# kwea123/nsff_pl

Measured on AMD Instinct MI355X. Metric: ray-samples/sec (coarse+fine, static+dynamic), higher is better.
Workload: dtype f16x3 (fp32 operands split into 2 halfs, 3 f16 MFMAs per product, fp32 accumulate; same 1e-4 parity as f32); 1 GPU; C2 (BASELINE.json configs[1]): static+dynamic NSFF, 1024 rays/GPU x (64 coarse + 64 importance -> 192 fine pts), train-mode fwd, fw/bw flow warp t+-1, perturb=1 noise_std=1, 8x256 MLPs, N_tau=48, all 47 outputs on device.  `value` is render_rays' throughput with autograd DISABLED (the train-mode FLAGS, inference launches: nothing kept for a backward pass); what a trainer's forward costs is aux.tra; rays_per_gpu=1024, N_samples=64, N_importance=64, parallelism=single GPU, field_launch=persistent (one workgroup per CU)

## Files before the change

### include/nsff_render.h

```cpp
#ifndef NSFF_RENDER_H
#define NSFF_RENDER_H

#include <stddef.h>
#include <stdint.h>

#ifdef __cplusplus
extern "C" {
#endif

#define NSFF_OK               0
#define NSFF_ERR_INVALID     -1
#define NSFF_ERR_NULL        -2
#define NSFF_ERR_ALIGN       -3
#define NSFF_ERR_HIP         -4

#define NSFF_ABI_VERSION      32
#define NSFF_RAW_STRIDE      16
#define NSFF_MAX_FREQS       24
#define NSFF_MAX_LAYERS       8


typedef struct NsffModelDesc {
    int32_t D;
    int32_t W;
// ... 43 lines not shown
    int32_t tile_points;
    int32_t pts_per_ray;
    int32_t static_mode;
    int32_t transient_mode;
    int32_t flow_heads;
    const float* xyz;
    int32_t n_freqs;
    float   freqs[NSFF_MAX_FREQS];
    const float* dir_emb;
    const float* a_emb;
    const float* t_emb;
    const float* x_emb;
    int32_t ld_emb;
    int32_t off_xyz, off_dir, off_a, off_t;
    float*  raw;
    void*   save_acts;
    void*   save_xin;
    void*   save_masks;
    void*   save_side;
    const float* t_bias;
    int32_t t_bias_rows;
    int32_t reserved0;
    const float* s_bias;
    int32_t s_bias_rows;
    int32_t launch_form;
    int64_t save_lo_delta[3];
} NsffFieldArgs;

int nsff_field_query(const NsffModelDesc* desc, const void* packed,
                     const NsffFieldArgs* args, void* stream);

#define NSFF_MAX_TIME_BIAS_JOBS 4
typedef struct NsffTimeBiasJob {
    const NsffModelDesc* desc;
    const float* w[NSFF_MAX_LAYERS];
    const float* b[NSFF_MAX_LAYERS];
    const float* t_rows;
    float* out;
    const float* table;
    const int64_t* ts;
    int64_t n_table, max_t;
    int32_t delta, pad_;
    float* rows_out;
} NsffTimeBiasJob;
int nsff_time_bias_rows(const NsffModelDesc* desc);
int nsff_time_bias(const NsffTimeBiasJob* jobs, int32_t n_jobs, int64_t n_rays, void* stream);

#define NSFF_MAX_RNG_JOBS 12
typedef struct NsffRngJob {
    float*   out;
    int64_t  numel;
    uint64_t offset;
    int32_t  kind;
    uint32_t grid;
} NsffRngJob;
int nsff_rng_draws(const NsffRngJob* jobs, int32_t n_jobs, uint64_t seed, void* stream);
typedef struct NsffRngCoarse {
    const float* rays;
    const float* z_lin;
    float*       zs;
    float*       xyz;
    int32_t      n_samples;
    float        perturb;
    int32_t      job;
    int32_t      pad_;
} NsffRngCoarse;
int nsff_rng_draws_coarse(const NsffRngJob* jobs, int32_t n_jobs, uint64_t seed, const NsffRngCoarse* coarse, void* stream);

int nsff_side_bias(const NsffModelDesc* desc, const void* packed_f16x3, const float* w_dir, const float* dir_rows,
                   const float* a_rows, int64_t n_rays, float* out, void* stream);

int nsff_train_dims(const NsffModelDesc* desc, int32_t* xin_rows, int32_t* t_row0, int32_t* side_rows);
int nsff_bwd_packed_bytes(const NsffModelDesc* desc, size_t* bytes);
int nsff_pack_weights_bwd(const NsffModelDesc* desc, const float* const* params, void* packed, void* stream);
int nsff_pack_weights_bwd_ex(const NsffModelDesc* desc, const float* const* params, void* packed, const void* fwd_packed, void* stream);

typedef struct NsffFieldBwdArgs {
    int64_t n_points;
    int32_t static_mode;
    int32_t transient_mode;
    const float* d_raw;
    const float* raw;
    const float* gmax;
    const void*  masks;
    void*  dpre;
    void*  dhead;
    float* d_xin;
    float* d_side;
    int64_t dpre_lo_delta;
} NsffFieldBwdArgs;
int nsff_field_backward(const NsffModelDesc* desc, const void* packed_bwd, const NsffFieldBwdArgs* args, void* stream);
int nsff_last_bwd_kernel(void);
int nsff_last_bwd_grid(void);
int nsff_field_bwd_phase_program(const NsffModelDesc* desc, int32_t dynamic, int32_t want_xin, int64_t n_tiles, uint32_t* out,
                                 int32_t max_phases, uint32_t* seg_offsets, int32_t max_segs);

#define NSFF_BWD_LAUNCH_C    1
#define NSFF_BWD_LAUNCH_H3B  2
#define NSFF_BWD_LAUNCH_X3   3
int nsff_field_bwd_launch_plan(const NsffModelDesc* desc, const NsffFieldBwdArgs* args, int32_t n_cus, int32_t kernel_override,
                               int32_t persist, int32_t* out, int32_t max_launches);

int nsff_field_input_backward(const float* d_xin, int32_t xin_rows, int32_t t_row0, const float* xyz, int64_t n_rays,
                              int32_t pts_per_ray, const float* freqs_host, int32_t n_freqs, int32_t in_t, float* d_xyz,
                              float* d_t, void* stream);

typedef struct NsffWgradJob {
    const void* a;  const void* b;
    int32_t a_rows, b_rows;
    int64_t out_off;
    int32_t trunk, pad_;
    int64_t a_lo_delta, b_lo_delta;
} NsffWgradJob;
int64_t nsff_weight_grad_scratch(const NsffWgradJob* jobs, int32_t n_jobs, int64_t n_tiles, int32_t n_splits);
int nsff_weight_grad(const NsffWgradJob* jobs, int32_t n_jobs, int64_t n_tiles, int32_t n_splits,
                     float* scratch, float* out, float* bias, const float* gmax, void* stream);

typedef struct NsffGradMapEntry {
    int32_t dst;
    int32_t e_a, e_b;
    int16_t job_a, job_b;
} NsffGradMapEntry;
int nsff_weight_grad_accumulate(const NsffWgradJob* jobs, int32_t n_jobs, int64_t n_tiles, int32_t n_splits, float* scratch,
                                const NsffGradMapEntry* map, int64_t n_map, float* grad_base, const float* gmax, void* stream);

int nsff_weight_grad_accumulate_aux(const NsffWgradJob* jobs, int32_t n_jobs, int64_t n_tiles, int32_t n_splits, float* scratch,
                                    const NsffGradMapEntry* map, int64_t n_map, float* grad_base, float* aux, const float* gmax,
                                    void* stream);

typedef struct NsffFoldGradArgs {
    int32_t n_rows, pad_;
    const float* g; const float* gb;
    const float* w_final; const float* b_final;
    const float* w_head[16];
    float* d_w_head[16]; float* d_b_head[16];
    float* d_w_final; float* d_b_final;
} NsffFoldGradArgs;
int nsff_fold_grads(const NsffFoldGradArgs* args, void* stream);

typedef struct NsffFoldDenseArgs {
    int32_t n_rows, accumulate;
    int32_t ld_head, ld_dhead;
    const float* g; const float* g2; const float* gb; const float* gb2;
    const float* w_head; const float* w_final; const float* b_final;
    float* d_w_head; float* d_b_head; float* d_w_final; float* d_b_final;
} NsffFoldDenseArgs;
int nsff_fold_grads_dense(const NsffFoldDenseArgs* args, void* stream);

int nsff_absmax(const float* x, int64_t n, float* out, void* stream);
int nsff_absmax_raw(const float* d_raw, int64_t n_points, float* out16, void* stream);

int nsff_adam_step(float* param, const float* grad, float* exp_avg, float* exp_avg_sq, int64_t n, float* state,
                   const float* lr, double beta1, double beta2, double eps, double weight_decay, void* stream);

int nsff_adam_step_segments(float* param, const float* grad, float* exp_avg, float* exp_avg_sq, int64_t n, float* state,
                            const float* lr, double beta1, double beta2, double eps, double weight_decay,
                            const int64_t* seg_start, int n_seg, int32_t* seg_used, void* stream);

int nsff_sgd_step(float* param, const float* grad, float* momentum_buf, int64_t n, float* state, const float* lr,
                  double momentum, double weight_decay, const int64_t* seg_start, int n_seg, int32_t* seg_used, void* stream);

int nsff_radam_step(float* param, const float* grad, float* exp_avg, float* exp_avg_sq, int64_t n, float* state,
                    const float* lr, double beta1, double beta2, double eps, double weight_decay,
                    const int64_t* seg_start, int n_seg, int32_t* seg_used, void* stream);

typedef struct NsffLossArgs {
    int64_t n_rays; int32_t n_samples; int32_t n_keep;
    int32_t n_frames; int32_t max_t;
    double  topk;
    int32_t thickness; int32_t pad_;
    const float* rgb_fine; const float* rgb_coarse;
    const float* depth_fine; const float* depth_coarse;
    const float* t_weights; const float* s_weights;
    const float* xyz_fw; const float* xyz_bw;
    const float* rgb_fw; const float* rgb_bw;
    const float* disocc_fw; const float* disocc_bw;
    const float* disoccs_fw; const float* disoccs_bw;
    const float* xyzs_fw_bw; const float* xyzs_bw_fw;
    const float* xyzs_fine; const float* xyzs_fw; const float* xyzs_bw;
    const float* rgbs; const float* disps;
    const int64_t* ts; const int64_t* cam_ids;
    const float* uv_fw; const float* uv_bw;
    const float* Ks; const float* Ps;
    const float* hyper;
    float* stats;
    float* terms;
    const float* term_w;
    const float* weights;
    float* per_ray;
    float* coef;
    float* g_rgb_fine; float* g_rgb_coarse; float* g_depth_fine; float* g_depth_coarse;
    float* g_t_weights; float* g_s_weights; float* g_xyz_fw; float* g_xyz_bw; float* g_rgb_fw; float* g_rgb_bw;
    float* g_xyzs_fw_bw; float* g_xyzs_bw_fw; float* g_xyzs_fw; float* g_xyzs_bw;
} NsffLossArgs;
int nsff_nerfw_loss(const NsffLossArgs* args, int mode, void* stream);
#define NSFF_LOSS_MAX_RAYS 1048576
size_t nsff_nerfw_loss_work_bytes(long long n_rays);
int nsff_nerfw_loss_ex(const NsffLossArgs* args, int mode, void* work, size_t work_bytes, void* stream);
int nsff_last_loss_path(void);

int nsff_coarse_samples(const float* rays, int64_t n_rays, const float* z_lin, int32_t n_samples,
                        float perturb, const float* perturb_rand,
                        float* zs, float* xyz, void* stream);

int nsff_fine_samples(const float* rays, int64_t n_rays, const float* z_lin, const float* zs_coarse,
                      int32_t n_samples, int32_t n_importance,
                      const float* weights_static, const float* weights_transient,
                      const float* u_static, const float* u_transient, int32_t u_per_ray,
                      float* samples_static, float* samples_transient,
                      float* zs_fine, float* xyz_fine, void* stream);

int nsff_sample_pdf(const float* bins, const float* weights, int64_t n_rays, int32_t n_bins_minus1,
                    const float* u, int32_t n_importance, int32_t u_per_ray, float eps,
                    float* samples, void* stream);

int nsff_warp_points(const float* raw, const float* xyz, const float* zs, int64_t n_points,
                     float z_far, float* xyz_fw, float* xyz_bw, void* stream);

int nsff_frame_rays(const float* K4_host, const float* c2w_host, int32_t H, int32_t W, float near, float shift_near,
                    int64_t first_pixel, int64_t n_pixels, float* rays, void* stream);

#define NSFF_FRAME_TABLE     16
typedef struct NsffRayRecordArgs {
    int32_t n_frames, H, W;
    int32_t first_frame, frame_count;
    int32_t image_u8, mask_u8;
    float   fx, fy, cx, cy, near;
    int64_t n_pixels;
    const void*  images;
    const float* disps;
    const void*  masks;
    const float* flow_fw;
    const float* flow_bw;
    const float* frame_table;
    float*       records;
} NsffRayRecordArgs;
int nsff_ray_records(const NsffRayRecordArgs* args, void* stream);

#define NSFF_ERR_UNSUPPORTED     -5
#define NSFF_RESIZE_LANCZOS_U8    0
#define NSFF_RESIZE_NEAREST_PIL   1
#define NSFF_RESIZE_NEAREST_CV    2
#define NSFF_RESIZE_LINEAR_CV     3
#define NSFF_RESIZE_MAX_KSIZE    49
int nsff_resize_ksize(int32_t filter, int32_t n_in, int32_t n_out);
int nsff_resize_table(int32_t filter, int32_t n_in, int32_t n_out, int32_t* start, int32_t* count, void* weights);

typedef struct NsffFrameResizeArgs {
    int32_t n_frames, filter, channels, pad_;
    int32_t src_h, src_w, dst_h, dst_w;
    int32_t ksize_x, ksize_y;
    float   ratio[2];
    const void* src;  void* dst;
    const int32_t* x_start;  const int32_t* x_count;  const void* x_weights;
    const int32_t* y_start;  const int32_t* y_count;  const void* y_weights;
} NsffFrameResizeArgs;
int nsff_frame_resize(const NsffFrameResizeArgs* args, void* stream);

typedef struct NsffFrustumArgs {
    const float*   w2c;
    const int64_t* ts;
    float   K4[4];
    int32_t n_cams, n_frames, H, W;
} NsffFrustumArgs;

typedef struct NsffCompositeArgs {
    int64_t n_rays;
    int32_t n_samples;
    int32_t has_transient;
    int32_t has_rgb;
    int32_t flow_mode;
    int32_t want_disocc;
    float   noise_std;
    float   z_far;
    const float* raw;
    const float* raw_fw;
    const float* raw_bw;
    const float* zs;
    const float* xyz;
    const float* xyz_fw;
    const float* xyz_bw;
    const float* noise_static;
    const float* noise_transient;
    const float* noise_fw;
    const float* noise_bw;
    const float* visibility;
    float* static_rgbs;  float* transient_rgbs;
    float* flows_fw;     float* flows_bw;
    float* static_sigmas; float* transient_sigmas;
    float* static_alphas; float* transient_alphas;
    float* static_weights; float* transient_weights; float* weights;
    float* xyzs_fw_bw;   float* xyzs_bw_fw;
    float* disoccs_fw;   float* disoccs_bw;
    float* depth;  float* rgb;  float* transient_alpha;  float* transient_rgb;
    float* static_only_rgb;  float* static_only_depth;
    float* xyz_exp;  float* flow_fw_exp;  float* flow_bw_exp;  float* xyz_fw_exp;  float* xyz_bw_exp;
    float* rgb_fw;   float* rgb_bw;
    float* disocc_fw;  float* disocc_bw;
    NsffFrustumArgs vis;
} NsffCompositeArgs;

int nsff_composite(const NsffCompositeArgs* args, void* stream);

int nsff_frustum_visibility(const NsffFrustumArgs* vis, const float* xyz, int64_t n_points, float* vis_count,
                            void* stream);

typedef struct NsffSplatArgs {
    int32_t H, W, n_planes;
    float   K4[4];
    float   P[12];
    float   scale;
    const float* xyz;
    const float* flow;
    const float* rgb;
    const float* alpha;
    float*       accum;
    void*        work;
    int64_t      work_bytes;
} NsffSplatArgs;
int64_t nsff_splat_work_bytes(int32_t H, int32_t W, int32_t n_planes);
int nsff_splat_planes(const NsffSplatArgs* args, void* stream);

typedef struct NsffMpiArgs {
    int32_t H, W, n_planes;
    float   dt;
    const float* accum_fw;
    const float* accum_bw;
    const float* static_rgb;
    const float* static_alpha;
    const float* zs;
    float* rgb;
    float* depth;
} NsffMpiArgs;
int nsff_mpi_composite(const NsffMpiArgs* args, void* stream);

typedef struct NsffCompositeBwdArgs {
    int64_t n_rays;
    int32_t n_samples, has_transient, flow_mode;
    float   noise_std;
    const float* raw;  const float* raw_fw;  const float* raw_bw;
    const float* zs;   const float* xyz;     const float* f_fw;  const float* f_bw;
    const float* noise_static;  const float* noise_transient;  const float* noise_fw;  const float* noise_bw;
    const float* g_static_sigmas;  const float* g_transient_sigmas;
    const float* g_static_weights; const float* g_transient_weights;  const float* g_weights;
    const float* g_depth;  const float* g_rgb;  const float* g_transient_alpha;  const float* g_transient_rgb;
    const float* g_so_rgb; const float* g_so_depth;
    const float* g_xyz_exp;  const float* g_flow_fw_exp;  const float* g_flow_bw_exp;
    const float* g_rgb_fw;   const float* g_rgb_bw;
    float* scratch;
    float* d_raw;  float* d_raw_fw;  float* d_raw_bw;  float* d_f_fw;  float* d_f_bw;
} NsffCompositeBwdArgs;
int nsff_composite_backward(const NsffCompositeBwdArgs* args, void* stream);

typedef struct {
    int64_t n_points;
    const float* zs;
    float z_far;
    int32_t accumulate;
    int32_t col_a, col_b;
    int32_t pad_;
    const float* g_a[4];
    const float* g_b[4];
    float* out;
} NsffFlowGradArgs;
int nsff_flow_grad(const NsffFlowGradArgs* args, void* stream);

#define NSFF_RAY_RECORD      16

typedef struct NsffSsimArgs {
    int32_t n_frames, H, W, window;
    const float* gt;  const float* pred;  const uint8_t* mask;
    float* map;  float* mean_map;  double* sums;
    void* scratch;  int64_t scratch_bytes;
} NsffSsimArgs;
int64_t nsff_ssim_scratch_bytes(int32_t n_frames, int32_t H, int32_t W);
int nsff_ssim(const NsffSsimArgs* args, void* stream);

typedef struct NsffFrameFinishArgs {
    int32_t n_frames, H, W, pad_;
    const float* rgb;  const float* gt;  const uint8_t* valid;  const float* depth;  const uint8_t* lut;
    float* rgb_clipped;  uint8_t* rgb_u8;  double* sums;  float* depth_range;  uint8_t* depth_u8;  uint8_t* depth_rgb_u8;
    void* scratch;  int64_t scratch_bytes;
} NsffFrameFinishArgs;
int64_t nsff_frame_finish_scratch_bytes(int32_t n_frames, int32_t H, int32_t W);
int nsff_frame_finish(const NsffFrameFinishArgs* args, void* stream);

typedef struct NsffValPanelsArgs {
    int32_t n_frames, H, W, pad_;
    const float* gt;  const float* pred;  const float* depth;  const float* transient_alpha;  const float* static_rgb;
    const float* static_depth;  const float* mask;  const float* disp;  const float* ssim_loss;
    const uint8_t* lut_depth;  const uint8_t* lut_mask;
    float* ranges;  uint8_t* grid_u8;  uint8_t* rmse_u8;  uint8_t* ssim_u8;  uint8_t* rmse_blend_u8;  uint8_t* ssim_blend_u8;
    void* scratch;  int64_t scratch_bytes;
} NsffValPanelsArgs;
int64_t nsff_val_panels_scratch_bytes(int32_t n_frames, int32_t H, int32_t W);
int nsff_val_panels(const NsffValPanelsArgs* args, void* stream);

#define NSFF_FLOW_UNKNOWN    1e10f
typedef struct NsffFlowMapsArgs {
    int32_t n_frames, H, W, n_poses, max_t, share_gt_scale;
    float   fx, fy, cx, cy;
    const float* xyz[2];  const float* Ps;  const int32_t* ts;
    float* flow[2];  const float* gt[2];  const uint8_t* mask;
    double* epe_sums;  int64_t* epe_counts;  float* maxrad;  const float* scale;
    uint8_t* image[2];  uint8_t* gt_image[2];
    void* scratch;  int64_t scratch_bytes;
} NsffFlowMapsArgs;
int64_t nsff_flow_maps_scratch_bytes(int32_t n_frames, int32_t H, int32_t W);
int nsff_flow_maps(const NsffFlowMapsArgs* args, void* stream);

#define NSFF_TRACK_MAX_POINTS 0x7fffffffLL
typedef struct NsffTrackStepArgs {
    int64_t n_rows;
    int32_t pts_per_row, direction, max_t, n_poses, fixed_view, pad_;
    float   fx, fy, cx, cy;
    const float* raw;  const float* xyz_in;  const int32_t* t_in;  const uint8_t* alive_in;
    float* xyz_out;  int32_t* t_out;  uint8_t* alive_out;
    const float* Ps;  float* uv;  float* depth;
} NsffTrackStepArgs;
int nsff_track_step(const NsffTrackStepArgs* args, void* stream);

#define NSFF_TRACK_MAX_TRACKS (1 << 20)
#define NSFF_TRACK_MAX_STEPS  (1 << 11)
typedef struct NsffTrackDrawArgs {
    int32_t H, W, n_steps, n_tracks;
    const float* uv;  const uint8_t* ok;  const uint8_t* image;  const uint8_t* lut;  uint8_t* out;
    void* scratch;  int64_t scratch_bytes;
} NsffTrackDrawArgs;
int64_t nsff_track_draw_scratch_bytes(int32_t H, int32_t W);
int nsff_track_draw(const NsffTrackDrawArgs* args, void* stream);

typedef struct NsffMotionMapsArgs {
    int32_t n_frames, H, W, epipolar;
    float   alpha, beta, threshold, pad_;
    const float* flow_fw;  const float* flow_bw;  const float* Fm;
    float* err;  uint8_t* valid;  uint8_t* raw;
    int64_t* counts;  double* err_sums;
    void* scratch;  int64_t scratch_bytes;
} NsffMotionMapsArgs;
int64_t nsff_motion_maps_scratch_bytes(int32_t n_frames, int32_t H, int32_t W);
int nsff_motion_maps(const NsffMotionMapsArgs* args, void* stream);

#define NSFF_ERODE_MAX_K 31
typedef struct NsffMaskErodeArgs {
    int32_t n_frames, H, W, k;
    const uint8_t* src;  uint8_t* dst;  int64_t* zero_counts;
    void* scratch;  int64_t scratch_bytes;
} NsffMaskErodeArgs;
int nsff_mask_erode(const NsffMaskErodeArgs* args, void* stream);

#define NSFF_OPTFLOW_MIN_SIZE 16
#define NSFF_OPTFLOW_TILE     32
#define NSFF_OPTFLOW_K        3
#define NSFF_OPTFLOW_FUSED    1
typedef struct NsffOptflowIterArgs {
    int32_t n_pairs, H, W, iters;
    int32_t fused, tile, k, pad_;
    float   lambda, theta, tau, pad1_;
    const float* consts;  float* state[2];
} NsffOptflowIterArgs;
typedef struct NsffOptflowArgs {
    int32_t n_pairs, H, W, channels;
    int32_t levels, warps, iters, median;
    int32_t fused, tile, k, pad_;
    float   lambda, theta, tau, pad1_;
    const void* images0;  const void* images1;  float* flow;
    void* scratch;  int64_t scratch_bytes;
} NsffOptflowArgs;
int     nsff_optflow_grey(const void* src, float* dst, int32_t n, int32_t H, int32_t W, int32_t channels, void* stream);
int     nsff_optflow_down(const float* src, float* dst, int32_t n, int32_t H, int32_t W, void* stream);
int     nsff_optflow_up(const float* src, float* dst, int32_t n, int32_t H, int32_t W, void* stream);
int     nsff_optflow_median(const float* src, float* dst, int32_t n, int32_t H, int32_t W, void* stream);
int     nsff_optflow_warp(const float* I0, const float* I1, const float* u, float* consts, int32_t n_pairs, int32_t H, int32_t W,
                          void* stream);
int     nsff_optflow_iterate(const NsffOptflowIterArgs* args, void* stream);
int     nsff_optflow_result_slot(int32_t iters, int32_t k);
int     nsff_optflow_levels(int32_t H, int32_t W, int32_t levels);
int64_t nsff_optflow_scratch_bytes(int32_t n_pairs, int32_t H, int32_t W, int32_t levels);
int     nsff_optflow(const NsffOptflowArgs* args, void* stream);

int nsff_cdf(const float* weights, int64_t n_frames, int64_t n, double* cdf, void* stream);

typedef struct NsffRayDrawArgs {
    int64_t n_frames, n_pixels, frame, batch;
    const float* records;  const double* cdf;  const float* u;
    float* rays;  float* rgbs;  int64_t* ts;  int64_t* cam_ids;  float* disps;  float* rays_mask;  float* uv_fw;  float* uv_bw;
    int64_t* rand_idx;
} NsffRayDrawArgs;
int nsff_ray_draw(const NsffRayDrawArgs* args, void* stream);

int nsff_prof_enable(int on);
int nsff_prof_collect(int64_t* launches, double* total_ms, double* total_flops, double* executed_flops);
int nsff_prof_collect_clock(int64_t* launches, double* total_ms, double* total_flops, double* executed_flops,
                            double* shader_ticks, double* ticks_ms);

#define NSFF_KERNEL_F32       1
#define NSFF_KERNEL_H3_64     2
#define NSFF_KERNEL_H3_8WAVE  3
#define NSFF_KERNEL_H3A       4
#define NSFF_KERNEL_H3_SAVE   5
#define NSFF_KERNEL_H3A_TBIAS 7
#define NSFF_KERNEL_H3A_SAVE  9
#define NSFF_KERNEL_H3A_SIDE  8
int         nsff_last_field_kernel(void);
int         nsff_last_field_grid(void);
int         nsff_field_mfma_shape(const NsffModelDesc* desc, const NsffFieldArgs* args);
int         nsff_repack_field_weights(const NsffModelDesc* desc, const void* packed, void* repacked, void* stream);
int         nsff_field_query_repacked(const NsffModelDesc* desc, const void* packed, const void* repacked, const NsffFieldArgs* args,
                                      void* stream);
int         nsff_last_field_mfma_shape(void);
int         nsff_field_phase_program(const NsffModelDesc* desc, int static_mode, int transient_mode, int fold_t, uint32_t* steps,
                             int* n_steps, int* n_static_steps, uint32_t* phases_static, uint32_t* phases_dynamic, int* n_phases);

#define NSFF_PLAN_WORDS 12
#define NSFF_LAUNCH_SIDE_TILE      1
#define NSFF_LAUNCH_H3_64          2
#define NSFF_LAUNCH_H3_64_SAVE     3
#define NSFF_LAUNCH_H3_8WAVE       4
#define NSFF_LAUNCH_H3_8WAVE_SAVE  5
#define NSFF_LAUNCH_H3A            6
#define NSFF_LAUNCH_H3A_SAVE       7
int         nsff_field_launch_plan(const NsffModelDesc* desc, const NsffFieldArgs* args, int32_t n_cus, int32_t no_persist,
                                   int32_t* out, int32_t max_launches);

#define NSFF_RANGE_ACT     0x1u
#define NSFF_RANGE_SAVED   0x2u
#define NSFF_RANGE_PARAMS  0x4u
#define NSFF_RANGE_CODES   0x8u
int         nsff_range_flags(uint32_t* out, int32_t clear, void* stream);

#define NSFF_LPIPS_MIN_SIZE  31

typedef struct NsffLpipsWeights {
    const float* conv_w[5];  const float* conv_b[5];  const float* lin[5];
} NsffLpipsWeights;
int64_t nsff_lpips_packed_bytes(void);
int     nsff_lpips_pack(const NsffLpipsWeights* weights, float* packed, void* stream);

int     nsff_lpips_dims(int32_t H, int32_t W, int32_t* hw);

typedef struct NsffLpipsArgs {
    int32_t n_frames, H, W, normalize;
    const float* gt;  const float* pred;  const uint8_t* valid;
    const float* packed;
    float* map;  double* sums;
    void* workspace;  int64_t workspace_bytes;
} NsffLpipsArgs;
int64_t nsff_lpips_workspace_bytes(int32_t n_frames, int32_t H, int32_t W);
int     nsff_lpips(const NsffLpipsArgs* args, void* stream);

typedef struct NsffSceneScaleArgs {
    int32_t n_frames, n_points, H, W;
    int32_t disp_rank[2];
    const double* points;  const uint8_t* vis;  const double* w2c;  const float* K;  const float* disps;
    double* stats;  float* disp_os;  double* depth_os;  int32_t* pix;
    void* work;  int64_t work_bytes;
} NsffSceneScaleArgs;
int64_t nsff_scene_scale_work_bytes(int32_t n_frames, int32_t n_points, int32_t H, int32_t W);
int     nsff_scene_scale(const NsffSceneScaleArgs* args, void* stream);

int         nsff_abi_version(void);
const char* nsff_last_hip_error(void);

#ifdef __cplusplus
}
#endif
#endif
```

### nsff_pl_amd/_lib.py

```python
import ctypes as C
import os

import torch

_HERE = os.path.dirname(os.path.abspath(__file__))
LIB_PATH = os.environ.get("NSFF_LIB") or os.path.join(_HERE, "libnsff_hip.so")

RAW_STRIDE = 16
ABI_VERSION = 32
MAX_FREQS = 24

_ERR = {-1: "NSFF_ERR_INVALID (bad shape/flag/unsupported architecture)",
        -2: "NSFF_ERR_NULL (required pointer missing)",
        -3: "NSFF_ERR_ALIGN (pointer not 16-byte aligned)",
        -4: "NSFF_ERR_HIP",
        -5: "NSFF_ERR_UNSUPPORTED (a valid request outside what the kernels are built for)"}

_fp = C.c_void_p


class ModelDesc(C.Structure):
    _fields_ = [("D", C.c_int32), ("W", C.c_int32), ("skip", C.c_int32),
                ("in_xyz", C.c_int32), ("in_dir", C.c_int32), ("in_a", C.c_int32),
                ("in_t", C.c_int32), ("use_viewdir", C.c_int32),
                ("has_transient", C.c_int32), ("has_flow", C.c_int32),
                ("flow_scale", C.c_float), ("skip_mask", C.c_int32)]


class FieldArgs(C.Structure):
    _fields_ = [("n_points", C.c_int64), ("precision", C.c_int32), ("tile_points", C.c_int32),
                ("pts_per_ray", C.c_int32),
                ("static_mode", C.c_int32), ("transient_mode", C.c_int32),
                ("flow_heads", C.c_int32),
                ("xyz", _fp), ("n_freqs", C.c_int32), ("freqs", C.c_float * MAX_FREQS),
                ("dir_emb", _fp), ("a_emb", _fp), ("t_emb", _fp),
                ("x_emb", _fp), ("ld_emb", C.c_int32),
                ("off_xyz", C.c_int32), ("off_dir", C.c_int32), ("off_a", C.c_int32),
                ("off_t", C.c_int32), ("raw", _fp), ("save_acts", _fp), ("save_xin", _fp), ("save_masks", _fp),
                ("save_side", _fp), ("t_bias", _fp), ("t_bias_rows", C.c_int32), ("reserved0", C.c_int32),
                ("s_bias", _fp), ("s_bias_rows", C.c_int32), ("launch_form", C.c_int32), ("save_lo_delta", C.c_int64 * 3)]


class TimeBiasJob(C.Structure):
    _fields_ = [("desc", C.POINTER(ModelDesc)), ("w", _fp * 8), ("b", _fp * 8), ("t_rows", _fp), ("out", _fp),
                ("table", _fp), ("ts", _fp), ("n_table", C.c_int64), ("max_t", C.c_int64), ("delta", C.c_int32), ("pad_", C.c_int32),
                ("rows_out", _fp)]


MAX_TIME_BIAS_JOBS = 4


class RngJob(C.Structure):
    _fields_ = [("out", _fp), ("numel", C.c_int64), ("offset", C.c_uint64), ("kind", C.c_int32), ("grid", C.c_uint32)]


MAX_RNG_JOBS = 12


class RngCoarse(C.Structure):
    _fields_ = [("rays", _fp), ("z_lin", _fp), ("zs", _fp), ("xyz", _fp), ("n_samples", C.c_int32), ("perturb", C.c_float),
                ("job", C.c_int32), ("pad_", C.c_int32)]


_COMPOSITE_PTRS_IN = ["raw", "raw_fw", "raw_bw", "zs", "xyz", "xyz_fw", "xyz_bw",
                      "noise_static", "noise_transient", "noise_fw", "noise_bw", "visibility"]
_COMPOSITE_PTRS_OUT = ["static_rgbs", "transient_rgbs", "flows_fw", "flows_bw",
                       "static_sigmas", "transient_sigmas", "static_alphas", "transient_alphas",
                       "static_weights", "transient_weights", "weights",
                       "xyzs_fw_bw", "xyzs_bw_fw", "disoccs_fw", "disoccs_bw",
                       "depth", "rgb", "transient_alpha", "transient_rgb",
                       "static_only_rgb", "static_only_depth",
                       "xyz_exp", "flow_fw_exp", "flow_bw_exp", "xyz_fw_exp", "xyz_bw_exp",
                       "rgb_fw", "rgb_bw", "disocc_fw", "disocc_bw"]


class FrustumArgs(C.Structure):
    _fields_ = [("w2c", _fp), ("ts", _fp), ("K4", C.c_float * 4), ("n_cams", C.c_int32), ("n_frames", C.c_int32),
                ("H", C.c_int32), ("W", C.c_int32)]


class CompositeArgs(C.Structure):
    _fields_ = ([("n_rays", C.c_int64), ("n_samples", C.c_int32), ("has_transient", C.c_int32),
                 ("has_rgb", C.c_int32), ("flow_mode", C.c_int32), ("want_disocc", C.c_int32),
                 ("noise_std", C.c_float), ("z_far", C.c_float)]
                + [(n, _fp) for n in _COMPOSITE_PTRS_IN]
                + [(n, _fp) for n in _COMPOSITE_PTRS_OUT]
                + [("vis", FrustumArgs)])


_CBWD_IN = ["raw", "raw_fw", "raw_bw", "zs", "xyz", "f_fw", "f_bw", "noise_static", "noise_transient", "noise_fw", "noise_bw"]
_CBWD_G = ["g_static_sigmas", "g_transient_sigmas", "g_static_weights", "g_transient_weights", "g_weights", "g_depth",
           "g_rgb", "g_transient_alpha", "g_transient_rgb", "g_so_rgb", "g_so_depth", "g_xyz_exp", "g_flow_fw_exp",
           "g_flow_bw_exp", "g_rgb_fw", "g_rgb_bw"]
_CBWD_OUT = ["scratch", "d_raw", "d_raw_fw", "d_raw_bw", "d_f_fw", "d_f_bw"]


class CompositeBwdArgs(C.Structure):
    _fields_ = ([("n_rays", C.c_int64), ("n_samples", C.c_int32), ("has_transient", C.c_int32), ("flow_mode", C.c_int32),
                 ("noise_std", C.c_float)] + [(n, _fp) for n in _CBWD_IN + _CBWD_G + _CBWD_OUT])


class FieldBwdArgs(C.Structure):
    _fields_ = [("n_points", C.c_int64), ("static_mode", C.c_int32), ("transient_mode", C.c_int32),
                ("d_raw", _fp), ("raw", _fp), ("gmax", _fp), ("masks", _fp), ("dpre", _fp), ("dhead", _fp),
                ("d_xin", _fp), ("d_side", _fp), ("dpre_lo_delta", C.c_int64)]


class WgradJob(C.Structure):
    _fields_ = [("a", _fp), ("b", _fp), ("a_rows", C.c_int32), ("b_rows", C.c_int32), ("out_off", C.c_int64), ("trunk", C.c_int32),
                ("pad_", C.c_int32), ("a_lo_delta", C.c_int64), ("b_lo_delta", C.c_int64)]


class FoldGradArgs(C.Structure):
    _fields_ = [("n_rows", C.c_int32), ("pad_", C.c_int32), ("g", _fp), ("gb", _fp), ("w_final", _fp), ("b_final", _fp),
                ("w_head", _fp * 16), ("d_w_head", _fp * 16), ("d_b_head", _fp * 16), ("d_w_final", _fp), ("d_b_final", _fp)]


class FoldDenseArgs(C.Structure):
    _fields_ = [("n_rows", C.c_int32), ("accumulate", C.c_int32), ("ld_head", C.c_int32), ("ld_dhead", C.c_int32),
                ("g", _fp), ("g2", _fp), ("gb", _fp), ("gb2", _fp), ("w_head", _fp), ("w_final", _fp), ("b_final", _fp),
                ("d_w_head", _fp), ("d_b_head", _fp), ("d_w_final", _fp), ("d_b_final", _fp)]


class SplatArgs(C.Structure):
    _fields_ = [("H", C.c_int32), ("W", C.c_int32), ("n_planes", C.c_int32), ("K4", C.c_float * 4),
                ("P", C.c_float * 12), ("scale", C.c_float),
                ("xyz", _fp), ("flow", _fp), ("rgb", _fp), ("alpha", _fp), ("accum", _fp), ("work", _fp),
                ("work_bytes", C.c_int64)]


class MpiArgs(C.Structure):
    _fields_ = [("H", C.c_int32), ("W", C.c_int32), ("n_planes", C.c_int32), ("dt", C.c_float),
                ("accum_fw", _fp), ("accum_bw", _fp), ("static_rgb", _fp), ("static_alpha", _fp), ("zs", _fp),
                ("rgb", _fp), ("depth", _fp)]


_LOSS_IN = ["rgb_fine", "rgb_coarse", "depth_fine", "depth_coarse", "t_weights", "s_weights", "xyz_fw", "xyz_bw", "rgb_fw",
            "rgb_bw", "disocc_fw", "disocc_bw", "disoccs_fw", "disoccs_bw", "xyzs_fw_bw", "xyzs_bw_fw", "xyzs_fine",
            "xyzs_fw", "xyzs_bw", "rgbs", "disps", "ts", "cam_ids", "uv_fw", "uv_bw", "Ks", "Ps", "hyper", "stats", "terms",
            "term_w"]
LOSS_GRADS = ["g_rgb_fine", "g_rgb_coarse", "g_depth_fine", "g_depth_coarse", "g_t_weights", "g_s_weights", "g_xyz_fw",
              "g_xyz_bw", "g_rgb_fw", "g_rgb_bw", "g_xyzs_fw_bw", "g_xyzs_bw_fw", "g_xyzs_fw", "g_xyzs_bw"]


class LossArgs(C.Structure):
    _fields_ = ([("n_rays", C.c_int64), ("n_samples", C.c_int32), ("n_keep", C.c_int32), ("n_frames", C.c_int32),
                 ("max_t", C.c_int32), ("topk", C.c_double), ("thickness", C.c_int32), ("pad_", C.c_int32)]
                + [(n, _fp) for n in _LOSS_IN] + [("weights", _fp), ("per_ray", _fp), ("coef", _fp)]
                + [(n, _fp) for n in LOSS_GRADS])


class FlowGradArgs(C.Structure):
    _fields_ = [("n_points", C.c_int64), ("zs", _fp), ("z_far", C.c_float), ("accumulate", C.c_int32), ("col_a", C.c_int32),
                ("col_b", C.c_int32), ("pad_", C.c_int32), ("g_a", _fp * 4), ("g_b", _fp * 4), ("out", _fp)]


class SsimArgs(C.Structure):
    _fields_ = [("n_frames", C.c_int32), ("H", C.c_int32), ("W", C.c_int32), ("window", C.c_int32),
                ("gt", _fp), ("pred", _fp), ("mask", _fp), ("map", _fp), ("mean_map", _fp), ("sums", _fp),
                ("scratch", _fp), ("scratch_bytes", C.c_int64)]


class LpipsWeights(C.Structure):
    _fields_ = [("conv_w", _fp * 5), ("conv_b", _fp * 5), ("lin", _fp * 5)]


class LpipsArgs(C.Structure):
    _fields_ = [("n_frames", C.c_int32), ("H", C.c_int32), ("W", C.c_int32), ("normalize", C.c_int32),
                ("gt", _fp), ("pred", _fp), ("valid", _fp), ("packed", _fp), ("map", _fp), ("sums", _fp),
                ("workspace", _fp), ("workspace_bytes", C.c_int64)]


_FINISH_PTRS = ["rgb", "gt", "valid", "depth", "lut", "rgb_clipped", "rgb_u8", "sums", "depth_range", "depth_u8", "depth_rgb_u8"]


class FrameFinishArgs(C.Structure):
    _fields_ = ([("n_frames", C.c_int32), ("H", C.c_int32), ("W", C.c_int32), ("pad_", C.c_int32)]
                + [(n, _fp) for n in _FINISH_PTRS] + [("scratch", _fp), ("scratch_bytes", C.c_int64)])


_PANEL_IN = ["gt", "pred", "depth", "transient_alpha", "static_rgb", "static_depth", "mask", "disp", "ssim_loss"]
_PANEL_LUT = ["lut_depth", "lut_mask"]
_PANEL_OUT = ["ranges", "grid_u8", "rmse_u8", "ssim_u8", "rmse_blend_u8", "ssim_blend_u8"]
PANEL_FIELDS = ("depth", "static_depth", "neg_disp", "neg_rmse", "neg_ssim")


class ValPanelsArgs(C.Structure):
    _fields_ = ([("n_frames", C.c_int32), ("H", C.c_int32), ("W", C.c_int32), ("pad_", C.c_int32)]
                + [(n, _fp) for n in _PANEL_IN + _PANEL_LUT + _PANEL_OUT] + [("scratch", _fp), ("scratch_bytes", C.c_int64)])


FLOW_UNKNOWN = 1e10


class FlowMapsArgs(C.Structure):
    _fields_ = [("n_frames", C.c_int32), ("H", C.c_int32), ("W", C.c_int32), ("n_poses", C.c_int32), ("max_t", C.c_int32),
                ("share_gt_scale", C.c_int32), ("fx", C.c_float), ("fy", C.c_float), ("cx", C.c_float), ("cy", C.c_float),
                ("xyz", _fp * 2), ("Ps", _fp), ("ts", _fp), ("flow", _fp * 2), ("gt", _fp * 2), ("mask", _fp),
                ("epe_sums", _fp), ("epe_counts", _fp), ("maxrad", _fp), ("scale", _fp), ("image", _fp * 2), ("gt_image", _fp * 2),
                ("scratch", _fp), ("scratch_bytes", C.c_int64)]


TRACK_MAX_POINTS, TRACK_MAX_TRACKS, TRACK_MAX_STEPS = 0x7fffffff, 1 << 20, 1 << 11


class TrackStepArgs(C.Structure):
    _fields_ = [("n_rows", C.c_int64), ("pts_per_row", C.c_int32), ("direction", C.c_int32), ("max_t", C.c_int32),
                ("n_poses", C.c_int32), ("fixed_view", C.c_int32), ("pad_", C.c_int32),
                ("fx", C.c_float), ("fy", C.c_float), ("cx", C.c_float), ("cy", C.c_float),
                ("raw", _fp), ("xyz_in", _fp), ("t_in", _fp), ("alive_in", _fp), ("xyz_out", _fp), ("t_out", _fp), ("alive_out", _fp),
                ("Ps", _fp), ("uv", _fp), ("depth", _fp)]


class TrackDrawArgs(C.Structure):
    _fields_ = [("H", C.c_int32), ("W", C.c_int32), ("n_steps", C.c_int32), ("n_tracks", C.c_int32),
                ("uv", _fp), ("ok", _fp), ("image", _fp), ("lut", _fp), ("out", _fp), ("scratch", _fp), ("scratch_bytes", C.c_int64)]


ERODE_MAX_K = 31


class MotionMapsArgs(C.Structure):
    _fields_ = [("n_frames", C.c_int32), ("H", C.c_int32), ("W", C.c_int32), ("epipolar", C.c_int32),
                ("alpha", C.c_float), ("beta", C.c_float), ("threshold", C.c_float), ("pad_", C.c_float),
                ("flow_fw", _fp), ("flow_bw", _fp), ("Fm", _fp), ("err", _fp), ("valid", _fp), ("raw", _fp),
                ("counts", _fp), ("err_sums", _fp), ("scratch", _fp), ("scratch_bytes", C.c_int64)]


class MaskErodeArgs(C.Structure):
    _fields_ = [("n_frames", C.c_int32), ("H", C.c_int32), ("W", C.c_int32), ("k", C.c_int32),
                ("src", _fp), ("dst", _fp), ("zero_counts", _fp), ("scratch", _fp), ("scratch_bytes", C.c_int64)]


OPTFLOW_MIN_SIZE, OPTFLOW_TILE, OPTFLOW_K, OPTFLOW_FUSED = 16, 32, 3, 1
OPTFLOW_PAIRS = ((16, 2), (32, 2), (32, 3), (32, 4), (32, 6))


class OptflowIterArgs(C.Structure):
    _fields_ = [("n_pairs", C.c_int32), ("H", C.c_int32), ("W", C.c_int32), ("iters", C.c_int32),
                ("fused", C.c_int32), ("tile", C.c_int32), ("k", C.c_int32), ("pad_", C.c_int32),
                ("lam", C.c_float), ("theta", C.c_float), ("tau", C.c_float), ("pad1_", C.c_float),
                ("consts", _fp), ("state", _fp * 2)]


class OptflowArgs(C.Structure):
    _fields_ = [("n_pairs", C.c_int32), ("H", C.c_int32), ("W", C.c_int32), ("channels", C.c_int32),
                ("levels", C.c_int32), ("warps", C.c_int32), ("iters", C.c_int32), ("median", C.c_int32),
                ("fused", C.c_int32), ("tile", C.c_int32), ("k", C.c_int32), ("pad_", C.c_int32),
                ("lam", C.c_float), ("theta", C.c_float), ("tau", C.c_float), ("pad1_", C.c_float),
                ("images0", _fp), ("images1", _fp), ("flow", _fp), ("scratch", _fp), ("scratch_bytes", C.c_int64)]


RAY_RECORD = 16
_DRAW_OUT = ["rays", "rgbs", "ts", "cam_ids", "disps", "rays_mask", "uv_fw", "uv_bw", "rand_idx"]


class RayDrawArgs(C.Structure):
    _fields_ = ([("n_frames", C.c_int64), ("n_pixels", C.c_int64), ("frame", C.c_int64), ("batch", C.c_int64),
                 ("records", _fp), ("cdf", _fp), ("u", _fp)] + [(n, _fp) for n in _DRAW_OUT])


FRAME_TABLE = 16


class RayRecordArgs(C.Structure):
    _fields_ = [("n_frames", C.c_int32), ("H", C.c_int32), ("W", C.c_int32), ("first_frame", C.c_int32),
                ("frame_count", C.c_int32), ("image_u8", C.c_int32), ("mask_u8", C.c_int32),
                ("fx", C.c_float), ("fy", C.c_float), ("cx", C.c_float), ("cy", C.c_float), ("near", C.c_float),
                ("n_pixels", C.c_int64), ("images", _fp), ("disps", _fp), ("masks", _fp), ("flow_fw", _fp), ("flow_bw", _fp),
                ("frame_table", _fp), ("records", _fp)]


RESIZE_LANCZOS_U8, RESIZE_NEAREST_PIL, RESIZE_NEAREST_CV, RESIZE_LINEAR_CV = range(4)
RESIZE_MAX_KSIZE = 49
ERR_UNSUPPORTED = -5


class FrameResizeArgs(C.Structure):
    _fields_ = [("n_frames", C.c_int32), ("filter", C.c_int32), ("channels", C.c_int32), ("pad_", C.c_int32),
                ("src_h", C.c_int32), ("src_w", C.c_int32), ("dst_h", C.c_int32), ("dst_w", C.c_int32),
                ("ksize_x", C.c_int32), ("ksize_y", C.c_int32), ("ratio", C.c_float * 2), ("src", _fp), ("dst", _fp),
                ("x_start", _fp), ("x_count", _fp), ("x_weights", _fp), ("y_start", _fp), ("y_count", _fp), ("y_weights", _fp)]


class SceneScaleArgs(C.Structure):
    _fields_ = [("n_frames", C.c_int32), ("n_points", C.c_int32), ("H", C.c_int32), ("W", C.c_int32),
                ("disp_rank", C.c_int32 * 2), ("points", _fp), ("vis", _fp), ("w2c", _fp), ("K", _fp), ("disps", _fp),
                ("stats", _fp), ("disp_os", _fp), ("depth_os", _fp), ("pix", _fp), ("work", _fp), ("work_bytes", C.c_int64)]


_SIGNATURES = {
    "nsff_abi_version": (C.c_int, []),
    "nsff_range_flags": (C.c_int, [_fp, C.c_int32, _fp]),
    "nsff_last_field_kernel": (C.c_int, []),
    "nsff_last_field_grid": (C.c_int, []),
    "nsff_field_mfma_shape": (C.c_int, [C.POINTER(ModelDesc), C.POINTER(FieldArgs)]),
    "nsff_repack_field_weights": (C.c_int, [C.POINTER(ModelDesc), _fp, _fp, _fp]),
    "nsff_field_query_repacked": (C.c_int, [C.POINTER(ModelDesc), _fp, _fp, C.POINTER(FieldArgs), _fp]),
    "nsff_last_field_mfma_shape": (C.c_int, []),
    "nsff_field_phase_program": (C.c_int, [C.POINTER(ModelDesc), C.c_int, C.c_int, C.c_int, C.POINTER(C.c_uint32), C.POINTER(C.c_int),
                                   C.POINTER(C.c_int), C.POINTER(C.c_uint32), C.POINTER(C.c_uint32), C.POINTER(C.c_int)]),
    "nsff_field_launch_plan": (C.c_int, [C.POINTER(ModelDesc), C.POINTER(FieldArgs), C.c_int32, C.c_int32, C.POINTER(C.c_int32), C.c_int32]),
    "nsff_time_bias_rows": (C.c_int, [C.POINTER(ModelDesc)]),
    "nsff_time_bias": (C.c_int, [C.POINTER(TimeBiasJob), C.c_int32, C.c_int64, C.c_void_p]),
    "nsff_rng_draws": (C.c_int, [C.POINTER(RngJob), C.c_int32, C.c_uint64, C.c_void_p]),
    "nsff_rng_draws_coarse": (C.c_int, [C.POINTER(RngJob), C.c_int32, C.c_uint64, C.POINTER(RngCoarse), C.c_void_p]),
    "nsff_side_bias": (C.c_int, [C.POINTER(ModelDesc), _fp, _fp, _fp, _fp, C.c_int64, _fp, C.c_void_p]),
    "nsff_last_hip_error": (C.c_char_p, []),
    "nsff_packed_bytes": (C.c_int, [C.POINTER(ModelDesc), C.c_int, C.POINTER(C.c_size_t)]),
    "nsff_param_count": (C.c_int, [C.POINTER(ModelDesc)]),
    "nsff_pack_weights": (C.c_int, [C.POINTER(ModelDesc), C.c_int, C.POINTER(_fp), _fp, _fp]),
    "nsff_pack_weights_ex": (C.c_int, [C.POINTER(ModelDesc), C.c_int, C.POINTER(_fp), _fp, C.c_int32, _fp]),
    "nsff_fold_heads": (C.c_int, [C.POINTER(ModelDesc), C.c_int, C.POINTER(_fp), _fp, _fp]),
    "nsff_posenc": (C.c_int, [_fp, C.c_int64, C.POINTER(C.c_float), C.c_int, _fp, _fp]),
    "nsff_time_rows": (C.c_int, [_fp, C.c_int64, C.c_int32, _fp, C.c_int64, C.c_int64, _fp, _fp, _fp]),
    "nsff_time_rows_backward": (C.c_int, [_fp, _fp, _fp, _fp, C.c_int64, C.c_int64, C.c_int64, C.c_int32, _fp, _fp]),
    "nsff_field_query": (C.c_int, [C.POINTER(ModelDesc), _fp, C.POINTER(FieldArgs), _fp]),
    "nsff_coarse_samples": (C.c_int, [_fp, C.c_int64, _fp, C.c_int32, C.c_float, _fp, _fp, _fp, _fp]),
    "nsff_fine_samples": (C.c_int, [_fp, C.c_int64, _fp, _fp, C.c_int32, C.c_int32, _fp, _fp, _fp, _fp,
                                    C.c_int32, _fp, _fp, _fp, _fp, _fp]),
    "nsff_sample_pdf": (C.c_int, [_fp, _fp, C.c_int64, C.c_int32, _fp, C.c_int32, C.c_int32,
                                  C.c_float, _fp, _fp]),
    "nsff_warp_points": (C.c_int, [_fp, _fp, _fp, C.c_int64, C.c_float, _fp, _fp, _fp]),
    "nsff_composite": (C.c_int, [C.POINTER(CompositeArgs), _fp]),
    "nsff_frustum_visibility": (C.c_int, [C.POINTER(FrustumArgs), _fp, C.c_int64, _fp, _fp]),
    "nsff_frame_rays": (C.c_int, [C.POINTER(C.c_float), C.POINTER(C.c_float), C.c_int32, C.c_int32, C.c_float,
                                  C.c_float, C.c_int64, C.c_int64, _fp, _fp]),
    "nsff_ray_records": (C.c_int, [C.POINTER(RayRecordArgs), _fp]),
    "nsff_resize_ksize": (C.c_int, [C.c_int32, C.c_int32, C.c_int32]),
    "nsff_resize_table": (C.c_int, [C.c_int32, C.c_int32, C.c_int32, C.c_void_p, C.c_void_p, C.c_void_p]),
    "nsff_frame_resize": (C.c_int, [C.POINTER(FrameResizeArgs), _fp]),
    "nsff_scene_scale_work_bytes": (C.c_int64, [C.c_int32, C.c_int32, C.c_int32, C.c_int32]),
    "nsff_scene_scale": (C.c_int, [C.POINTER(SceneScaleArgs), _fp]),
    "nsff_bwd_packed_bytes": (C.c_int, [C.POINTER(ModelDesc), C.POINTER(C.c_size_t)]),
    "nsff_pack_weights_bwd": (C.c_int, [C.POINTER(ModelDesc), C.POINTER(_fp), _fp, _fp]),
    "nsff_field_backward": (C.c_int, [C.POINTER(ModelDesc), _fp, C.POINTER(FieldBwdArgs), _fp]),
    "nsff_field_input_backward": (C.c_int, [_fp, C.c_int32, C.c_int32, _fp, C.c_int64, C.c_int32, C.POINTER(C.c_float), C.c_int32,
                                            C.c_int32, _fp, _fp, _fp]),
    "nsff_train_dims": (C.c_int, [C.POINTER(ModelDesc), C.POINTER(C.c_int32), C.POINTER(C.c_int32), C.POINTER(C.c_int32)]),
    "nsff_weight_grad_scratch": (C.c_int64, [C.POINTER(WgradJob), C.c_int32, C.c_int64, C.c_int32]),
    "nsff_weight_grad": (C.c_int, [C.POINTER(WgradJob), C.c_int32, C.c_int64, C.c_int32, _fp, _fp, _fp, _fp, _fp]),
    "nsff_weight_grad_accumulate": (C.c_int, [C.POINTER(WgradJob), C.c_int32, C.c_int64, C.c_int32, _fp, _fp, C.c_int64,
                                              _fp, _fp, _fp]),
    "nsff_weight_grad_accumulate_aux": (C.c_int, [C.POINTER(WgradJob), C.c_int32, C.c_int64, C.c_int32, _fp, _fp, C.c_int64,
                                                  _fp, _fp, _fp, _fp]),
    "nsff_absmax_raw": (C.c_int, [_fp, C.c_int64, _fp, _fp]),
    "nsff_last_bwd_kernel": (C.c_int, []),
    "nsff_last_bwd_grid": (C.c_int, []),
    "nsff_field_bwd_phase_program": (C.c_int, [C.POINTER(ModelDesc), C.c_int32, C.c_int32, C.c_int64, C.POINTER(C.c_uint32), C.c_int32,
                                                C.POINTER(C.c_uint32), C.c_int32]),
    "nsff_field_bwd_launch_plan": (C.c_int, [C.POINTER(ModelDesc), C.POINTER(FieldBwdArgs), C.c_int32, C.c_int32, C.c_int32,
                                             C.POINTER(C.c_int32), C.c_int32]),
    "nsff_fold_grads": (C.c_int, [C.POINTER(FoldGradArgs), _fp]),
    "nsff_fold_grads_dense": (C.c_int, [C.POINTER(FoldDenseArgs), _fp]),
    "nsff_pack_weights_bwd_ex": (C.c_int, [C.POINTER(ModelDesc), C.POINTER(_fp), _fp, _fp, _fp]),
    "nsff_absmax": (C.c_int, [_fp, C.c_int64, _fp, _fp]),
    "nsff_adam_step": (C.c_int, [_fp, _fp, _fp, _fp, C.c_int64, _fp, _fp, C.c_double, C.c_double, C.c_double, C.c_double, _fp]),
    "nsff_adam_step_segments": (C.c_int, [_fp, _fp, _fp, _fp, C.c_int64, _fp, _fp, C.c_double, C.c_double, C.c_double, C.c_double,
                                          _fp, C.c_int, _fp, _fp]),
    "nsff_sgd_step": (C.c_int, [_fp, _fp, _fp, C.c_int64, _fp, _fp, C.c_double, C.c_double, _fp, C.c_int, _fp, _fp]),
    "nsff_radam_step": (C.c_int, [_fp, _fp, _fp, _fp, C.c_int64, _fp, _fp, C.c_double, C.c_double, C.c_double, C.c_double,
                                  _fp, C.c_int, _fp, _fp]),
    "nsff_composite_backward": (C.c_int, [C.POINTER(CompositeBwdArgs), _fp]),
    "nsff_flow_grad": (C.c_int, [C.POINTER(FlowGradArgs), _fp]),
    "nsff_nerfw_loss": (C.c_int, [C.POINTER(LossArgs), C.c_int, _fp]),
    "nsff_nerfw_loss_work_bytes": (C.c_size_t, [C.c_longlong]),
    "nsff_nerfw_loss_ex": (C.c_int, [C.POINTER(LossArgs), C.c_int, _fp, C.c_size_t, _fp]),
    "nsff_last_loss_path": (C.c_int, []),
    "nsff_splat_planes": (C.c_int, [C.POINTER(SplatArgs), _fp]),
    "nsff_splat_work_bytes": (C.c_int64, [C.c_int32, C.c_int32, C.c_int32]),
    "nsff_mpi_composite": (C.c_int, [C.POINTER(MpiArgs), _fp]),
    "nsff_ssim_scratch_bytes": (C.c_int64, [C.c_int32, C.c_int32, C.c_int32]),
    "nsff_ssim": (C.c_int, [C.POINTER(SsimArgs), _fp]),
    "nsff_lpips_packed_bytes": (C.c_int64, []),
    "nsff_lpips_pack": (C.c_int, [C.POINTER(LpipsWeights), _fp, _fp]),
    "nsff_lpips_dims": (C.c_int, [C.c_int32, C.c_int32, C.POINTER(C.c_int32)]),
    "nsff_lpips_workspace_bytes": (C.c_int64, [C.c_int32, C.c_int32, C.c_int32]),
    "nsff_lpips": (C.c_int, [C.POINTER(LpipsArgs), _fp]),
    "nsff_frame_finish_scratch_bytes": (C.c_int64, [C.c_int32, C.c_int32, C.c_int32]),
    "nsff_frame_finish": (C.c_int, [C.POINTER(FrameFinishArgs), _fp]),
    "nsff_val_panels_scratch_bytes": (C.c_int64, [C.c_int32, C.c_int32, C.c_int32]),
    "nsff_val_panels": (C.c_int, [C.POINTER(ValPanelsArgs), _fp]),
    "nsff_flow_maps_scratch_bytes": (C.c_int64, [C.c_int32, C.c_int32, C.c_int32]),
    "nsff_flow_maps": (C.c_int, [C.POINTER(FlowMapsArgs), _fp]),
    "nsff_track_step": (C.c_int, [C.POINTER(TrackStepArgs), _fp]),
    "nsff_track_draw_scratch_bytes": (C.c_int64, [C.c_int32, C.c_int32]),
    "nsff_track_draw": (C.c_int, [C.POINTER(TrackDrawArgs), _fp]),
    "nsff_motion_maps_scratch_bytes": (C.c_int64, [C.c_int32, C.c_int32, C.c_int32]),
    "nsff_motion_maps": (C.c_int, [C.POINTER(MotionMapsArgs), _fp]),
    "nsff_mask_erode": (C.c_int, [C.POINTER(MaskErodeArgs), _fp]),
    "nsff_optflow_grey": (C.c_int, [_fp, _fp, C.c_int32, C.c_int32, C.c_int32, C.c_int32, _fp]),
    "nsff_optflow_down": (C.c_int, [_fp, _fp, C.c_int32, C.c_int32, C.c_int32, _fp]),
    "nsff_optflow_up": (C.c_int, [_fp, _fp, C.c_int32, C.c_int32, C.c_int32, _fp]),
    "nsff_optflow_median": (C.c_int, [_fp, _fp, C.c_int32, C.c_int32, C.c_int32, _fp]),
    "nsff_optflow_warp": (C.c_int, [_fp, _fp, _fp, _fp, C.c_int32, C.c_int32, C.c_int32, _fp]),
    "nsff_optflow_iterate": (C.c_int, [C.POINTER(OptflowIterArgs), _fp]),
    "nsff_optflow_result_slot": (C.c_int, [C.c_int32, C.c_int32]),
    "nsff_optflow_levels": (C.c_int, [C.c_int32, C.c_int32, C.c_int32]),
    "nsff_optflow_scratch_bytes": (C.c_int64, [C.c_int32, C.c_int32, C.c_int32, C.c_int32]),
    "nsff_optflow": (C.c_int, [C.POINTER(OptflowArgs), _fp]),
    "nsff_cdf": (C.c_int, [_fp, C.c_int64, C.c_int64, _fp, _fp]),
    "nsff_ray_draw": (C.c_int, [C.POINTER(RayDrawArgs), _fp]),
    "nsff_prof_enable": (C.c_int, [C.c_int]),
    "nsff_prof_collect": (C.c_int, [C.POINTER(C.c_int64), C.POINTER(C.c_double), C.POINTER(C.c_double), C.POINTER(C.c_double)]),
    "nsff_prof_collect_clock": (C.c_int, [C.POINTER(C.c_int64)] + [C.POINTER(C.c_double)] * 5),
}
EXPORTED_SYMBOLS = tuple(_SIGNATURES)

_lib = None


def load():
    global _lib
    if _lib is None:
        if not os.path.exists(LIB_PATH):
            raise RuntimeError(
                f"{LIB_PATH} is missing: build it with `python -c 'import __graft_entry__ as g; g.build()'` "
                "(or `make -C nsff_pl_amd/csrc`).  There is no CPU fallback for the render path.")
        lib = C.CDLL(LIB_PATH)
        for name, (res, args) in _SIGNATURES.items():
            fn = getattr(lib, name)
            fn.restype, fn.argtypes = res, args
        if lib.nsff_abi_version() != ABI_VERSION:
            raise RuntimeError("libnsff_hip.so ABI version mismatch")
        _lib = lib
    return _lib


def _check(rc, what):
    if rc != 0:
        msg = _ERR.get(rc, f"error {rc}")
        if rc == -4:
            msg += ": " + load().nsff_last_hip_error().decode()
        raise RuntimeError(f"{what} failed: {msg}")


def require_gpu_tensor(t, what):
    if not isinstance(t, torch.Tensor) or not t.is_cuda:
        raise RuntimeError(f"{what} must be a GPU tensor: the NSFF render path runs only on the "
                           "HIP kernels of libnsff_hip.so (no CPU fallback)")


def _ptr(t):
    if t is None:
        return None
    assert t.is_cuda and t.dtype == torch.float32 and t.is_contiguous(), "need contiguous fp32 GPU tensor"
    return t.data_ptr()


def _stream():
    return torch.cuda.current_stream().cuda_stream


def model_desc(model):
    if model.W != 256:
        raise RuntimeError(f"unsupported NeRF architecture: W={model.W} (the gfx950 field kernels tile W=256 trunks "
                           "into 4 x 64-neuron wave blocks; other widths are not built)")
    skips = sorted(set(int(s) for s in model.skips))
    if not 2 <= model.D <= 8 or any(not 1 <= s < model.D for s in skips):
        raise RuntimeError(f"unsupported NeRF architecture: D={model.D}, skips={list(model.skips)} (need 2 <= D <= 8 "
                           "and every skip layer in 1..D-1; a skip at layer 0 would concatenate the input with itself)")
    mask = sum(1 << s for s in skips)
    return ModelDesc(D=model.D, W=model.W, skip=skips[0] if len(skips) == 1 else 0, skip_mask=mask if len(skips) != 1 else 0,
                     in_xyz=model.in_channels_xyz,
                     in_dir=model.in_channels_dir,
                     in_a=model.in_channels_a if model.use_viewdir else 0,
                     in_t=model.in_channels_t, use_viewdir=int(model.use_viewdir),
                     has_transient=int(model.encode_transient),
                     has_flow=int(getattr(model, "has_flow_heads", hasattr(model, "transient_flow_fw"))),
                     flow_scale=float(getattr(model, "flow_scale", 0.0)))


def param_list(model):
    def lin(m):
        layer = m[0] if isinstance(m, torch.nn.Sequential) else m
        return [layer.weight, layer.bias]
    out = []
    for i in range(model.D):
        out += lin(getattr(model, f"static_xyz_encoding_{i + 1}"))
    out += lin(model.static_xyz_encoding_final)
    if model.use_viewdir:
        out += lin(model.static_dir_encoding)
    out += lin(model.static_sigma) + lin(model.static_rgb)
    if model.encode_transient:
        for i in range(model.D):
            out += lin(getattr(model, f"transient_xyz_encoding_{i + 1}"))
        out += lin(model.transient_xyz_encoding_final)
        out += lin(model.transient_sigma) + lin(model.transient_rgb)
        if hasattr(model, "transient_flow_fw"):
            out += lin(model.transient_flow_fw) + lin(model.transient_flow_bw)
    return out


def packed_bytes(desc, precision=0):
    n = C.c_size_t(0)
    _check(load().nsff_packed_bytes(C.byref(desc), int(precision), C.byref(n)), "nsff_packed_bytes")
    return n.value


PACK_SKIP_FOLD = 1


def pack_weights(desc, params, packed, precision=0, fold=True):
    lib = load()
    if lib.nsff_param_count(C.byref(desc)) != len(params):
        raise RuntimeError("parameter list does not match the model description")
    keep = [p.detach().contiguous().float() for p in params]
    for p in keep:
        require_gpu_tensor(p, "model parameter")
    arr = (_fp * len(keep))(*[p.data_ptr() for p in keep])
    _check(lib.nsff_pack_weights_ex(C.byref(desc), int(precision), arr, _ptr(packed), 0 if fold else PACK_SKIP_FOLD,
                                    _stream()), "nsff_pack_weights_ex")
    return keep


def fold_heads(desc, params, packed, precision):
    keep = [p.detach().contiguous().float() for p in params]
    arr = (_fp * len(keep))(*[p.data_ptr() for p in keep])
    _check(load().nsff_fold_heads(C.byref(desc), int(precision), arr, _ptr(packed), _stream()), "nsff_fold_heads")
    return keep


def time_rows_backward(g_cur, g_next, g_prev, ts, max_t, n_table):
    gs = [None if g is None else g.contiguous() for g in (g_cur, g_next, g_prev)]
    width = next(g for g in gs if g is not None).shape[1]
    assert ts.dtype == torch.int64 and ts.is_cuda and ts.is_contiguous()
    d = torch.empty(int(n_table), width, device=ts.device)
    _check(load().nsff_time_rows_backward(_ptr(gs[0]), _ptr(gs[1]), _ptr(gs[2]), C.c_void_p(ts.data_ptr()), ts.shape[0],
                                          int(max_t), int(n_table), width, _ptr(d), _stream()), "nsff_time_rows_backward")
    return d


def time_rows(table, ts, max_t, want_next=True, want_prev=True):
    n, width = ts.shape[0], table.shape[1]
    if want_next and want_prev:
        both = torch.empty(2, n, width, device=table.device)
        nxt, prv = both[0], both[1]
    else:
        nxt = torch.empty(n, width, device=table.device) if want_next else None
        prv = torch.empty(n, width, device=table.device) if want_prev else None
    assert ts.dtype == torch.int64 and ts.is_cuda and ts.is_contiguous()
    _check(load().nsff_time_rows(_ptr(table), table.shape[0], width, C.c_void_p(ts.data_ptr()), n, int(max_t),
                                 _ptr(nxt), _ptr(prv), _stream()), "nsff_time_rows")
    return nxt, prv


def posenc(x, freqs, out):
    f = [float(v) for v in freqs]
    arr = (C.c_float * len(f))(*f)
    _check(load().nsff_posenc(_ptr(x), x.shape[0], arr, len(f), _ptr(out), _stream()), "nsff_posenc")


def field_query(model, raw, n_points, pts_per_ray, static_mode, transient_mode, flow_heads=0,
                xyz=None, freqs=None, dir_emb=None, a_emb=None, t_emb=None,
                x_emb=None, emb_offsets=(0, -1, -1, -1), save_acts=None, save_xin=None, save_masks=None, save_side=None,
                precision=None, t_bias=None, s_bias=None, save_lo=False):
    from . import config
    desc = model_desc(model)
    prec = config.precision_code(model) if precision is None else precision
    saves = not (save_acts is None and save_xin is None and save_masks is None and save_side is None)
    packed = model.packed(prec)
    a = FieldArgs()
    a.precision, a.tile_points = prec, config.get_tile_points()
    a.launch_form = 0 if config.get_persistent() else 1
    a.n_points, a.pts_per_ray = int(n_points), int(pts_per_ray)
    a.static_mode, a.transient_mode, a.flow_heads = int(static_mode), int(transient_mode), int(flow_heads)
    a.xyz = _ptr(xyz)
    if freqs is not None:
        f = [float(v) for v in freqs]
        if len(f) > MAX_FREQS:
            raise RuntimeError("too many embedding frequencies")
        a.n_freqs = len(f)
        for i, v in enumerate(f):
            a.freqs[i] = v
    a.dir_emb, a.a_emb, a.t_emb = _ptr(dir_emb), _ptr(a_emb), _ptr(t_emb)
    a.x_emb = _ptr(x_emb)
    a.ld_emb = int(x_emb.shape[1]) if x_emb is not None else 0
    a.off_xyz, a.off_dir, a.off_a, a.off_t = [int(v) for v in emb_offsets]
    a.raw = _ptr(raw)
    a.save_acts = None if save_acts is None else save_acts.data_ptr()
    a.save_xin = None if save_xin is None else save_xin.data_ptr()
    a.save_masks = None if save_masks is None else save_masks.data_ptr()
    a.save_side = None if save_side is None else save_side.data_ptr()
    if save_lo:
        for i, t in enumerate((save_acts, save_xin, save_side)):
            a.save_lo_delta[i] = 0 if t is None else lo_delta(t)
    if t_bias is not None:
        a.t_bias, a.t_bias_rows = _ptr(t_bias), int(t_bias.shape[1])
    if s_bias is not None:
        a.s_bias, a.s_bias_rows = _ptr(s_bias), int(s_bias.shape[1])
    if os.environ.get("NSFF_H3A_SHAPE") != "32" and prec == config.PRECISIONS["f16x3"] and not saves and \
            load().nsff_field_mfma_shape(C.byref(desc), C.byref(a)) == 16:
        _check(load().nsff_field_query_repacked(C.byref(desc), _ptr(packed), _ptr(model.packed(REPACKED)), C.byref(a), _stream()),
               "nsff_field_query_repacked")
        return
    _check(load().nsff_field_query(C.byref(desc), _ptr(packed), C.byref(a), _stream()), "nsff_field_query")


def lo_delta(t):
    n = t.numel()
    if t.untyped_storage().nbytes() < (t.storage_offset() + 2 * n) * t.element_size():
        raise RuntimeError("three-product backward: this buffer has no remainder plane behind it (field_grad.alloc_saves(..., x3=True))")
    return n


def side_bias(model, dir_rows, a_rows=None):
    from . import config
    desc = model_desc(model)
    n_rays = int(dir_rows.shape[0])
    assert dir_rows.shape == (n_rays, desc.in_dir) and (desc.in_a == 0 or (a_rows is not None and a_rows.shape == (n_rays, desc.in_a)))
    packed = model.packed(config.PRECISIONS["f16x3"])
    w = model.static_dir_encoding[0].weight.detach()
    out = torch.empty(n_rays, 1, 256, device=dir_rows.device, dtype=torch.float32)
    _check(load().nsff_side_bias(C.byref(desc), _ptr(packed), _ptr(w), _ptr(dir_rows), _ptr(a_rows) if desc.in_a > 0 else None,
                                 n_rays, _ptr(out), _stream()), "nsff_side_bias")
    return out


_DEVICE_RNG_GEOMETRY = {}


def fused_draws(plan, device, values=True, coarse=None):
    dev = torch.device(device)
    idx = dev.index if dev.index is not None else torch.cuda.current_device()
    if idx not in _DEVICE_RNG_GEOMETRY:
        p = torch.cuda.get_device_properties(idx)
        _DEVICE_RNG_GEOMETRY[idx] = p.multi_processor_count * (p.max_threads_per_multi_processor // 256)
    max_grid = _DEVICE_RNG_GEOMETRY[idx]
    gen = torch.cuda.default_generators[idx]
    seed, offset = gen.initial_seed(), gen.get_offset()
    wanted = values if isinstance(values, (list, tuple)) else [bool(values)] * len(plan)
    sizes = []
    for kind, shape in plan:
        n = 1
        for s in shape:
            n *= int(s)
        sizes.append(n)
    total = sum(n for n, w in zip(sizes, wanted) if w)
    buf = torch.empty(max(total, 1), device=dev, dtype=torch.float32)
    outs, jobs, at = [], [], 0
    for (kind, shape), numel, want in zip(plan, sizes, wanted):
        if numel == 0:
            outs.append(torch.empty(*shape, device=dev, dtype=torch.float32))
            continue
        grid = min(max_grid, (numel + 255) // 256)
        if coarse is not None and not outs and not want:
            jobs.append((None, numel, offset, 0, grid))
            outs.append(None)
        elif want:
            t = buf[at:at + numel].view(*shape)
            at += numel
            jobs.append((t, numel, offset, 1 if kind == "randn" else 0, grid))
            outs.append(t)
        else:
            outs.append(None)
        offset += ((numel - 1) // (1024 * grid) + 1) * 4
    hook = None
    if coarse is not None:
        rays, z_lin, perturb, zs, xyz = coarse
        assert plan and plan[0][0] == "rand" and tuple(plan[0][1]) == (rays.shape[0], z_lin.shape[0]) and perturb > 0
        if sizes[0]:
            hook = RngCoarse(_ptr(rays), _ptr(z_lin), _ptr(zs), _ptr(xyz), int(z_lin.shape[0]), float(perturb), 0, 0)
    for k in range(0, len(jobs), MAX_RNG_JOBS):
        part = jobs[k:k + MAX_RNG_JOBS]
        arr = (RngJob * len(part))()
        for j, (t, numel, off, kind, grid) in enumerate(part):
            arr[j].out, arr[j].numel, arr[j].offset, arr[j].kind, arr[j].grid = (None if t is None else t.data_ptr()), numel, off, kind, grid
        with torch.cuda.device(idx):
            _check(load().nsff_rng_draws_coarse(arr, len(part), seed, C.byref(hook) if (hook is not None and k == 0) else None, _stream()),
                   "nsff_rng_draws")
    gen.set_offset(offset)
    return outs


_FUSED_DRAWS_OK = {}


def fused_draws_match_torch(device):
    dev = torch.device(device)
    idx = dev.index if dev.index is not None else torch.cuda.current_device()
    if idx in _FUSED_DRAWS_OK:
        return _FUSED_DRAWS_OK[idx]
    if torch.cuda.is_current_stream_capturing():
        return False
    gen = torch.cuda.default_generators[idx]
    state = gen.get_state()
    ok = True
    try:
        plan = [("rand", (7, 64)), ("randn", (1031,)), ("rand", (3, 5, 2)), ("randn", (70000,)), ("rand", (300001,))]
        gen.manual_seed(0x5EED1234)
        gen.set_offset(8)
        mine = fused_draws(plan, torch.device("cuda", idx))
        end_mine = gen.get_offset()
        gen.manual_seed(0x5EED1234)
        gen.set_offset(8)
        with torch.cuda.device(idx):
            ref = [(torch.rand if k == "rand" else torch.randn)(*shape, device=torch.device("cuda", idx)) for k, shape in plan]
        end_ref = gen.get_offset()
        ok = end_mine == end_ref and all(torch.equal(a.view(torch.int32), b.view(torch.int32)) for a, b in zip(mine, ref))
    except Exception:
        ok = False
    finally:
        gen.set_state(state)
    if not ok:
        import warnings
        warnings.warn("nsff_pl_amd: the fused generator kernel (nsff_rng_draws) no longer reproduces torch.rand / torch.randn on "
                      f"cuda:{idx} (torch {torch.__version__}); render_rays draws with the torch calls instead (slower by ~1 %, same "
                      "numbers as the reference)")
    _FUSED_DRAWS_OK[idx] = ok
    return ok


def time_bias_rows(model):
    return load().nsff_time_bias_rows(C.byref(model_desc(model)))


def time_bias(jobs, index=None):
    assert 1 <= len(jobs) <= MAX_TIME_BIAS_JOBS
    arr = (TimeBiasJob * len(jobs))()
    keep, outs, per_model, pair = [], [], {}, None
    rows_of = {}
    if index is not None:
        table, ts, max_t = index
        assert ts.dtype == torch.int64 and ts.is_cuda and ts.is_contiguous() and ts.dim() == 1, "ts: one int64 frame index per ray"
        n_rays, width = int(ts.shape[0]), int(table.shape[1])
        deltas = sorted({int(d) for _, d in jobs})
        if 1 in deltas and -1 in deltas:
            both = torch.empty(2, n_rays, width, device=table.device, dtype=torch.float32)
            rows_of[1], rows_of[-1] = both[0], both[1]
        for d in deltas:
            if d not in rows_of:
                rows_of[d] = torch.empty(n_rays, width, device=table.device, dtype=torch.float32)
        written = set()
    else:
        n_rays = int(jobs[0][1].shape[0])
    for j, (model, t_rows) in enumerate(jobs):
        if id(model) not in per_model:
            desc = model_desc(model)
            lins = [getattr(model, f"transient_xyz_encoding_{l + 1}")[0] for l in [0] + sorted(set(int(v) for v in model.skips))]
            wb = [(m.weight.detach(), m.bias.detach()) for m in lins]
            for w, b in wb:
                _ptr(w), _ptr(b)
            per_model[id(model)] = (desc, C.pointer(desc), wb)
        desc, pdesc, wb = per_model[id(model)]
        if index is not None:
            delta, t_rows = int(t_rows), None
            assert width == desc.in_t
        else:
            assert t_rows.shape == (n_rays, desc.in_t)
        dev = wb[0][0].device
        if j + 1 < len(jobs) and jobs[j + 1][0] is model and pair is None:
            pair = torch.empty(2, n_rays, len(wb), 256, device=dev, dtype=torch.float32)
            out = pair[0]
        elif pair is not None:
            out, pair = pair[1], None
        else:
            out = torch.empty(n_rays, len(wb), 256, device=dev, dtype=torch.float32)
        arr[j].desc = pdesc
        for i, (w, b) in enumerate(wb):
            arr[j].w[i], arr[j].b[i] = w.data_ptr(), b.data_ptr()
        arr[j].t_rows, arr[j].out = _ptr(t_rows), _ptr(out)
        if index is not None:
            arr[j].table, arr[j].ts = _ptr(table), ts.data_ptr()
            arr[j].n_table, arr[j].max_t, arr[j].delta = int(table.shape[0]), int(max_t), delta
            if delta not in written:
                arr[j].rows_out = _ptr(rows_of[delta])
                written.add(delta)
        outs.append(out)
    keep.append(per_model)
    _check(load().nsff_time_bias(arr, len(jobs), n_rays, _stream()), "nsff_time_bias")
    return outs if index is None else (outs, rows_of)


def coarse_samples(rays, z_lin, perturb, perturb_rand, zs, xyz):
    _check(load().nsff_coarse_samples(_ptr(rays), rays.shape[0], _ptr(z_lin), z_lin.shape[0],
                                      float(perturb), _ptr(perturb_rand), _ptr(zs), _ptr(xyz), _stream()),
           "nsff_coarse_samples")


def fine_samples(rays, z_lin, zs_coarse, n_importance, w_static, w_transient, u_static, u_transient,
                 u_per_ray, samples_static, samples_transient, zs_fine, xyz_fine):
    _check(load().nsff_fine_samples(_ptr(rays), rays.shape[0], _ptr(z_lin), _ptr(zs_coarse),
                                    z_lin.shape[0], int(n_importance), _ptr(w_static), _ptr(w_transient),
                                    _ptr(u_static), _ptr(u_transient), int(u_per_ray),
                                    _ptr(samples_static), _ptr(samples_transient),
                                    _ptr(zs_fine), _ptr(xyz_fine), _stream()), "nsff_fine_samples")


def sample_pdf(bins, weights, u, u_per_ray, eps, samples):
    _check(load().nsff_sample_pdf(_ptr(bins), _ptr(weights), weights.shape[0], weights.shape[1],
                                  _ptr(u), samples.shape[1], int(u_per_ray), float(eps),
                                  _ptr(samples), _stream()), "nsff_sample_pdf")


def warp_points(raw, xyz, zs, z_far, xyz_fw, xyz_bw):
    _check(load().nsff_warp_points(_ptr(raw), _ptr(xyz), _ptr(zs), zs.numel(), float(z_far),
                                   _ptr(xyz_fw), _ptr(xyz_bw), _stream()), "nsff_warp_points")


def frustum_args(w2c, ts, K4, n_cams, n_frames, H, W):
    assert w2c.is_cuda and w2c.dtype == torch.float32 and w2c.is_contiguous() and w2c.shape == (n_cams * n_frames, 12)
    assert ts.is_cuda and ts.dtype == torch.int64 and ts.is_contiguous() and ts.numel() >= 1
    a = FrustumArgs(w2c=w2c.data_ptr(), ts=ts.data_ptr(), n_cams=int(n_cams), n_frames=int(n_frames), H=int(H), W=int(W))
    a.K4[:] = [float(v) for v in K4]
    a._keep = (w2c, ts)
    return a


def frustum_visibility(vis, xyz, out):
    _check(load().nsff_frustum_visibility(C.byref(vis), _ptr(xyz), xyz.shape[0], _ptr(out), _stream()),
           "nsff_frustum_visibility")


def composite(vis=None, **kw):
    a = CompositeArgs()
    for k, v in kw.items():
        if k in _COMPOSITE_PTRS_IN or k in _COMPOSITE_PTRS_OUT:
            setattr(a, k, _ptr(v))
        else:
            setattr(a, k, v)
    if vis is not None:
        a.vis = vis
    _check(load().nsff_composite(C.byref(a), _stream()), "nsff_composite")


def frame_rays(K4, c2w12, H, W, near, shift_near, first, count, rays):
    k = (C.c_float * 4)(*[float(v) for v in K4])
    m = (C.c_float * 12)(*[float(v) for v in c2w12])
    _check(load().nsff_frame_rays(k, m, int(H), int(W), float(near), float(shift_near), int(first), int(count),
                                  _ptr(rays), _stream()), "nsff_frame_rays")


REPACKED = 101


def repack_weights(desc, packed, repacked):
    _check(load().nsff_repack_field_weights(C.byref(desc), _ptr(packed), _ptr(repacked), _stream()), "nsff_repack_field_weights")


def last_field_mfma_shape():
    return int(load().nsff_last_field_mfma_shape())


BWD_PACK = 100


def bwd_packed_bytes(desc):
    n = C.c_size_t(0)
    _check(load().nsff_bwd_packed_bytes(C.byref(desc), C.byref(n)), "nsff_bwd_packed_bytes")
    return n.value


def pack_weights_bwd(desc, params, packed, fwd_packed=None):
    arr = (_fp * len(params))(*[p.data_ptr() for p in params])
    _check(load().nsff_pack_weights_bwd_ex(C.byref(desc), arr, _ptr(packed), _ptr(fwd_packed), _stream()), "nsff_pack_weights_bwd_ex")


def last_bwd_kernel():
    return {0: "c", 1: "h3b", 2: "c+h3b", 3: "x3"}[load().nsff_last_bwd_kernel()]


def last_bwd_grid():
    return load().nsff_last_bwd_grid()


PLAN_WORDS = 12


def field_launch_plan(desc, args, n_cus, no_persist=False):
    out = (C.c_int32 * (3 * PLAN_WORDS))()
    code = load().nsff_field_launch_plan(C.byref(desc), C.byref(args), int(n_cus), int(bool(no_persist)), out, 3)
    recs = [list(out[i * PLAN_WORDS:(i + 1) * PLAN_WORDS]) for i in range(3)]
    return code, [r for r in recs if r[0] != 0]


def field_bwd_launch_plan(desc, args, n_cus, kernel_override=None, persist=True):
    out = (C.c_int32 * (2 * PLAN_WORDS))()
    code = load().nsff_field_bwd_launch_plan(C.byref(desc), C.byref(args), int(n_cus), ord(kernel_override) if kernel_override else 0,
                                                      int(bool(persist)), out, 2)
    recs = [list(out[i * PLAN_WORDS:(i + 1) * PLAN_WORDS]) for i in range(2)]
    return code, [r for r in recs if r[0] != 0]


def field_bwd_phase_program(model, dynamic, want_xin, n_tiles, max_phases=32):
    import numpy as np
    desc = model_desc(model)
    out = (C.c_uint32 * (8 * max_phases))()
    segs = (C.c_uint32 * 48)()
    n = load().nsff_field_bwd_phase_program(C.byref(desc), 1 if dynamic else 0, 1 if want_xin else 0, int(n_tiles), out, max_phases, segs, 48)
    if n < 0:
        raise RuntimeError(f"nsff_field_bwd_phase_program failed ({n})")
    offs = np.array(list(segs), np.uint32)
    return (np.array(list(out), np.uint32).reshape(max_phases, 8)[:n] if n > 0 else None), offs


def field_backward(model, n_points, static, transient, d_raw, raw, gmax, masks, dpre, dhead, d_xin, d_side=None, x3=False):
    desc = model_desc(model)
    a = FieldBwdArgs(n_points=int(n_points), static_mode=2 if static else 0, transient_mode=2 if transient else 0,
                     d_raw=_ptr(d_raw), raw=_ptr(raw), gmax=_ptr(gmax), masks=masks.data_ptr(), dpre=dpre.data_ptr(),
                     dhead=dhead.data_ptr(), d_xin=_ptr(d_xin), d_side=_ptr(d_side), dpre_lo_delta=lo_delta(dpre) if x3 else 0)
    _check(load().nsff_field_backward(C.byref(desc), _ptr(model.packed(BWD_PACK)), C.byref(a), _stream()),
           "nsff_field_backward")


def train_dims(model):
    desc = model_desc(model)
    xr, t0, sr = C.c_int32(0), C.c_int32(0), C.c_int32(0)
    _check(load().nsff_train_dims(C.byref(desc), C.byref(xr), C.byref(t0), C.byref(sr)), "nsff_train_dims")
    return xr.value, t0.value, sr.value


def field_input_backward(d_xin, t_row0, xyz, pts_per_ray, freqs, in_t, want_xyz, want_t):
    P, xin_rows = d_xin.shape
    n_rays = P // pts_per_ray
    d_xyz = torch.empty(P, 3, device=d_xin.device) if want_xyz else None
    d_t = torch.empty(n_rays, in_t, device=d_xin.device) if want_t else None
    f = [float(v) for v in freqs]
    arr = (C.c_float * max(len(f), 1))(*f)
    _check(load().nsff_field_input_backward(_ptr(d_xin), int(xin_rows), int(t_row0), _ptr(xyz), n_rays, int(pts_per_ray), arr,
                                            len(f), int(in_t), _ptr(d_xyz), _ptr(d_t), _stream()), "nsff_field_input_backward")
    return d_xyz, d_t


def _wgrad_jobs(jobs, with_off):
    return (WgradJob * len(jobs))(*[WgradJob(a=j[0], b=j[1], a_rows=j[2], b_rows=j[3], out_off=j[4] if with_off else 0, trunk=j[5],
                                             a_lo_delta=j[6] if len(j) > 6 else 0, b_lo_delta=j[7] if len(j) > 7 else 0) for j in jobs])


def weight_grad(jobs, n_tiles, n_splits, out, bias, gmax):
    arr = _wgrad_jobs(jobs, True)
    n = load().nsff_weight_grad_scratch(arr, len(jobs), int(n_tiles), int(n_splits))
    if n < 0:
        raise RuntimeError("nsff_weight_grad_scratch failed")
    scratch = torch.empty(n, device=out.device)
    _check(load().nsff_weight_grad(arr, len(jobs), int(n_tiles), int(n_splits), _ptr(scratch), _ptr(out), _ptr(bias),
                                   _ptr(gmax), _stream()), "nsff_weight_grad")


def weight_grad_accumulate(jobs, n_tiles, n_splits, grad_map, grad_base_ptr, gmax, aux=None):
    arr = _wgrad_jobs(jobs, False)
    n = load().nsff_weight_grad_scratch(arr, len(jobs), int(n_tiles), int(n_splits))
    if n < 0:
        raise RuntimeError("nsff_weight_grad_scratch failed")
    assert grad_map.dtype == torch.int32 and grad_map.is_contiguous() and grad_map.shape[1] == 4
    scratch = torch.empty(n, device=gmax.device)
    _check(load().nsff_weight_grad_accumulate_aux(arr, len(jobs), int(n_tiles), int(n_splits), _ptr(scratch),
                                                  C.c_void_p(grad_map.data_ptr()), grad_map.shape[0], C.c_void_p(grad_base_ptr),
                                                  _ptr(aux), _ptr(gmax), _stream()), "nsff_weight_grad_accumulate_aux")
    return scratch


def fold_grads(g, gb, w_final, b_final, head_rows, d_w_final, d_b_final):
    a = FoldGradArgs(n_rows=len(head_rows), g=_ptr(g), gb=_ptr(gb), w_final=_ptr(w_final), b_final=_ptr(b_final),
                     d_w_final=_ptr(d_w_final), d_b_final=_ptr(d_b_final))
    for r, (w, dw, db) in enumerate(head_rows):
        a.w_head[r], a.d_w_head[r], a.d_b_head[r] = w.data_ptr(), dw.data_ptr(), db.data_ptr()
    _check(load().nsff_fold_grads(C.byref(a), _stream()), "nsff_fold_grads")


def fold_grads_dense(g, gb, w_head, w_final, b_final, d_w_head, d_b_head, d_w_final, d_b_final, accumulate, g2=None, gb2=None):
    R = int(g.shape[0])
    for t in (g, g2, gb, gb2, w_final, b_final, d_w_final, d_b_final, d_b_head):
        assert t is None or (t.is_cuda and t.dtype == torch.float32 and t.is_contiguous())
    for t in (w_head, d_w_head):
        assert t.is_cuda and t.dtype == torch.float32 and t.shape[0] == R and t.shape[1] == 256 and t.stride(1) == 1
    a = FoldDenseArgs(n_rows=R, accumulate=1 if accumulate else 0, ld_head=int(w_head.stride(0)), ld_dhead=int(d_w_head.stride(0)),
                      g=g.data_ptr(), g2=None if g2 is None else g2.data_ptr(), gb=gb.data_ptr(), gb2=None if gb2 is None else gb2.data_ptr(),
                      w_head=w_head.data_ptr(), w_final=w_final.data_ptr(), b_final=b_final.data_ptr(), d_w_head=d_w_head.data_ptr(),
                      d_b_head=d_b_head.data_ptr(), d_w_final=d_w_final.data_ptr(), d_b_final=d_b_final.data_ptr())
    _check(load().nsff_fold_grads_dense(C.byref(a), _stream()), "nsff_fold_grads_dense")


def absmax(x):
    x = x.contiguous()
    if x.dim() == 2 and x.shape[1] == RAW_STRIDE:
        out = torch.empty(RAW_STRIDE, device=x.device, dtype=torch.float32)
        _check(load().nsff_absmax_raw(_ptr(x), x.shape[0], _ptr(out), _stream()), "nsff_absmax_raw")
        return out
    out = torch.empty((), device=x.device, dtype=torch.float32)
    _check(load().nsff_absmax(_ptr(x), x.numel(), _ptr(out), _stream()), "nsff_absmax")
    return out


def adam_step(param, grad, exp_avg, exp_avg_sq, state, lr, beta1, beta2, eps, weight_decay, seg_start=None, seg_used=None):
    if seg_start is None:
        _check(load().nsff_adam_step(_ptr(param), _ptr(grad), _ptr(exp_avg), _ptr(exp_avg_sq), param.numel(), _ptr(state), _ptr(lr),
                                     float(beta1), float(beta2), float(eps), float(weight_decay), _stream()), "nsff_adam_step")
        return
    _check(load().nsff_adam_step_segments(_ptr(param), _ptr(grad), _ptr(exp_avg), _ptr(exp_avg_sq), param.numel(), _ptr(state),
                                          _ptr(lr), float(beta1), float(beta2), float(eps), float(weight_decay),
                                          C.c_void_p(seg_start.data_ptr()), int(seg_used.numel()),
                                          C.c_void_p(seg_used.data_ptr()), _stream()),
           "nsff_adam_step_segments")


def _segments(seg_start, seg_used):
    if seg_start is None:
        return None, 0, None
    return C.c_void_p(seg_start.data_ptr()), int(seg_used.numel()), C.c_void_p(seg_used.data_ptr())


def sgd_step(param, grad, momentum_buf, state, lr, momentum, weight_decay, seg_start=None, seg_used=None):
    _check(load().nsff_sgd_step(_ptr(param), _ptr(grad), _ptr(momentum_buf), param.numel(), _ptr(state), _ptr(lr), float(momentum),
                                float(weight_decay), *_segments(seg_start, seg_used), _stream()), "nsff_sgd_step")


def radam_step(param, grad, exp_avg, exp_avg_sq, state, lr, beta1, beta2, eps, weight_decay, seg_start=None, seg_used=None):
    _check(load().nsff_radam_step(_ptr(param), _ptr(grad), _ptr(exp_avg), _ptr(exp_avg_sq), param.numel(), _ptr(state), _ptr(lr),
                                  float(beta1), float(beta2), float(eps), float(weight_decay), *_segments(seg_start, seg_used),
                                  _stream()), "nsff_radam_step")


def composite_backward(n_rays, n_samples, has_transient, flow_mode, noise_std, **tensors):
    a = CompositeBwdArgs(n_rays=int(n_rays), n_samples=int(n_samples), has_transient=int(has_transient),
                         flow_mode=int(flow_mode), noise_std=float(noise_std))
    for k, v in tensors.items():
        setattr(a, k, _ptr(v))
    _check(load().nsff_composite_backward(C.byref(a), _stream()), "nsff_composite_backward")


def flow_grad(zs, z_far, out, accumulate, col_a=-1, g_a=(), col_b=-1, g_b=()):
    a = FlowGradArgs(n_points=int(out.shape[0]), zs=_ptr(zs), z_far=float(z_far), accumulate=int(bool(accumulate)),
                     col_a=int(col_a), col_b=int(col_b), out=_ptr(out))
    if len(g_a) > 4 or len(g_b) > 4:
        raise ValueError("flow_grad: at most four cotangents per group")
    keep = [g.contiguous() for g in list(g_a) + list(g_b)]
    for i, g in enumerate(keep[:len(g_a)]):
        a.g_a[i] = _ptr(g)
    for i, g in enumerate(keep[len(g_a):]):
        a.g_b[i] = _ptr(g)
    _check(load().nsff_flow_grad(C.byref(a), _stream()), "nsff_flow_grad")


def nerfw_loss(mode, n_rays, n_samples, n_keep, n_frames, max_t, topk=1.0, thickness=1, work=None, **tensors):
    a = LossArgs(n_rays=int(n_rays), n_samples=int(n_samples), n_keep=int(n_keep), n_frames=int(n_frames), max_t=int(max_t),
                 topk=float(topk), thickness=int(thickness))
    for k, v in tensors.items():
        if v is None:
            continue
        if not torch.is_tensor(v):
            raise TypeError(f"nerfw_loss: {k} must be a tensor")
        if v.dtype == torch.int64:
            assert v.is_cuda and v.is_contiguous()
            setattr(a, k, v.data_ptr())
        else:
            setattr(a, k, _ptr(v))
    if work is None:
        _check(load().nsff_nerfw_loss(C.byref(a), int(mode), _stream()), "nsff_nerfw_loss")
        return
    if not (torch.is_tensor(work) and work.is_cuda and work.dtype == torch.uint8 and work.is_contiguous()):
        raise TypeError("nerfw_loss: work must be a contiguous uint8 GPU tensor")
    _check(load().nsff_nerfw_loss_ex(C.byref(a), int(mode), work.data_ptr(), work.numel(), _stream()), "nsff_nerfw_loss_ex")


LOSS_MAX_RAYS = 1 << 20


def nerfw_loss_work_bytes(n_rays):
    return int(load().nsff_nerfw_loss_work_bytes(int(n_rays)))


def last_loss_path():
    return int(load().nsff_last_loss_path())


def splat_work_bytes(H, W, S):
    return int(load().nsff_splat_work_bytes(int(H), int(W), int(S)))


def splat_planes(H, W, S, K4, P12, scale, xyz, flow, rgb, alpha, accum, work=None):
    a = SplatArgs(H=int(H), W=int(W), n_planes=int(S), scale=float(scale), xyz=_ptr(xyz), flow=_ptr(flow),
                  rgb=_ptr(rgb), alpha=_ptr(alpha), accum=_ptr(accum))
    if work is not None:
        assert work.is_cuda and work.is_contiguous() and work.dtype == torch.uint8
        a.work, a.work_bytes = work.data_ptr(), work.numel()
    a.K4[:] = [float(v) for v in K4]
    a.P[:] = [float(v) for v in P12]
    _check(load().nsff_splat_planes(C.byref(a), _stream()), "nsff_splat_planes")


def mpi_composite(H, W, S, dt, accum_fw, accum_bw, static_rgb, static_alpha, zs, rgb, depth):
    a = MpiArgs(H=int(H), W=int(W), n_planes=int(S), dt=float(dt), accum_fw=_ptr(accum_fw), accum_bw=_ptr(accum_bw),
                static_rgb=_ptr(static_rgb), static_alpha=_ptr(static_alpha), zs=_ptr(zs), rgb=_ptr(rgb),
                depth=_ptr(depth))
    _check(load().nsff_mpi_composite(C.byref(a), _stream()), "nsff_mpi_composite")


KERNEL_NAMES = {0: None, 1: "f32", 2: "h3_64", 3: "h3_8wave", 4: "h3a", 5: "h3_save", 7: "h3a_tb", 8: "h3a_side", 9: "h3a_save"}


def _dptr(t, dtype, what):
    if t is None:
        return None
    require_gpu_tensor(t, what)
    if t.dtype != dtype or not t.is_contiguous():
        raise RuntimeError(f"{what}: need a contiguous {dtype} tensor, got {t.dtype}"
                           f"{'' if t.is_contiguous() else ' (non-contiguous)'}")
    return t.data_ptr()


def ssim_scratch_bytes(n_frames, H, W):
    return int(load().nsff_ssim_scratch_bytes(int(n_frames), int(H), int(W)))


def ssim(gt, pred, mask=None, map=None, mean_map=None, sums=None, scratch=None):
    require_gpu_tensor(gt, "ssim: image_gt")
    require_gpu_tensor(pred, "ssim: image_pred")
    if gt.dim() != 4 or gt.shape[-1] != 3 or pred.shape != gt.shape:
        raise RuntimeError(f"ssim: need (F, H, W, 3) image pairs of one shape, got {tuple(gt.shape)} and {tuple(pred.shape)}")
    F, H, W = (int(v) for v in gt.shape[:3])
    if mask is not None and mask.dtype == torch.bool:
        mask = mask.view(torch.uint8)
    if sums is not None and scratch is None:
        scratch = torch.zeros(max(ssim_scratch_bytes(F, H, W), 16), dtype=torch.uint8, device=gt.device)
    a = SsimArgs(n_frames=F, H=H, W=W, window=11, gt=_dptr(gt, torch.float32, "ssim: image_gt"),
                 pred=_dptr(pred, torch.float32, "ssim: image_pred"), mask=_dptr(mask, torch.uint8, "ssim: mask"),
                 map=_dptr(map, torch.float32, "ssim: map"), mean_map=_dptr(mean_map, torch.float32, "ssim: mean_map"),
                 sums=_dptr(sums, torch.float64, "ssim: sums"), scratch=_dptr(scratch, torch.uint8, "ssim: scratch"),
                 scratch_bytes=0 if scratch is None else scratch.numel())
    for t, n in ((mask, F * H * W), (map, F * H * W * 3), (mean_map, F * H * W), (sums, F * 3)):
        if t is not None and t.numel() != n:
            raise RuntimeError(f"ssim: an output / mask has {t.numel()} elements, expected {n}")
    with torch.cuda.device(gt.device):
        _check(load().nsff_ssim(C.byref(a), _stream()), "nsff_ssim")


# ... 516 lines not shown
```

### nsff_pl_amd/csrc/rays.hip

```cpp
#include <hip/hip_runtime.h>
#include <cstdlib>
#include "nsff_common.h"

namespace {

constexpr int WAVES_PER_BLOCK = 4;
constexpr int RS = NSFF_RAW_STRIDE;

__device__ __forceinline__ float wave_sum(float v) {
#pragma unroll
    for (int off = 32; off > 0; off >>= 1) v += __shfl_xor(v, off);
    return v;
}

__device__ __forceinline__ float wave_scan_mul(float v, int lane) {
#pragma unroll
    for (int off = 1; off < 64; off <<= 1) {
        const float u = __shfl_up(v, off);
        if (lane >= off) v *= u;
    }
    return v;
}
__device__ __forceinline__ float wave_scan_add(float v, int lane) {
#pragma unroll
    for (int off = 1; off < 64; off <<= 1) {
        const float u = __shfl_up(v, off);
        if (lane >= off) v += u;
    }
    return v;
}

__device__ __forceinline__ float softplus(float x) { return x > 20.f ? x : log1pf(expf(x)); }

__global__ void coarse_samples_kernel(const float* __restrict__ rays, long long n_rays,
                                      const float* __restrict__ z_lin, int S, float perturb,
                                      const float* __restrict__ rnd, float* __restrict__ zs,
                                      float* __restrict__ xyz) {
    const long long idx = (long long)blockIdx.x * blockDim.x + threadIdx.x;
    if (idx >= n_rays * S) return;
    const long long n = idx / S;
    const int i = (int)(idx - n * S);
    float z = z_lin[i];
    if (perturb > 0.f) {
        const float lower = i > 0 ? 0.5f * (z_lin[i - 1] + z_lin[i]) : z_lin[0];
        const float upper = i < S - 1 ? 0.5f * (z_lin[i] + z_lin[i + 1]) : z_lin[S - 1];
        z = lower + (upper - lower) * (perturb * rnd[idx]);
    }
    zs[idx] = z;
    const float* r = rays + n * 6;
#pragma unroll
    for (int c = 0; c < 3; ++c) xyz[idx * 3 + c] = r[c] + r[3 + c] * z;
}

__device__ __forceinline__ void sample_pdf_ray(const float* w, const float* bins, int M, float eps,
                                               const float* u, int n_imp, float* cdf,
                                               float* out_a, float* out_b, int lane, bool active) {
    float part = 0.f;
    for (int j = lane; j < M; j += 64) part += (active ? w[j] : 0.f) + eps;
    const float total = wave_sum(part);
    float carry = 0.f;
    if (lane == 0) cdf[0] = 0.f;
    for (int base = 0; base < M; base += 64) {
        const int j = base + lane;
        const float pdf = j < M ? ((active ? w[j] : 0.f) + eps) / total : 0.f;
        const float inc = wave_scan_add(pdf, lane) + carry;
        if (j < M) cdf[j + 1] = inc;
        carry = __shfl(inc, 63);
    }
    __syncthreads();
    for (int k = lane; k < n_imp; k += 64) {
        const float uk = active ? u[k] : 0.f;
        int lo = 0, hi = M + 1;
        while (lo < hi) {
            const int mid = (lo + hi) >> 1;
            if (cdf[mid] <= uk) lo = mid + 1; else hi = mid;
        }
        const int below = max(lo - 1, 0), above = min(lo, M);
        const float cb = cdf[below], ca = cdf[above];
        const float bb = bins[below], ba = bins[above];
        float denom = ca - cb;
        if (denom < eps) denom = 1.f;
        const float s = bb + (uk - cb) / denom * (ba - bb);
        if (active) {
            if (out_a) out_a[k] = s;
            if (out_b) out_b[k] = s;
        }
    }
    __syncthreads();
}

struct FineArgs {
    const float* rays; long long n_rays; const float* z_lin; const float* zs_coarse;
    int S, n_imp;
    const float* w_static; const float* w_transient;
    const float* u_static; const float* u_transient; int u_per_ray;
    float* samples_static; float* samples_transient;
    float* zs_fine; float* xyz_fine;
};

__global__ __launch_bounds__(64 * WAVES_PER_BLOCK) void fine_samples_kernel(const FineArgs a) {
    extern __shared__ __attribute__((aligned(16))) float smem[];
    const int lane = threadIdx.x & 63, wave = threadIdx.x >> 6, tid = threadIdx.x;
    constexpr int T = 64 * WAVES_PER_BLOCK;
    const long long ray = blockIdx.x;
    const int S = a.S, n_imp = a.n_imp;
    const int k_sets = a.w_transient ? 2 : 1;
    const int Sf = S + k_sets * n_imp;
    float* cdf = smem + wave * S;
    float* bins = smem + WAVES_PER_BLOCK * S;
    float* merged = bins + ((S + 3) & ~3);
    for (int j = tid; j < S - 1; j += T) bins[j] = 0.5f * (a.z_lin[j] + a.z_lin[j + 1]);
    for (int j = tid; j < S; j += T) merged[j] = a.zs_coarse[ray * S + j];
    __syncthreads();
    {
        const bool mine = wave < k_sets;
        const int set = mine ? wave : 0;
        const float* w = (set == 0 ? a.w_static : a.w_transient) + ray * S + 1;
        const float* ub = set == 0 ? a.u_static : a.u_transient;
        const float* u = a.u_per_ray ? ub + ray * n_imp : ub;
        float* keep = set == 0 ? a.samples_static : a.samples_transient;
        sample_pdf_ray(w, bins, S - 2, 1e-5f, u, n_imp, cdf, merged + S + set * n_imp,
                       keep ? keep + ray * n_imp : nullptr, lane, mine);
    }
    const float* r = a.rays + ray * 6;
    const float o0 = r[0], o1 = r[1], o2 = r[2], d0 = r[3], d1 = r[4], d2 = r[5];
    for (int i = tid; i < Sf; i += T) {
        const float v = merged[i];
        int rank = 0;
        int j = 0;
        for (; j + 4 <= Sf; j += 4) {
            const float4 o = *reinterpret_cast<const float4*>(merged + j);
            rank += (o.x < v || (o.x == v && j < i)) ? 1 : 0;
            rank += (o.y < v || (o.y == v && j + 1 < i)) ? 1 : 0;
            rank += (o.z < v || (o.z == v && j + 2 < i)) ? 1 : 0;
            rank += (o.w < v || (o.w == v && j + 3 < i)) ? 1 : 0;
        }
        for (; j < Sf; ++j) {
            const float o = merged[j];
            rank += (o < v || (o == v && j < i)) ? 1 : 0;
        }
        const long long dst = ray * Sf + rank;
        a.zs_fine[dst] = v;
        a.xyz_fine[dst * 3 + 0] = o0 + d0 * v;
        a.xyz_fine[dst * 3 + 1] = o1 + d1 * v;
        a.xyz_fine[dst * 3 + 2] = o2 + d2 * v;
    }
}

struct PdfArgs {
    const float* bins; const float* weights; long long n_rays; int M;
    const float* u; int n_imp; int u_per_ray; float eps; float* samples;
};

__global__ __launch_bounds__(64 * WAVES_PER_BLOCK) void sample_pdf_kernel(const PdfArgs a) {
    extern __shared__ __attribute__((aligned(16))) float smem[];
    const int lane = threadIdx.x & 63, wave = threadIdx.x >> 6;
    const long long ray_raw = (long long)blockIdx.x * WAVES_PER_BLOCK + wave;
    const bool active = ray_raw < a.n_rays;
    const long long ray = active ? ray_raw : a.n_rays - 1;
    float* cdf = smem + wave * (a.M + 1);
    const float* u = a.u_per_ray ? a.u + ray * a.n_imp : a.u;
    sample_pdf_ray(a.weights + ray * a.M, a.bins + ray * (a.M + 1), a.M, a.eps, u, a.n_imp, cdf,
                   active ? a.samples + ray * a.n_imp : nullptr, nullptr, lane, true);
}

struct FrameRayArgs {
    float fx, fy, cx, cy;
    float c2w[12];
    int W;
    float near, shift_near;
    long long first, count;
    float* rays;
};

__device__ __forceinline__ void ndc_pixel_ray(float fx, float fy, float cx, float cy, const float* c2w, float near,
                                              float shift_near, float i, float j, float* r) {
    const float dc[3] = {(i - cx) / fx, -(j - cy) / fy, -1.0f};
    float d[3];
#pragma unroll
    for (int k = 0; k < 3; ++k) d[k] = dc[0] * c2w[4 * k + 0] + dc[1] * c2w[4 * k + 1] + dc[2] * c2w[4 * k + 2];
    const float nrm = sqrtf(d[0] * d[0] + d[1] * d[1] + d[2] * d[2]);
#pragma unroll
    for (int k = 0; k < 3; ++k) d[k] /= nrm;
    float o[3] = {c2w[3], c2w[7], c2w[11]};
    const float t = -(shift_near + o[2]) / d[2];
#pragma unroll
    for (int k = 0; k < 3; ++k) o[k] = o[k] + t * d[k];
    const float ox_oz = o[0] / o[2], oy_oz = o[1] / o[2];
    const float sx = -1.0f / (cx / fx), sy = -1.0f / (cy / fy);
    const float o2 = 1.0f + 2.0f * near / o[2];
    r[0] = sx * ox_oz;
    r[1] = sy * oy_oz;
    r[2] = o2;
    r[3] = sx * (d[0] / d[2] - ox_oz);
    r[4] = sy * (d[1] / d[2] - oy_oz);
    r[5] = 1.0f - o2;
}

__global__ void frame_rays_kernel(const FrameRayArgs a) {
    const long long idx = (long long)blockIdx.x * blockDim.x + threadIdx.x;
    if (idx >= a.count) return;
    float r[6];
    const long long pix = a.first + idx;
    ndc_pixel_ray(a.fx, a.fy, a.cx, a.cy, a.c2w, a.near, a.shift_near, (float)(pix % a.W), (float)(pix / a.W), r);
    float* out = a.rays + idx * 6;
#pragma unroll
    for (int k = 0; k < 6; ++k) out[k] = r[k];
}

constexpr int REC_THREADS = 256;

__global__ __launch_bounds__(REC_THREADS) void ray_records_kernel(const NsffRayRecordArgs a) {
    const long long n = (long long)a.H * a.W;
    const long long pix = (long long)blockIdx.x * REC_THREADS + threadIdx.x;
    const int frame = a.first_frame + (int)blockIdx.y;
    float4 q[4] = {};
    if (pix < n) {
        const float* tab = a.frame_table + (long long)frame * NSFF_FRAME_TABLE;
        const unsigned row = (unsigned)pix / (unsigned)a.W, col = (unsigned)pix - row * (unsigned)a.W;
        const float u = (float)col, v = (float)row;
        float r[6];
        ndc_pixel_ray(a.fx, a.fy, a.cx, a.cy, tab, a.near, tab[12], u, v, r);
        const long long p = (long long)frame * n + pix;
        float rgb[3];
        if (a.image_u8) {
            const uint8_t* s = static_cast<const uint8_t*>(a.images) + p * 3;
#pragma unroll
            for (int c = 0; c < 3; ++c) rgb[c] = (float)s[c] / 255.0f;
        } else {
            const float* s = static_cast<const float*>(a.images) + p * 3;
#pragma unroll
            for (int c = 0; c < 3; ++c) rgb[c] = s[c];
        }
        const float mask = a.mask_u8 ? (float)static_cast<const uint8_t*>(a.masks)[p] / 255.0f
                                     : static_cast<const float*>(a.masks)[p];
        float2 fw = {0.f, 0.f}, bw = {0.f, 0.f};
        if (a.flow_fw && frame < a.n_frames - 1) fw = reinterpret_cast<const float2*>(a.flow_fw)[p];
        if (a.flow_bw && frame > 0) bw = reinterpret_cast<const float2*>(a.flow_bw)[p];
        q[0] = make_float4(r[0], r[1], r[2], r[3]);
        q[1] = make_float4(r[4], r[5], rgb[0], rgb[1]);
        q[2] = make_float4(rgb[2], (float)frame, a.disps[p], mask);
        q[3] = make_float4(u + fw.x, v + fw.y, u + bw.x, v + bw.y);
    }
    float4* out = reinterpret_cast<float4*>(a.records) + (long long)frame * n * 4;
    __shared__ float4 s_rec[REC_THREADS * 4];
    const int lane = threadIdx.x & 63, wave = threadIdx.x >> 6;
    float4* sw = s_rec + wave * 256;
#pragma unroll
    for (int k = 0; k < 4; ++k) sw[lane * 4 + (k ^ ((lane >> 2) & 3))] = q[k];
    __syncthreads();
    const long long pix0 = (long long)blockIdx.x * REC_THREADS + wave * 64;
#pragma unroll
    for (int k = 0; k < 4; ++k) {
        const int rec = k * 16 + (lane >> 2), c = lane & 3;
        if (pix0 + rec < n) out[(pix0 + rec) * 4 + c] = sw[rec * 4 + (c ^ ((rec >> 2) & 3))];
    }
}

__global__ void warp_points_kernel(const float* __restrict__ raw, const float* __restrict__ xyz,
                                   const float* __restrict__ zs, long long n_points, float z_far,
                                   float* __restrict__ xyz_fw, float* __restrict__ xyz_bw) {
    const long long idx = (long long)blockIdx.x * blockDim.x + threadIdx.x;
    if (idx >= n_points * 3) return;
    const long long p = idx / 3;
    const int c = (int)(idx - p * 3);
    const bool far = zs[p] > z_far;
    const float x = xyz[idx];
    xyz_fw[idx] = x + (far ? 0.f : raw[p * RS + 8 + c]);
    xyz_bw[idx] = x + (far ? 0.f : raw[p * RS + 11 + c]);
}

__device__ __forceinline__ float frustum_count(const NsffFrustumArgs& v, float x, float y, float z) {
    const float fx = v.K4[0], fy = v.K4[1], cx = v.K4[2], cy = v.K4[3];
    const float rz = 2.0f / (z - 1.0f - 1e-6f);
    const float rx = -rz * x * cx / fx;
    const float ry = -rz * y * cy / fy;
    const long long frame = v.ts[0];
    float count = 0.f;
    if (frame < 0 || frame >= v.n_frames) return count;
    for (int c = 0; c < v.n_cams; ++c) {
        const float* m = v.w2c + ((long long)c * v.n_frames + frame) * 12;
        const float cam0 = fmaf(m[2], rz, fmaf(m[1], ry, m[0] * rx)) + m[3];
        const float cam1 = fmaf(m[6], rz, fmaf(m[5], ry, m[4] * rx)) + m[7];
        const float cam2 = fmaf(m[10], rz, fmaf(m[9], ry, m[8] * rx)) + m[11];
        if (!(cam2 < 0.f)) continue;
        const float c1 = -cam1, c2 = -cam2;
        const float u = fmaf(cx, c2, fx * cam0) / c2, w = fmaf(cy, c2, fy * c1) / c2;
        if (u >= 0.f && u < (float)v.W && w >= 0.f && w < (float)v.H) count += 1.f;
    }
    return count;
}

__global__ __launch_bounds__(256) void frustum_visibility_kernel(const NsffFrustumArgs v, const float* __restrict__ xyz,
                                                                 long long n_points, float* __restrict__ out) {
    const long long p = (long long)blockIdx.x * 256 + threadIdx.x;
    if (p < n_points) out[p] = frustum_count(v, xyz[3 * p], xyz[3 * p + 1], xyz[3 * p + 2]);
}

__global__ __launch_bounds__(64 * WAVES_PER_BLOCK) void composite_kernel(const NsffCompositeArgs a) {
    const int lane = threadIdx.x & 63;
    const long long ray = (long long)blockIdx.x * WAVES_PER_BLOCK + (threadIdx.x >> 6);
    if (ray >= a.n_rays) return;
    const int S = a.n_samples;
    const bool tr = a.has_transient != 0;
    const bool flows = tr && a.flow_mode >= 1;
    const bool warps = tr && a.flow_mode >= 2;

    float cT = 1.f, cTs = 1.f, cTfw = 1.f, cTbw = 1.f;
    float s_depth = 0.f, s_rgb[3] = {0, 0, 0}, s_talpha = 0.f, s_trgb[3] = {0, 0, 0};
    float s_sorgb[3] = {0, 0, 0}, s_sodepth = 0.f;
    float s_xyz[3] = {0, 0, 0}, s_ffw[3] = {0, 0, 0}, s_fbw[3] = {0, 0, 0};
    float s_rgbfw[3] = {0, 0, 0}, s_rgbbw[3] = {0, 0, 0}, s_occfw = 0.f, s_occbw = 0.f;

    for (int base = 0; base < S; base += 64) {
        const int i = base + lane;
        const bool on = i < S;
        const long long idx = ray * S + (on ? i : S - 1);
        const float z = a.zs[idx];
        const bool last = i >= S - 1;
        const float dz = last ? 0.f : a.zs[idx + 1] - z;
        const float d_s = last ? 100.f : dz;
        const float d_t = last ? 1e-3f : dz;
        const float* rec = a.raw + idx * RS;

        float sig_s = rec[3];
        if (a.noise_static) sig_s += a.noise_static[idx] * a.noise_std;
        sig_s = softplus(sig_s);
        const float al_s = 1.f - expf(-d_s * sig_s);
        float rgb_s[3] = {0, 0, 0};
        if (a.has_rgb) { rgb_s[0] = rec[0]; rgb_s[1] = rec[1]; rgb_s[2] = rec[2]; }

        float sig_t = 0.f, al_t = 0.f, alpha = al_s;
        float rgb_t[3] = {0, 0, 0};
        if (tr) {
            sig_t = rec[7];
            if (a.visibility && a.visibility[idx] == 0.f) sig_t = -10.f;
            if (a.vis.w2c && frustum_count(a.vis, a.xyz[idx * 3], a.xyz[idx * 3 + 1], a.xyz[idx * 3 + 2]) == 0.f) sig_t = -10.f;
            if (a.noise_transient) sig_t += a.noise_transient[idx] * a.noise_std;
            sig_t = softplus(sig_t);
            al_t = 1.f - expf(-d_t * sig_t);
            alpha = 1.f - (1.f - al_s) * (1.f - al_t);
            if (a.has_rgb) { rgb_t[0] = rec[4]; rgb_t[1] = rec[5]; rgb_t[2] = rec[6]; }
        }
        const float om = on ? 1.f - alpha : 1.f;
        const float inc = wave_scan_mul(om, lane);
        float exc = __shfl_up(inc, 1);
        if (lane == 0) exc = 1.f;
        const float T = cT * exc;
        cT *= __shfl(inc, 63);
        const float w = alpha * T, w_s = al_s * T, w_t = al_t * T;

        if (on) {
            if (a.static_sigmas) a.static_sigmas[idx] = sig_s;
            if (a.has_rgb && a.static_rgbs) {
                a.static_rgbs[idx * 3 + 0] = rgb_s[0]; a.static_rgbs[idx * 3 + 1] = rgb_s[1];
                a.static_rgbs[idx * 3 + 2] = rgb_s[2];
            }
            if (tr) {
                if (a.transient_sigmas) a.transient_sigmas[idx] = sig_t;
                if (a.has_rgb && a.transient_rgbs) {
                    a.transient_rgbs[idx * 3 + 0] = rgb_t[0]; a.transient_rgbs[idx * 3 + 1] = rgb_t[1];
                    a.transient_rgbs[idx * 3 + 2] = rgb_t[2];
                }
                if (a.static_alphas) a.static_alphas[idx] = al_s;
                if (a.transient_alphas) a.transient_alphas[idx] = al_t;
                if (a.static_weights) a.static_weights[idx] = w_s;
                if (a.transient_weights) a.transient_weights[idx] = w_t;
                if (a.weights) a.weights[idx] = w;
            } else {
                if (a.static_weights) a.static_weights[idx] = w;
                if (a.weights) a.weights[idx] = w;
            }
        }
        if (!a.has_rgb) continue;

        if (on) {
            s_depth += w * z;
            if (tr) {
#pragma unroll
                for (int c = 0; c < 3; ++c) { s_rgb[c] += w_s * rgb_s[c]; s_trgb[c] += w_t * rgb_t[c]; }
                s_talpha += w_t;
            } else {
#pragma unroll
                for (int c = 0; c < 3; ++c) s_rgb[c] += w * rgb_s[c];
            }
        }
        if (!tr) continue;

        {
            const float oms = on ? 1.f - al_s : 1.f;
            const float incs = wave_scan_mul(oms, lane);
            float excs = __shfl_up(incs, 1);
            if (lane == 0) excs = 1.f;
            const float Ts = cTs * excs;
            cTs *= __shfl(incs, 63);
            const float wso = al_s * Ts;
            if (on) {
#pragma unroll
                for (int c = 0; c < 3; ++c) s_sorgb[c] += wso * rgb_s[c];
                s_sodepth += wso * z;
            }
        }
        if (!flows) continue;

        const bool far = z > a.z_far;
        float ffw[3], fbw[3], x[3];
#pragma unroll
        for (int c = 0; c < 3; ++c) {
            ffw[c] = far ? 0.f : rec[8 + c];
            fbw[c] = far ? 0.f : rec[11 + c];
            x[c] = a.xyz[idx * 3 + c];
        }
        if (on) {
#pragma unroll
            for (int c = 0; c < 3; ++c) {
                if (a.flows_fw) a.flows_fw[idx * 3 + c] = ffw[c];
                if (a.flows_bw) a.flows_bw[idx * 3 + c] = fbw[c];
                s_xyz[c] += w * x[c]; s_ffw[c] += w * ffw[c]; s_fbw[c] += w * fbw[c];
            }
        }
        if (!warps) continue;

#pragma unroll
        for (int dir = 0; dir < 2; ++dir) {
            const float* recw = (dir == 0 ? a.raw_fw : a.raw_bw) + idx * RS;
            const float* nz = dir == 0 ? a.noise_fw : a.noise_bw;
            float sg = recw[7];
            if (nz) sg += nz[idx] * a.noise_std;
            const float al_tw = 1.f - expf(-d_t * softplus(sg));
            const float al_w = 1.f - (1.f - al_s) * (1.f - al_tw);
            const float omw = on ? 1.f - al_w : 1.f;
            const float incw = wave_scan_mul(omw, lane);
            float excw = __shfl_up(incw, 1);
            if (lane == 0) excw = 1.f;
            float& cw = dir == 0 ? cTfw : cTbw;
            const float Tw = cw * excw;
            cw *= __shfl(incw, 63);
            const float ws_w = al_s * Tw, wt_w = al_tw * Tw;
            if (on) {
                float* srgb = dir == 0 ? s_rgbfw : s_rgbbw;
#pragma unroll
                for (int c = 0; c < 3; ++c) srgb[c] += ws_w * rgb_s[c] + wt_w * recw[4 + c];
                const float* xw = (dir == 0 ? a.xyz_fw : a.xyz_bw) + idx * 3;
                float* cyc = dir == 0 ? a.xyzs_fw_bw : a.xyzs_bw_fw;
                const int head = dir == 0 ? 11 : 8;
                if (cyc) {
#pragma unroll
                    for (int c = 0; c < 3; ++c) cyc[idx * 3 + c] = xw[c] + (far ? 0.f : recw[head + c]);
                }
                const float occ = wt_w - w_t;
                if (dir == 0) { s_occfw += occ; if (a.disoccs_fw) a.disoccs_fw[idx] = 1.f - fabsf(occ); }
                else          { s_occbw += occ; if (a.disoccs_bw) a.disoccs_bw[idx] = 1.f - fabsf(occ); }
            }
        }
    }
    if (!a.has_rgb) return;

    s_depth = wave_sum(s_depth);
#pragma unroll
    for (int c = 0; c < 3; ++c) s_rgb[c] = wave_sum(s_rgb[c]);
    if (tr) {
        s_talpha = wave_sum(s_talpha); s_sodepth = wave_sum(s_sodepth);
#pragma unroll
        for (int c = 0; c < 3; ++c) { s_trgb[c] = wave_sum(s_trgb[c]); s_sorgb[c] = wave_sum(s_sorgb[c]); }
    }
    if (flows) {
#pragma unroll
        for (int c = 0; c < 3; ++c) { s_xyz[c] = wave_sum(s_xyz[c]); s_ffw[c] = wave_sum(s_ffw[c]); s_fbw[c] = wave_sum(s_fbw[c]); }
    }
    if (warps) {
        s_occfw = wave_sum(s_occfw); s_occbw = wave_sum(s_occbw);
#pragma unroll
        for (int c = 0; c < 3; ++c) { s_rgbfw[c] = wave_sum(s_rgbfw[c]); s_rgbbw[c] = wave_sum(s_rgbbw[c]); }
    }
    if (lane != 0) return;
    if (a.depth) a.depth[ray] = s_depth;
    if (!tr) {
        if (a.rgb) for (int c = 0; c < 3; ++c) a.rgb[ray * 3 + c] = s_rgb[c];
        return;
    }
    for (int c = 0; c < 3; ++c) {
        if (a.rgb) a.rgb[ray * 3 + c] = s_rgb[c] + s_trgb[c];
        if (a.transient_rgb) a.transient_rgb[ray * 3 + c] = s_trgb[c] + 0.8f * (1.f - s_talpha);
        if (a.static_only_rgb) a.static_only_rgb[ray * 3 + c] = s_sorgb[c];
    }
    if (a.transient_alpha) a.transient_alpha[ray] = s_talpha;
    if (a.static_only_depth) a.static_only_depth[ray] = s_sodepth;
    if (flows) {
        for (int c = 0; c < 3; ++c) {
            if (a.xyz_exp) a.xyz_exp[ray * 3 + c] = s_xyz[c];
            if (a.flow_fw_exp) a.flow_fw_exp[ray * 3 + c] = s_ffw[c];
            if (a.flow_bw_exp) a.flow_bw_exp[ray * 3 + c] = s_fbw[c];
            if (a.xyz_fw_exp) a.xyz_fw_exp[ray * 3 + c] = s_xyz[c] + s_ffw[c];
            if (a.xyz_bw_exp) a.xyz_bw_exp[ray * 3 + c] = s_xyz[c] + s_fbw[c];
        }
    }
    if (warps) {
        for (int c = 0; c < 3; ++c) {
            if (a.rgb_fw) a.rgb_fw[ray * 3 + c] = s_rgbfw[c];
            if (a.rgb_bw) a.rgb_bw[ray * 3 + c] = s_rgbbw[c];
        }
        if (a.disocc_fw) a.disocc_fw[ray] = 1.f - fabsf(s_occfw);
        if (a.disocc_bw) a.disocc_bw[ray] = 1.f - fabsf(s_occbw);
    }
}

template <int NCH>
__global__ __launch_bounds__(64 * NCH) void composite_kernel_chunks(const NsffCompositeArgs a) {
    __shared__ float tot[NCH][4];
    __shared__ float part[NCH][32];
    const int lane = threadIdx.x & 63, c = threadIdx.x >> 6;
    const long long ray = blockIdx.x;
    const int S = a.n_samples;
    const bool tr = a.has_transient != 0;
    const bool flows = tr && a.flow_mode >= 1;
    const bool warps = tr && a.flow_mode >= 2;

    const int i = 64 * c + lane;
    const bool on = i < S;
    const long long idx = ray * S + (on ? i : S - 1);
    const float z = a.zs[idx];
    const bool last = i >= S - 1;
    const float dz = last ? 0.f : a.zs[idx + 1] - z;
    const float d_s = last ? 100.f : dz;
    const float d_t = last ? 1e-3f : dz;
    const float* rec = a.raw + idx * RS;

    float sig_s = rec[3];
    if (a.noise_static) sig_s += a.noise_static[idx] * a.noise_std;
    sig_s = softplus(sig_s);
    const float al_s = 1.f - expf(-d_s * sig_s);
    float rgb_s[3] = {0, 0, 0};
    if (a.has_rgb) { rgb_s[0] = rec[0]; rgb_s[1] = rec[1]; rgb_s[2] = rec[2]; }

    float sig_t = 0.f, al_t = 0.f, alpha = al_s;
    float rgb_t[3] = {0, 0, 0};
    if (tr) {
        sig_t = rec[7];
        if (a.visibility && a.visibility[idx] == 0.f) sig_t = -10.f;
        if (a.vis.w2c && frustum_count(a.vis, a.xyz[idx * 3], a.xyz[idx * 3 + 1], a.xyz[idx * 3 + 2]) == 0.f) sig_t = -10.f;
        if (a.noise_transient) sig_t += a.noise_transient[idx] * a.noise_std;
        sig_t = softplus(sig_t);
        al_t = 1.f - expf(-d_t * sig_t);
        alpha = 1.f - (1.f - al_s) * (1.f - al_t);
        if (a.has_rgb) { rgb_t[0] = rec[4]; rgb_t[1] = rec[5]; rgb_t[2] = rec[6]; }
    }
    const float inc = wave_scan_mul(on ? 1.f - alpha : 1.f, lane);
    float incs = 1.f, incw[2] = {1.f, 1.f}, al_tw[2] = {0.f, 0.f};
    if (a.has_rgb && tr) incs = wave_scan_mul(on ? 1.f - al_s : 1.f, lane);
    if (a.has_rgb && warps) {
#pragma unroll
        for (int dir = 0; dir < 2; ++dir) {
            const float* recw = (dir == 0 ? a.raw_fw : a.raw_bw) + idx * RS;
            const float* nz = dir == 0 ? a.noise_fw : a.noise_bw;
            float sg = recw[7];
            if (nz) sg += nz[idx] * a.noise_std;
            al_tw[dir] = 1.f - expf(-d_t * softplus(sg));
            const float al_w = 1.f - (1.f - al_s) * (1.f - al_tw[dir]);
            incw[dir] = wave_scan_mul(on ? 1.f - al_w : 1.f, lane);
        }
    }
    if (lane == 63) { tot[c][0] = inc; tot[c][1] = incs; tot[c][2] = incw[0]; tot[c][3] = incw[1]; }
    __syncthreads();
    float cT = 1.f, cTs = 1.f, cTw[2] = {1.f, 1.f};
    for (int cc = 0; cc < c; ++cc) { cT *= tot[cc][0]; cTs *= tot[cc][1]; cTw[0] *= tot[cc][2]; cTw[1] *= tot[cc][3]; }

    float exc = __shfl_up(inc, 1);
    if (lane == 0) exc = 1.f;
    const float T = cT * exc;
    const float w = alpha * T, w_s = al_s * T, w_t = al_t * T;
    if (on) {
        if (a.static_sigmas) a.static_sigmas[idx] = sig_s;
        if (a.has_rgb && a.static_rgbs) {
            a.static_rgbs[idx * 3 + 0] = rgb_s[0]; a.static_rgbs[idx * 3 + 1] = rgb_s[1];
            a.static_rgbs[idx * 3 + 2] = rgb_s[2];
        }
        if (tr) {
            if (a.transient_sigmas) a.transient_sigmas[idx] = sig_t;
            if (a.has_rgb && a.transient_rgbs) {
                a.transient_rgbs[idx * 3 + 0] = rgb_t[0]; a.transient_rgbs[idx * 3 + 1] = rgb_t[1];
                a.transient_rgbs[idx * 3 + 2] = rgb_t[2];
            }
            if (a.static_alphas) a.static_alphas[idx] = al_s;
            if (a.transient_alphas) a.transient_alphas[idx] = al_t;
            if (a.static_weights) a.static_weights[idx] = w_s;
            if (a.transient_weights) a.transient_weights[idx] = w_t;
            if (a.weights) a.weights[idx] = w;
        } else {
            if (a.static_weights) a.static_weights[idx] = w;
            if (a.weights) a.weights[idx] = w;
        }
    }
    if (!a.has_rgb) return;

    enum { P_DEPTH, P_RGB, P_TRGB = P_RGB + 3, P_TALPHA = P_TRGB + 3, P_SORGB, P_SODEPTH = P_SORGB + 3, P_XYZ, P_FFW = P_XYZ + 3,
           P_FBW = P_FFW + 3, P_RGBFW = P_FBW + 3, P_RGBBW = P_RGBFW + 3, P_OCCFW = P_RGBBW + 3, P_OCCBW, P_N };
    static_assert(P_N <= 32, "part[] columns");
    float p[P_N];
#pragma unroll
    for (int k = 0; k < P_N; ++k) p[k] = 0.f;
    if (on) {
        p[P_DEPTH] = w * z;
        if (tr) {
#pragma unroll
            for (int k = 0; k < 3; ++k) { p[P_RGB + k] = w_s * rgb_s[k]; p[P_TRGB + k] = w_t * rgb_t[k]; }
            p[P_TALPHA] = w_t;
        } else {
#pragma unroll
            for (int k = 0; k < 3; ++k) p[P_RGB + k] = w * rgb_s[k];
        }
    }
    if (tr) {
        float excs = __shfl_up(incs, 1);
        if (lane == 0) excs = 1.f;
        const float wso = al_s * (cTs * excs);
        if (on) {
#pragma unroll
            for (int k = 0; k < 3; ++k) p[P_SORGB + k] = wso * rgb_s[k];
            p[P_SODEPTH] = wso * z;
        }
    }
    if (flows) {
        const bool far = z > a.z_far;
        float ffw[3], fbw[3], x[3];
#pragma unroll
        for (int k = 0; k < 3; ++k) {
            ffw[k] = far ? 0.f : rec[8 + k];
            fbw[k] = far ? 0.f : rec[11 + k];
            x[k] = a.xyz[idx * 3 + k];
        }
        if (on) {
#pragma unroll
            for (int k = 0; k < 3; ++k) {
                if (a.flows_fw) a.flows_fw[idx * 3 + k] = ffw[k];
                if (a.flows_bw) a.flows_bw[idx * 3 + k] = fbw[k];
                p[P_XYZ + k] = w * x[k]; p[P_FFW + k] = w * ffw[k]; p[P_FBW + k] = w * fbw[k];
            }
        }
        if (warps) {
#pragma unroll
            for (int dir = 0; dir < 2; ++dir) {
                const float* recw = (dir == 0 ? a.raw_fw : a.raw_bw) + idx * RS;
                float excw = __shfl_up(incw[dir], 1);
                if (lane == 0) excw = 1.f;
                const float Tw = cTw[dir] * excw;
                const float ws_w = al_s * Tw, wt_w = al_tw[dir] * Tw;
                if (on) {
#pragma unroll
                    for (int k = 0; k < 3; ++k) p[(dir == 0 ? P_RGBFW : P_RGBBW) + k] = ws_w * rgb_s[k] + wt_w * recw[4 + k];
                    const float* xw = (dir == 0 ? a.xyz_fw : a.xyz_bw) + idx * 3;
                    float* cyc = dir == 0 ? a.xyzs_fw_bw : a.xyzs_bw_fw;
                    const int head = dir == 0 ? 11 : 8;
                    if (cyc) {
#pragma unroll
                        for (int k = 0; k < 3; ++k) cyc[idx * 3 + k] = xw[k] + (far ? 0.f : recw[head + k]);
                    }
                    const float occ = wt_w - w_t;
                    if (dir == 0) { p[P_OCCFW] = occ; if (a.disoccs_fw) a.disoccs_fw[idx] = 1.f - fabsf(occ); }
                    else          { p[P_OCCBW] = occ; if (a.disoccs_bw) a.disoccs_bw[idx] = 1.f - fabsf(occ); }
                }
            }
        }
    }
    const int n_used = warps ? (int)P_N : (flows ? (int)P_RGBFW : (tr ? (int)P_XYZ : (int)P_TRGB));
#pragma unroll
    for (int k = 0; k < P_N; ++k) {
        if (k < n_used) {
            const float v = wave_sum(p[k]);
            if (lane == 0) part[c][k] = v;
        }
    }
    __syncthreads();
    if (threadIdx.x != 0) return;
    float s[P_N];
#pragma unroll
    for (int k = 0; k < P_N; ++k) {
        s[k] = 0.f;
        if (k < n_used) for (int cc = 0; cc < NCH; ++cc) s[k] += part[cc][k];
    }
    if (a.depth) a.depth[ray] = s[P_DEPTH];
    if (!tr) {
        if (a.rgb) for (int k = 0; k < 3; ++k) a.rgb[ray * 3 + k] = s[P_RGB + k];
        return;
    }
    for (int k = 0; k < 3; ++k) {
        if (a.rgb) a.rgb[ray * 3 + k] = s[P_RGB + k] + s[P_TRGB + k];
        if (a.transient_rgb) a.transient_rgb[ray * 3 + k] = s[P_TRGB + k] + 0.8f * (1.f - s[P_TALPHA]);
        if (a.static_only_rgb) a.static_only_rgb[ray * 3 + k] = s[P_SORGB + k];
    }
    if (a.transient_alpha) a.transient_alpha[ray] = s[P_TALPHA];
    if (a.static_only_depth) a.static_only_depth[ray] = s[P_SODEPTH];
    if (flows) {
        for (int k = 0; k < 3; ++k) {
            if (a.xyz_exp) a.xyz_exp[ray * 3 + k] = s[P_XYZ + k];
            if (a.flow_fw_exp) a.flow_fw_exp[ray * 3 + k] = s[P_FFW + k];
            if (a.flow_bw_exp) a.flow_bw_exp[ray * 3 + k] = s[P_FBW + k];
            if (a.xyz_fw_exp) a.xyz_fw_exp[ray * 3 + k] = s[P_XYZ + k] + s[P_FFW + k];
            if (a.xyz_bw_exp) a.xyz_bw_exp[ray * 3 + k] = s[P_XYZ + k] + s[P_FBW + k];
        }
    }
    if (warps) {
        for (int k = 0; k < 3; ++k) {
            if (a.rgb_fw) a.rgb_fw[ray * 3 + k] = s[P_RGBFW + k];
            if (a.rgb_bw) a.rgb_bw[ray * 3 + k] = s[P_RGBBW + k];
        }
        if (a.disocc_fw) a.disocc_fw[ray] = 1.f - fabsf(s[P_OCCFW]);
        if (a.disocc_bw) a.disocc_bw[ray] = 1.f - fabsf(s[P_OCCBW]);
    }
}

__global__ __launch_bounds__(256) void time_rows_kernel(const float* __restrict__ table, long long n_table, int width,
                                                         const long long* __restrict__ ts, long long n, long long max_t,
                                                         float* __restrict__ next, float* __restrict__ prev, int vec) {
    const int per_row = vec ? width / 4 : width;
    const long long i = (long long)blockIdx.x * 256 + threadIdx.x;
    if (i >= n * per_row) return;
    const long long r = i / per_row;
    const int c = (int)(i - r * per_row);
    const long long t = ts[r];
    long long tn = t + 1 < max_t ? t + 1 : max_t, tp = t - 1 > 0 ? t - 1 : 0;
    tn = tn < 0 ? 0 : (tn > n_table - 1 ? n_table - 1 : tn);
    tp = tp > n_table - 1 ? n_table - 1 : tp;
    if (vec) {
        if (next) reinterpret_cast<float4*>(next)[i] = reinterpret_cast<const float4*>(table + tn * width)[c];
        if (prev) reinterpret_cast<float4*>(prev)[i] = reinterpret_cast<const float4*>(table + tp * width)[c];
    } else {
        if (next) next[i] = table[tn * width + c];
        if (prev) prev[i] = table[tp * width + c];
    }
}

constexpr int TRB_CHUNK = 2048;
constexpr int TRB_COLS = 4;
__global__ __launch_bounds__(256) void time_rows_bwd_kernel(const float* __restrict__ g_cur, const float* __restrict__ g_next,
                                                             const float* __restrict__ g_prev, const long long* __restrict__ ts,
                                                             long long n, long long max_t, long long n_table, int width,
                                                             float* __restrict__ d_table) {
    __shared__ int sList[3][TRB_CHUNK];
    __shared__ int sTs[TRB_CHUNK];
    __shared__ int sCnt[3];
    __shared__ float sPart[4][64];
    const long long r = blockIdx.x;
    const int lane = threadIdx.x & 63, part = threadIdx.x >> 6;
    const float* gs[3] = {g_cur, g_next, g_prev};
    for (int cg = 0; cg < width; cg += 64 * TRB_COLS) {
        float acc[TRB_COLS];
#pragma unroll
        for (int j = 0; j < TRB_COLS; ++j) acc[j] = 0.f;
        for (long long base = 0; base < n; base += TRB_CHUNK) {
            const long long end = base + TRB_CHUNK < n ? base + TRB_CHUNK : n;
            for (long long i = base + threadIdx.x; i < end; i += 256) {
                const long long t = ts[i];
                sTs[i - base] = (int)(t < -2 ? -2 : (t > 0x7ffffff0LL ? 0x7ffffff0LL : t));
            }
            __syncthreads();
            if (part == 0) {
                int cnt[3] = {0, 0, 0};
                for (long long i0 = base; i0 < end; i0 += 64) {
                    const long long i = i0 + lane;
                    bool hit[3] = {false, false, false};
                    if (i < end) {
                        const long long t = sTs[i - base];
                        long long tn = t + 1 < max_t ? t + 1 : max_t, tp = t - 1 > 0 ? t - 1 : 0;
                        tn = tn < 0 ? 0 : (tn > n_table - 1 ? n_table - 1 : tn);
                        tp = tp > n_table - 1 ? n_table - 1 : tp;
                        hit[0] = t == r; hit[1] = tn == r; hit[2] = tp == r;
                    }
#pragma unroll
                    for (int l = 0; l < 3; ++l) {
                        const unsigned long long m = __ballot(hit[l] && gs[l] != nullptr);
                        if (hit[l] && gs[l] != nullptr) sList[l][cnt[l] + __popcll(m & ((1ull << lane) - 1ull))] = (int)(i - base);
                        cnt[l] += __popcll(m);
                    }
                }
                if (lane == 0) { sCnt[0] = cnt[0]; sCnt[1] = cnt[1]; sCnt[2] = cnt[2]; }
            }
            __syncthreads();
#pragma unroll
            for (int l = 0; l < 3; ++l) {
                const float* __restrict__ g = gs[l];
                const int cnt = sCnt[l];
                for (int k0 = part; k0 < cnt; k0 += 16) {
                    float v[4][TRB_COLS];
#pragma unroll
                    for (int u = 0; u < 4; ++u) {
                        const int k = k0 + 4 * u;
                        const float* row = g + (base + sList[l][k < cnt ? k : k0]) * width + cg + lane;
#pragma unroll
                        for (int j = 0; j < TRB_COLS; ++j)
                            v[u][j] = (k < cnt && cg + 64 * j + lane < width) ? row[64 * j] : 0.f;
                    }
#pragma unroll
                    for (int u = 0; u < 4; ++u)
#pragma unroll
                        for (int j = 0; j < TRB_COLS; ++j) acc[j] += v[u][j];
                }
            }
            __syncthreads();
        }
#pragma unroll
        for (int j = 0; j < TRB_COLS; ++j) {
            const int c = cg + 64 * j + lane;
            if (cg + 64 * j >= width) break;
            sPart[part][lane] = acc[j];
            __syncthreads();
            if (part == 0 && c < width) d_table[r * width + c] = (sPart[0][lane] + sPart[1][lane]) + (sPart[2][lane] + sPart[3][lane]);
            __syncthreads();
        }
    }
}

}

extern "C" {

int nsff_time_rows_backward(const float* g_cur, const float* g_next, const float* g_prev, const int64_t* ts, int64_t n,
                            int64_t max_t, int64_t n_table, int32_t width, float* d_table, void* stream) {
    if (n < 0 || n_table < 1 || n_table > 0x7fffffffLL || width < 1) return NSFF_ERR_INVALID;
    if (!d_table || (n > 0 && !ts)) return NSFF_ERR_NULL;
    hipLaunchKernelGGL(time_rows_bwd_kernel, dim3((unsigned)n_table), dim3(256), 0, (hipStream_t)stream, g_cur, g_next, g_prev,
                       reinterpret_cast<const long long*>(ts), (long long)n, (long long)max_t, (long long)n_table, (int)width,
                       d_table);
    return nsff_launch_status();
}

int nsff_time_rows(const float* table, int64_t n_table, int32_t width, const int64_t* ts, int64_t n, int64_t max_t,
                   float* next, float* prev, void* stream) {
    if (n < 0 || n_table < 1 || width < 1) return NSFF_ERR_INVALID;
    if (n == 0 || (!next && !prev)) return NSFF_OK;
    if (!table || !ts) return NSFF_ERR_NULL;
    const int vec = (width % 4 == 0) && !(((uintptr_t)table | (uintptr_t)next | (uintptr_t)prev) & 15);
    const long long total = n * (vec ? width / 4 : width);
    hipLaunchKernelGGL(time_rows_kernel, dim3((unsigned)((total + 255) / 256)), dim3(256), 0, (hipStream_t)stream, table,
                       (long long)n_table, (int)width, reinterpret_cast<const long long*>(ts), (long long)n, (long long)max_t,
                       next, prev, vec);
    return nsff_launch_status();
}


int nsff_coarse_samples(const float* rays, int64_t n_rays, const float* z_lin, int32_t n_samples,
                        float perturb, const float* perturb_rand, float* zs, float* xyz, void* stream) {
    if (n_rays < 0 || n_samples < 1) return NSFF_ERR_INVALID;
    if (n_rays == 0) return NSFF_OK;
    if (!rays || !z_lin || !zs || !xyz) return NSFF_ERR_NULL;
    if (perturb > 0.f && !perturb_rand) return NSFF_ERR_NULL;
    const long long total = (long long)n_rays * n_samples;
    hipLaunchKernelGGL(coarse_samples_kernel, dim3((unsigned)((total + 255) / 256)), dim3(256), 0,
                       (hipStream_t)stream, rays, (long long)n_rays, z_lin, n_samples, perturb,
                       perturb_rand, zs, xyz);
    return nsff_launch_status();
}

int nsff_fine_samples(const float* rays, int64_t n_rays, const float* z_lin, const float* zs_coarse,
                      int32_t n_samples, int32_t n_importance,
                      const float* weights_static, const float* weights_transient,
                      const float* u_static, const float* u_transient, int32_t u_per_ray,
                      float* samples_static, float* samples_transient,
                      float* zs_fine, float* xyz_fine, void* stream) {
    if (n_rays < 0 || n_samples < 3 || n_importance < 1) return NSFF_ERR_INVALID;
    if (n_rays == 0) return NSFF_OK;
    if (!rays || !z_lin || !zs_coarse || !weights_static || !u_static || !zs_fine || !xyz_fine) return NSFF_ERR_NULL;
    if (weights_transient && !u_transient) return NSFF_ERR_NULL;
    FineArgs a{rays, (long long)n_rays, z_lin, zs_coarse, n_samples, n_importance,
               weights_static, weights_transient, u_static, u_transient, u_per_ray,
               samples_static, samples_transient, zs_fine, xyz_fine};
    const int Sf = n_samples + (weights_transient ? 2 : 1) * n_importance;
    const size_t lds = (size_t)(WAVES_PER_BLOCK * n_samples + ((n_samples + 3) & ~3) + Sf) * sizeof(float);
    if (lds > 64 * 1024 || n_rays > 0x7fffffffLL) return NSFF_ERR_INVALID;
    const unsigned blocks = (unsigned)n_rays;
    hipLaunchKernelGGL(fine_samples_kernel, dim3(blocks), dim3(64 * WAVES_PER_BLOCK), lds,
                       (hipStream_t)stream, a);
    return nsff_launch_status();
}

int nsff_sample_pdf(const float* bins, const float* weights, int64_t n_rays, int32_t n_bins_minus1,
                    const float* u, int32_t n_importance, int32_t u_per_ray, float eps,
                    float* samples, void* stream) {
    if (n_rays < 0 || n_bins_minus1 < 1 || n_importance < 1) return NSFF_ERR_INVALID;
    if (n_rays == 0) return NSFF_OK;
    if (!bins || !weights || !u || !samples) return NSFF_ERR_NULL;
    PdfArgs a{bins, weights, (long long)n_rays, n_bins_minus1, u, n_importance, u_per_ray, eps, samples};
    const size_t lds = (size_t)WAVES_PER_BLOCK * (n_bins_minus1 + 1) * sizeof(float);
    if (lds > 64 * 1024) return NSFF_ERR_INVALID;
    const unsigned blocks = (unsigned)((n_rays + WAVES_PER_BLOCK - 1) / WAVES_PER_BLOCK);
    hipLaunchKernelGGL(sample_pdf_kernel, dim3(blocks), dim3(64 * WAVES_PER_BLOCK), lds,
                       (hipStream_t)stream, a);
    return nsff_launch_status();
}

int nsff_warp_points(const float* raw, const float* xyz, const float* zs, int64_t n_points,
                     float z_far, float* xyz_fw, float* xyz_bw, void* stream) {
    if (n_points < 0) return NSFF_ERR_INVALID;
    if (n_points == 0) return NSFF_OK;
    if (!raw || !xyz || !zs || !xyz_fw || !xyz_bw) return NSFF_ERR_NULL;
    const long long total = (long long)n_points * 3;
    hipLaunchKernelGGL(warp_points_kernel, dim3((unsigned)((total + 255) / 256)), dim3(256), 0,
                       (hipStream_t)stream, raw, xyz, zs, (long long)n_points, z_far, xyz_fw, xyz_bw);
    return nsff_launch_status();
}

int nsff_frame_rays(const float* K4_host, const float* c2w_host, int32_t H, int32_t W, float near, float shift_near,
                    int64_t first_pixel, int64_t n_pixels, float* rays, void* stream) {
    if (!K4_host || !c2w_host) return NSFF_ERR_NULL;
    if (H < 1 || W < 1 || first_pixel < 0 || n_pixels < 0 || first_pixel + n_pixels > (int64_t)H * W) return NSFF_ERR_INVALID;
    if (n_pixels == 0) return NSFF_OK;
    if (!rays) return NSFF_ERR_NULL;
    FrameRayArgs a{};
    a.fx = K4_host[0]; a.fy = K4_host[1]; a.cx = K4_host[2]; a.cy = K4_host[3];
    for (int i = 0; i < 12; ++i) a.c2w[i] = c2w_host[i];
    a.W = W; a.near = near; a.shift_near = shift_near; a.first = first_pixel; a.count = n_pixels; a.rays = rays;
    hipLaunchKernelGGL(frame_rays_kernel, dim3((unsigned)((n_pixels + 255) / 256)), dim3(256), 0, (hipStream_t)stream, a);
    return nsff_launch_status();
}

int nsff_ray_records(const NsffRayRecordArgs* args, void* stream) {
    if (!args) return NSFF_ERR_NULL;
    const NsffRayRecordArgs& a = *args;
    if (a.n_frames < 0 || a.H < 1 || a.W < 1 || a.n_pixels != (int64_t)a.H * a.W) return NSFF_ERR_INVALID;
    if (a.first_frame < 0 || a.frame_count < 0 || (int64_t)a.first_frame + a.frame_count > a.n_frames) return NSFF_ERR_INVALID;
    if (a.frame_count > 65535 || a.n_pixels > 0x7fffffffLL) return NSFF_ERR_INVALID;
    if (a.frame_count == 0) return NSFF_OK;
    if (!a.images || !a.disps || !a.masks || !a.frame_table || !a.records) return NSFF_ERR_NULL;
    if (((uintptr_t)a.records & 15) || (((uintptr_t)a.flow_fw | (uintptr_t)a.flow_bw) & 7) ||
        (((uintptr_t)a.disps | (uintptr_t)a.frame_table) & 3) || (!a.image_u8 && ((uintptr_t)a.images & 3)) ||
        (!a.mask_u8 && ((uintptr_t)a.masks & 3)))
        return NSFF_ERR_ALIGN;
    const dim3 grid((unsigned)((a.n_pixels + REC_THREADS - 1) / REC_THREADS), (unsigned)a.frame_count);
    hipLaunchKernelGGL(ray_records_kernel, grid, dim3(REC_THREADS), 0, (hipStream_t)stream, a);
    return nsff_launch_status();
}

int nsff_composite(const NsffCompositeArgs* args, void* stream) {
    if (!args) return NSFF_ERR_NULL;
    const NsffCompositeArgs& a = *args;
    if (a.n_rays < 0 || a.n_samples < 1 || a.flow_mode < 0 || a.flow_mode > 2) return NSFF_ERR_INVALID;
    if (a.n_rays == 0) return NSFF_OK;
    if (!a.raw || !a.zs) return NSFF_ERR_NULL;
    if (a.flow_mode && (!a.has_transient || !a.has_rgb)) return NSFF_ERR_INVALID;
    if (a.flow_mode >= 1 && !a.xyz) return NSFF_ERR_NULL;
    if (a.flow_mode == 2 && (!a.raw_fw || !a.raw_bw || !a.xyz_fw || !a.xyz_bw)) return NSFF_ERR_NULL;
    if (a.vis.w2c && (!a.vis.ts || !a.xyz)) return NSFF_ERR_NULL;
    if (a.vis.w2c && (a.vis.n_cams < 1 || a.vis.n_frames < 1)) return NSFF_ERR_INVALID;
    const int nch = (a.n_samples + 63) / 64;
    if (nch >= 2 && nch <= 4 && a.n_rays <= 0x7fffffffLL && getenv("NSFF_SERIAL_COMPOSITE") == nullptr) {
        const dim3 grid((unsigned)a.n_rays);
        if (nch == 2) hipLaunchKernelGGL(composite_kernel_chunks<2>, grid, dim3(128), 0, (hipStream_t)stream, a);
        else if (nch == 3) hipLaunchKernelGGL(composite_kernel_chunks<3>, grid, dim3(192), 0, (hipStream_t)stream, a);
        else hipLaunchKernelGGL(composite_kernel_chunks<4>, grid, dim3(256), 0, (hipStream_t)stream, a);
        return nsff_launch_status();
    }
    const unsigned blocks = (unsigned)((a.n_rays + WAVES_PER_BLOCK - 1) / WAVES_PER_BLOCK);
    hipLaunchKernelGGL(composite_kernel, dim3(blocks), dim3(64 * WAVES_PER_BLOCK), 0,
                       (hipStream_t)stream, a);
    return nsff_launch_status();
}

int nsff_frustum_visibility(const NsffFrustumArgs* vis, const float* xyz, int64_t n_points, float* vis_count,
                            void* stream) {
    if (!vis || !vis->w2c || !vis->ts) return NSFF_ERR_NULL;
    if (n_points < 0 || vis->n_cams < 1 || vis->n_frames < 1) return NSFF_ERR_INVALID;
    if (n_points == 0) return NSFF_OK;
    if (!xyz || !vis_count) return NSFF_ERR_NULL;
    const long long blocks = (n_points + 255) / 256;
    if (blocks > 0x7fffffffLL) return NSFF_ERR_INVALID;
    hipLaunchKernelGGL(frustum_visibility_kernel, dim3((unsigned)blocks), dim3(256), 0, (hipStream_t)stream, *vis, xyz,
                       (long long)n_points, vis_count);
    return nsff_launch_status();
}

}
```

### nsff_pl_amd/graphs.py

```python
import os

import torch

from . import _lib, config
from .rendering import render_rays


class GraphedRender:
    def __init__(self, models, embeddings, max_t, N_samples=64, perturb=0, noise_std=0, N_importance=0, chunk=1024 * 32,
                 test_time=False, **kwargs):
        for k in ("view_dir", "t_embedded", "a_embedded"):
            if kwargs.get(k) is not None:
                raise ValueError(f"GraphedRender: per-ray keyword tensor '{k}' is not supported (static shapes only)")
        self.models, self.embeddings = models, embeddings
        self.args = (max_t, N_samples, perturb, noise_std, N_importance, chunk)
        self.test_time, self.kwargs = bool(test_time), dict(kwargs)
        self._graphs = {}

    def _param_addresses(self):
        mods = list(self.models.values()) + [m for m in self.embeddings.values() if isinstance(m, torch.nn.Module)]
        return tuple(p.data_ptr() for m in mods for p in m.parameters())

    def _refresh_packs(self):
        prec = config.PRECISIONS[config.get_precision()]
        for m in self.models.values():
            m.packed(prec)
            if prec == config.PRECISIONS["f16x3"] and m._pack_cache.built(_lib.REPACKED):
                m.packed(_lib.REPACKED)

    def _capture(self, key, rays, ts):
        dev = rays.device
        s_rays = rays.detach().clone().contiguous().float()
        s_ts = None if ts is None else ts.detach().clone()

        def call():
            with torch.no_grad():
                return render_rays(self.models, self.embeddings, s_rays, s_ts, *self.args, test_time=self.test_time, **self.kwargs)
        side = torch.cuda.Stream(device=dev)
        side.wait_stream(torch.cuda.current_stream(dev))
        with torch.cuda.stream(side):
            call()
            call()
        torch.cuda.current_stream(dev).wait_stream(side)
        graph = torch.cuda.CUDAGraph()
        with torch.cuda.graph(graph):
            results = call()
        self._graphs[key] = (graph, s_rays, s_ts, results)
        return self._graphs[key]

    def __call__(self, rays, ts=None):
        if not rays.is_cuda:
            raise RuntimeError("GraphedRender needs GPU tensors (there is no CPU path)")
        shape_key = (int(rays.shape[0]), ts is not None, config.get_precision(), config.get_tile_points(), config.get_persistent(),
                     os.environ.get("NSFF_H3A_SHAPE", ""))
        key = shape_key + (self._param_addresses(),)
        entry = self._graphs.get(key)
        if entry is None:
            for stale in [k for k in self._graphs if k[:-1] == shape_key]:
                del self._graphs[stale]
            entry = self._capture(key, rays, ts)
        graph, s_rays, s_ts, results = entry
        s_rays.copy_(rays)
        if s_ts is not None:
            s_ts.copy_(ts)
        self._refresh_packs()
        graph.replay()
        return results
```

### nsff_pl_amd/rendering.py

```python
import os

import torch

from . import _lib
from . import autograd
from . import config
from . import range_check
from . import field_grad
from . import ray_geometry

Z_FAR = 0.95

def _new(ref, *shape):
    return torch.empty(*shape, device=ref.device, dtype=torch.float32)


def sample_pdf(bins, weights, N_importance, det=False, eps=1e-5):
    _lib.require_gpu_tensor(bins, "sample_pdf bins")
    bins = bins.contiguous().float()
    weights = weights.contiguous().float()
    n_rays = weights.shape[0]
    if det:
        u = torch.linspace(0, 1, N_importance, device=bins.device)
    else:
        u = torch.rand(n_rays, N_importance, device=bins.device)
    out = _new(bins, n_rays, N_importance)
    if n_rays:
        _lib.sample_pdf(bins, weights, u.contiguous(), 0 if det else 1, eps, out)
    return out


_TORCH_RAND, _TORCH_RANDN = torch.rand, torch.randn


class _Draws:

    def __init__(self, device, n_rays, N_samples, N_importance, perturb, noise_std, test_time, models, kwargs, coarse=None):
        self.device = device
        self.coarse_done = False
        self.fused = (device.type == "cuda" and torch.rand is _TORCH_RAND and torch.randn is _TORCH_RANDN
                      and not os.environ.get("NSFF_TORCH_RNG") and not torch.cuda.is_current_stream_capturing()
                      and _lib.fused_draws_match_torch(device))
        self.at = 0
        if not self.fused:
            return
        first = models["coarse"] if N_importance > 0 else models["fine"]
        transient = bool(kwargs.get("output_transient", True) and first.encode_transient)
        flows = kwargs.get("output_transient_flow", []) if transient else []
        noisy = float(noise_std) != 0
        plan, need = [], []

        def add(kind, need_values, *shape):
            plan.append((kind, shape))
            need.append(bool(need_values))
        hook = None
        if perturb > 0:
            add("rand", coarse is None, n_rays, N_samples)
            if coarse is not None and n_rays:
                hook = (coarse[0], coarse[1], float(perturb), coarse[2], coarse[3])
        S = N_samples
        if N_importance > 0:
            add("randn", noisy, n_rays, S)
            if transient:
                add("randn", noisy, n_rays, S)
            if perturb != 0:
                add("rand", True, n_rays, N_importance)
                if transient:
                    add("rand", True, n_rays, N_importance)
            S = N_samples + (2 if transient else 1) * N_importance
        add("randn", noisy, n_rays, S)
        if transient:
            add("randn", noisy, n_rays, S)
            if flows and not test_time:
                add("randn", noisy, n_rays, S)
                add("randn", noisy, n_rays, S)
        self.plan = plan
        self.values = _lib.fused_draws(plan, device, need, coarse=hook)
        self.coarse_done = hook is not None

    def take(self, kind, *shape):
        if not self.fused:
            return (torch.rand if kind == "rand" else torch.randn)(*shape, device=self.device)
        if self.at >= len(self.plan) or self.plan[self.at] != (kind, shape):
            raise RuntimeError(f"draw {self.at}: {kind}{shape} is not the planned {self.plan[self.at:self.at + 1]}")
        self.at += 1
        return self.values[self.at - 1]


class _Pass:
    __slots__ = ("embeddings", "rays", "ts", "max_t", "noise_std", "test_time", "kwargs",
                 "freqs_xyz", "dir_embedded", "n_rays", "rec", "tbias", "neighbour_rows", "draws")


def _embed_rows(embeddings, key, idx):
    return embeddings[key](idx).detach().contiguous().float()


_LINSPACE = {}


def _unit_linspace(n, device):
    key = (int(n), str(device))
    if key not in _LINSPACE:
        if len(_LINSPACE) > 64:
            _LINSPACE.clear()
        _LINSPACE[key] = torch.linspace(0, 1, n, device=device)
    return _LINSPACE[key]


def _neighbour_time_rows(embeddings, ts, max_t):
    m = embeddings['t']
    if (isinstance(m, torch.nn.Embedding) and m.padding_idx is None and m.max_norm is None and m.weight.is_cuda
            and m.weight.dtype == torch.float32 and m.weight.is_contiguous() and ts.is_cuda and ts.dtype == torch.int64):
        return _lib.time_rows(m.weight.detach(), ts.contiguous(), max_t)
    return (_embed_rows(embeddings, 't', torch.clamp(ts + 1, max=max_t)),
            _embed_rows(embeddings, 't', torch.clamp(ts - 1, min=0)))


def _time_codes(ctx, models, kwargs, N_samples, N_importance, output_transient, flows):
    ctx.tbias, ctx.neighbour_rows = {}, None
    if not output_transient:
        return None
    n_rays, ts, m = ctx.n_rays, ctx.ts, ctx.embeddings.get('t')
    override = kwargs.get('t_embedded') if 't_embedded' in kwargs else None
    plan = []
    if not (ctx.rec is not None or n_rays == 0 or config.get_precision() != "f16x3" or config.get_tile_points() not in (0, 130)):
        passes = [('coarse', N_samples), ('fine', N_samples + 2 * N_importance)] if N_importance > 0 else [('fine', N_samples)]
        for typ, S in passes:
            model = models[typ]
            if not model.encode_transient or S % 64 or (n_rays * S < 32768 and config.get_tile_points() == 0):
                continue
            if model.in_channels_t > 64 or model.in_channels_t % 4:
                continue
            if typ == 'fine' and flows and not ctx.test_time and hasattr(model, "transient_flow_fw"):
                plan += [(typ, 'fw', model, 1), (typ, 'bw', model, -1)]
            plan.append((typ, 't', model, 0))
    plain = (override is None and isinstance(m, torch.nn.Embedding) and m.padding_idx is None and m.max_norm is None
             and m.weight.is_cuda and m.weight.dtype == torch.float32 and m.weight.is_contiguous()
             and torch.is_tensor(ts) and ts.is_cuda and ts.dtype == torch.int64
             and ts.dim() == 1 and ts.shape[0] == n_rays)
    if (plan and plain and all(mod.in_channels_t == m.weight.shape[1] for _, _, mod, _ in plan)
            and not os.environ.get('NSFF_NO_TIME_INDEX')):
        outs, rows = _lib.time_bias([(mod, d) for _, _, mod, d in plan], index=(m.weight.detach(), ts.contiguous(), ctx.max_t))
        for (typ, which, _, _), out in zip(plan, outs):
            ctx.tbias[(typ, which)] = out
        if 1 in rows:
            ctx.neighbour_rows = (rows[1], rows[-1])
        return rows[0]
    t_embedded = override if override is not None else ctx.embeddings['t'](ts)
    t_embedded = t_embedded.detach().contiguous().float()
    plan = [p for p in plan if t_embedded.shape == (n_rays, p[2].in_channels_t)]
    if plan:
        if any(w == 'fw' for _, w, _, _ in plan):
            ctx.neighbour_rows = _neighbour_time_rows(ctx.embeddings, ts, ctx.max_t)
        src = {0: t_embedded, 1: ctx.neighbour_rows[0] if ctx.neighbour_rows else None, -1: ctx.neighbour_rows[1] if ctx.neighbour_rows else None}
        for (typ, which, _, _), out in zip(plan, _lib.time_bias([(mod, src[d]) for _, _, mod, d in plan])):
            ctx.tbias[(typ, which)] = out
    return t_embedded


def _inference(results, ctx, model, xyz, zs, output_transient, output_transient_flow,
               t_embedded, a_embedded):
    typ = model.typ
    n_rays, S = zs.shape
    test_time = ctx.test_time
    results[f'zs_{typ}'] = zs
    results[f'xyzs_{typ}'] = xyz
    P = n_rays * S
    sigma_only = typ == 'coarse' and test_time
    want_flow = bool(output_transient_flow) and output_transient and not sigma_only
    warps = want_flow and not test_time
    disocc = warps and 'disocc' in output_transient_flow
    if want_flow and not hasattr(model, "transient_flow_fw"):
        raise AttributeError(f"{typ} model has no flow heads")

    raw = _new(zs, P, _lib.RAW_STRIDE)
    side = dict(dir_emb=ctx.dir_embedded if model.use_viewdir and not sigma_only else None,
                a_emb=a_embedded if (model.use_viewdir and model.in_channels_a > 0 and not sigma_only) else None)
    big_enough = ctx.rec is not None or config.get_tile_points() == 130 or (config.get_tile_points() == 0 and P >= 32768)
    if (side["dir_emb"] is not None and P and S % 64 == 0 and config.get_precision() == "f16x3" and config.get_tile_points() in (0, 130)
            and big_enough and not os.environ.get('NSFF_NO_SIDE_BIAS')):
        side["s_bias"] = _lib.side_bias(model, side["dir_emb"], side["a_emb"])

    def query(tag, raw_out, pts, static_mode, transient_mode, flow_heads, t_rows, which='t', **extra):
        saves = {}
        if ctx.rec is not None and field_grad.forward_can_save(model, static_mode, transient_mode):
            x3 = config.grad_x3()
            acts, xin, masks, side_rows = field_grad.alloc_saves(model, P, zs.device, bool(transient_mode), bool(static_mode), x3)
            saves = dict(save_acts=acts, save_xin=xin, save_masks=masks, save_side=side_rows, save_lo=x3)
            ctx.rec.setdefault("saved", {})[tag] = (raw_out, acts, xin, masks, pts.view(-1, 3), side_rows, x3)
        t_bias = ctx.tbias.get((typ, which)) if (transient_mode and not saves) else None
        _lib.field_query(model, raw_out, P, S, static_mode=static_mode, transient_mode=transient_mode,
                         flow_heads=flow_heads, xyz=pts, freqs=ctx.freqs_xyz, t_emb=t_rows, t_bias=t_bias, **saves, **extra)
    if P:
        query(typ, raw, xyz, 1 if sigma_only else 2, 0 if not output_transient else (1 if sigma_only else 2),
              2 if want_flow else 0, t_embedded if output_transient else None, **side)

    vis = None
    if test_time and output_transient and 'dataset' in ctx.kwargs and P:
        vis = ray_geometry.frustum_args(ctx.kwargs['dataset'], ctx.ts, zs.device)

    nstd = float(ctx.noise_std)
    noise_s = ctx.draws.take("randn", n_rays, S)
    noise_t = ctx.draws.take("randn", n_rays, S) if output_transient else None
    if ctx.rec is not None and nstd != 0:
        ctx.rec[f"{typ}_static"], ctx.rec[f"{typ}_transient"] = noise_s, noise_t

    args = dict(n_rays=n_rays, n_samples=S, has_transient=int(output_transient),
                has_rgb=int(not sigma_only), flow_mode=0, want_disocc=int(disocc),
                noise_std=nstd, z_far=Z_FAR, raw=raw, zs=zs, xyz=xyz, vis=vis,
                noise_static=noise_s if nstd != 0 else None,
                noise_transient=noise_t if (nstd != 0 and output_transient) else None)

    def out(key, *shape):
        t = _new(zs, *shape)
        results[key] = t
        return t

    if not sigma_only:
        args['static_rgbs'] = out(f'static_rgbs_{typ}', n_rays, S, 3)
        if output_transient:
            args['transient_rgbs'] = out(f'transient_rgbs_{typ}', n_rays, S, 3)
            if want_flow:
                args['flows_fw'] = out('transient_flows_fw', n_rays, S, 3)
                args['flows_bw'] = out('transient_flows_bw', n_rays, S, 3)
    args['static_sigmas'] = out(f'static_sigmas_{typ}', n_rays, S)
    if output_transient:
        args['transient_sigmas'] = out(f'transient_sigmas_{typ}', n_rays, S)

    if warps:
        ts = ctx.ts
        xyz_w = _new(zs, 2, n_rays, S, 3)
        xyz_fw, xyz_bw = xyz_w[0], xyz_w[1]
        results['xyzs_fw'] = xyz_fw
        raw_w = _new(zs, 2 * P, _lib.RAW_STRIDE)
        raw_fw, raw_bw = raw_w[:P], raw_w[P:]
        tp1, tm1 = ctx.neighbour_rows if ctx.neighbour_rows is not None else _neighbour_time_rows(ctx.embeddings, ts, ctx.max_t)
        tb_fw, tb_bw = ctx.tbias.get((typ, 'fw')), ctx.tbias.get((typ, 'bw'))
        def halves(a, b):
            return (a.untyped_storage().data_ptr() == b.untyped_storage().data_ptr()
                    and a.data_ptr() + a.numel() * 4 == b.data_ptr())
        merged = (ctx.rec is None and P > 0 and not os.environ.get('NSFF_NO_MERGED_REQUERY') and halves(tp1, tm1)
                  and (tb_fw is None) == (tb_bw is None) and (tb_fw is None or halves(tb_fw, tb_bw)))
        if P:
            _lib.warp_points(raw, xyz, zs, Z_FAR, xyz_fw, xyz_bw)
            if merged:
                ctx.tbias[(typ, 'fwbw')] = None if tb_fw is None else torch.as_strided(tb_fw, (2 * n_rays,) + tuple(tb_fw.shape[1:]),
                                                                                         tb_fw.stride())
                _lib.field_query(model, raw_w, 2 * P, S, static_mode=0, transient_mode=2, flow_heads=1, xyz=xyz_w,
                                 freqs=ctx.freqs_xyz, t_emb=torch.as_strided(tp1, (2 * n_rays, tp1.shape[1]), tp1.stride()),
                                 t_bias=ctx.tbias[(typ, 'fwbw')])
            else:
                query(f"{typ}_warp_fw", raw_fw, xyz_fw, 0, 2, 1, tp1, which='fw')
        noise_fw = ctx.draws.take("randn", n_rays, S)
        out('rgb_fw', n_rays, 3)
        results['xyzs_bw'] = xyz_bw
        if P and not merged:
            query(f"{typ}_warp_bw", raw_bw, xyz_bw, 0, 2, 1, tm1, which='bw')
        noise_bw = ctx.draws.take("randn", n_rays, S)
        if ctx.rec is not None and nstd != 0:
            ctx.rec[f"{typ}_warp_fw"], ctx.rec[f"{typ}_warp_bw"] = noise_fw, noise_bw
        out('rgb_bw', n_rays, 3)
        args.update(raw_fw=raw_fw, raw_bw=raw_bw, xyz_fw=xyz_fw, xyz_bw=xyz_bw,
                    noise_fw=noise_fw if nstd != 0 else None,
                    noise_bw=noise_bw if nstd != 0 else None,
                    rgb_fw=results['rgb_fw'], rgb_bw=results['rgb_bw'],
                    xyzs_fw_bw=out('xyzs_fw_bw', n_rays, S, 3),
                    xyzs_bw_fw=out('xyzs_bw_fw', n_rays, S, 3))

    if output_transient:
        args['static_weights'] = out(f'static_weights_{typ}', n_rays, S)
        args['transient_weights'] = out(f'transient_weights_{typ}', n_rays, S)
        args['weights'] = out(f'weights_{typ}', n_rays, S)
    else:
        args['static_weights'] = out(f'static_weights_{typ}', n_rays, S)
    if test_time and output_transient:
        args['static_alphas'] = out(f'static_alphas_{typ}', n_rays, S)
        args['transient_alphas'] = out(f'transient_alphas_{typ}', n_rays, S)

    if not sigma_only:
        args['depth'] = out(f'depth_{typ}', n_rays)
        args['rgb'] = out(f'rgb_{typ}', n_rays, 3)
        if output_transient:
            args['transient_alpha'] = out(f'transient_alpha_{typ}', n_rays)
            args['transient_rgb'] = out(f'transient_rgb_{typ}', n_rays, 3)
            args['static_only_rgb'] = out(f'_static_rgb_{typ}', n_rays, 3)
            args['static_only_depth'] = out(f'_static_depth_{typ}', n_rays)
            if want_flow:
                args['flow_mode'] = 2 if warps else 1
                args['xyz_exp'] = out('xyz_fine', n_rays, 3)
                args['flow_fw_exp'] = out('transient_flow_fw', n_rays, 3)
                args['xyz_fw_exp'] = out('xyz_fw', n_rays, 3)
                args['flow_bw_exp'] = out('transient_flow_bw', n_rays, 3)
                args['xyz_bw_exp'] = out('xyz_bw', n_rays, 3)
                if disocc:
                    args['disocc_fw'] = out('disocc_fw', n_rays, 1)
                    args['disoccs_fw'] = out('disoccs_fw', n_rays, S, 1)
                    args['disocc_bw'] = out('disocc_bw', n_rays, 1)
                    args['disoccs_bw'] = out('disoccs_bw', n_rays, S, 1)
    if n_rays:
        _lib.composite(**args)


def render_rays(models,
                embeddings,
                rays,
                ts,
                max_t,
                N_samples=64,
                perturb=0,
                noise_std=0,
                N_importance=0,
                chunk=1024 * 32,
                test_time=False,
                **kwargs):
    _lib.require_gpu_tensor(rays, "rays")
    return range_check.checked(
        "render_rays", rays.device,
        lambda: _render_rays(models, embeddings, rays, ts, max_t, N_samples, perturb, noise_std, N_importance, chunk, test_time, kwargs),
        can_fallback=bool(test_time) and perturb == 0 and noise_std == 0)


def _render_rays(models, embeddings, rays, ts, max_t, N_samples, perturb, noise_std, N_importance, chunk, test_time, kwargs,
                 fine_points=None):
    _lib.require_gpu_tensor(rays, "rays")
    _lib.load()
    want_grad = (torch.is_grad_enabled() and not test_time and
                 bool(autograd.grad_parameters(models, embeddings)))
    rec = {} if want_grad else None
    with torch.cuda.device(rays.device), torch.no_grad():
        results = {}
        rays = rays.contiguous().float()
        n_rays = rays.shape[0]
        embedding_xyz, embedding_dir = embeddings['xyz'], embeddings['dir']

        ctx = _Pass()
        ctx.embeddings, ctx.rays, ctx.ts, ctx.max_t = embeddings, rays, ts, max_t
        ctx.noise_std, ctx.test_time, ctx.kwargs, ctx.n_rays = noise_std, test_time, kwargs, n_rays
        ctx.freqs_xyz = [float(f) for f in embedding_xyz.freqs]
        ctx.rec = rec
        ctx.tbias, ctx.neighbour_rows = {}, None
        ctx.dir_embedded = None
        if any(m.use_viewdir for m in models.values()):
            view_dir = kwargs.get('view_dir', rays[:, 3:6])
            ctx.dir_embedded = embedding_dir(view_dir.contiguous().float())

        z_lin = _unit_linspace(N_samples, rays.device)
        zs = _new(rays, n_rays, N_samples)
        xyz_coarse = _new(rays, n_rays, N_samples, 3)
        ctx.draws = _Draws(rays.device, n_rays, N_samples, N_importance, perturb, noise_std, test_time, models, kwargs,
                           coarse=(rays, z_lin, zs, xyz_coarse))
        perturb_rand = ctx.draws.take("rand", n_rays, N_samples) if perturb > 0 else None
        if n_rays and not ctx.draws.coarse_done:
            _lib.coarse_samples(rays, z_lin, perturb, perturb_rand, zs, xyz_coarse)

        t_embedded = None
        if N_importance > 0:
            model = models['coarse']
            output_transient = bool(kwargs.get('output_transient', True) and model.encode_transient)
            t_embedded = _time_codes(ctx, models, kwargs, N_samples, N_importance, output_transient,
                                     kwargs.get('output_transient_flow', []))
            _inference(results, ctx, model, xyz_coarse, zs, output_transient, [], t_embedded, None)

            det = perturb == 0
            if det:
                u_s = _unit_linspace(N_importance, rays.device)
                u_t = u_s
            else:
                u_s = ctx.draws.take("rand", n_rays, N_importance)
                u_t = ctx.draws.take("rand", n_rays, N_importance) if output_transient else None
            S_fine = N_samples + (2 if output_transient else 1) * N_importance
            zs_static = _new(rays, n_rays, N_importance) if test_time else None
            zs_transient = _new(rays, n_rays, N_importance) if (test_time and output_transient) else None
            zs_fine = _new(rays, n_rays, S_fine)
            xyz_fine = _new(rays, n_rays, S_fine, 3)
            if n_rays:
                _lib.fine_samples(rays, z_lin, zs, N_importance,
                                  results['static_weights_coarse'],
                                  results['transient_weights_coarse'] if output_transient else None,
                                  u_s, u_t if output_transient else None, 0 if det else 1,
                                  zs_static, zs_transient, zs_fine, xyz_fine)
            if test_time:
                results['static_zs_fine'] = zs_static
                if output_transient:
                    results['transient_zs_fine'] = zs_transient
            if fine_points is not None:
                zs_fine, xyz_fine = fine_points(rays, zs_fine, xyz_fine)
                if tuple(zs_fine.shape) != (n_rays, S_fine) or tuple(xyz_fine.shape) != (n_rays, S_fine, 3):
                    raise ValueError(f"fine_points: expected shapes {(n_rays, S_fine)} / {(n_rays, S_fine, 3)}")
            zs, xyz = zs_fine, xyz_fine
        else:
            xyz = xyz_coarse

        model = models['fine']
        a_embedded = None
        if model.encode_appearance:
            a_embedded = kwargs['a_embedded'] if 'a_embedded' in kwargs else embeddings['a'](ts)
            a_embedded = a_embedded.detach().contiguous().float()
        if N_importance == 0:
            output_transient = bool(kwargs.get('output_transient', True) and model.encode_transient)
            t_embedded = _time_codes(ctx, models, kwargs, N_samples, 0, output_transient, kwargs.get('output_transient_flow', []))
        output_transient_flow = [] if not output_transient else kwargs.get('output_transient_flow', [])
        _inference(results, ctx, model, xyz, zs, output_transient, output_transient_flow,
                   t_embedded, a_embedded)
    if rec is None:
        return results
    rec.update(N_importance=N_importance, noise_std=float(noise_std), output_transient=output_transient,
               flows=list(output_transient_flow), zs_coarse=results.get('zs_coarse', results.get('zs_fine')),
               zs_fine=results['zs_fine'], view_dir=kwargs.get('view_dir', rays[:, 3:6]), dir_embedded=ctx.dir_embedded,
               t_embedded_override=kwargs.get('t_embedded'), a_embedded_override=kwargs.get('a_embedded'))
    return autograd.attach(results, models, embeddings, rays, ts, max_t, rec)


from .interpolation import interpolate
```

Baseline: 71.44 million ray-samples/s.

## Fuse coarse composite with fine sampling and vectorize chunked composite

Adds a coarse_fine kernel in which one wave composites the coarse ray and keeps its weights in LDS while the other waves stage bins and coarse z values. The fine importance sampling then reads those weights from LDS, which removes one kernel launch and a global round trip of the coarse weights. The chunked composite kernel also gains a vectorized variant that loads records as float4, stages xyz and per-sample outputs in LDS for coalesced stores, batches the four transmittance scans into one, and batches the wave reductions. The cost is that only one wave does the composite while the others wait, and the extra LDS may lower occupancy.

```diff
diff --git a/include/nsff_render.h b/include/nsff_render.h
--- a/include/nsff_render.h
+++ b/include/nsff_render.h
@@ -369,6 +369,10 @@
 
 int nsff_composite(const NsffCompositeArgs* args, void* stream);
 
+int nsff_coarse_fine(const NsffCompositeArgs* coarse, const float* rays, const float* z_lin, int32_t n_importance,
+                     const float* u_static, const float* u_transient, int32_t u_per_ray,
+                     float* samples_static, float* samples_transient, float* zs_fine, float* xyz_fine, void* stream);
+
 int nsff_frustum_visibility(const NsffFrustumArgs* vis, const float* xyz, int64_t n_points, float* vis_count,
                             void* stream);
 
diff --git a/nsff_pl_amd/_lib.py b/nsff_pl_amd/_lib.py
--- a/nsff_pl_amd/_lib.py
+++ b/nsff_pl_amd/_lib.py
@@ -323,6 +323,7 @@
                                   C.c_float, _fp, _fp]),
     "nsff_warp_points": (C.c_int, [_fp, _fp, _fp, C.c_int64, C.c_float, _fp, _fp, _fp]),
     "nsff_composite": (C.c_int, [C.POINTER(CompositeArgs), _fp]),
+    "nsff_coarse_fine": (C.c_int, [C.POINTER(CompositeArgs), _fp, _fp, C.c_int32, _fp, _fp, C.c_int32, _fp, _fp, _fp, _fp, _fp]),
     "nsff_frustum_visibility": (C.c_int, [C.POINTER(FrustumArgs), _fp, C.c_int64, _fp, _fp]),
     "nsff_frame_rays": (C.c_int, [C.POINTER(C.c_float), C.POINTER(C.c_float), C.c_int32, C.c_int32, C.c_float,
                                   C.c_float, C.c_int64, C.c_int64, _fp, _fp]),
@@ -812,7 +813,7 @@
            "nsff_frustum_visibility")
 
 
-def composite(vis=None, **kw):
+def _composite_args(vis, kw):
     a = CompositeArgs()
     for k, v in kw.items():
         if k in _COMPOSITE_PTRS_IN or k in _COMPOSITE_PTRS_OUT:
@@ -821,7 +822,28 @@
             setattr(a, k, v)
     if vis is not None:
         a.vis = vis
-    _check(load().nsff_composite(C.byref(a), _stream()), "nsff_composite")
+    return a
+
+
+def composite(vis=None, **kw):
+    _check(load().nsff_composite(C.byref(_composite_args(vis, kw)), _stream()), "nsff_composite")
+
+
+def stage_step_on(step):
+    return not (os.environ.get("NSFF_NO_STAGE_FUSION") or os.environ.get(step))
+
+
+def coarse_fine_can_fuse(coarse):
+    return (3 <= coarse["n_samples"] <= 64 and coarse.get("vis") is None and coarse.get("visibility") is None
+            and stage_step_on("NSFF_NO_COARSE_FINE"))
+
+
+def coarse_fine(coarse, rays, z_lin, n_importance, u_static, u_transient, u_per_ray, samples_static, samples_transient,
+                zs_fine, xyz_fine):
+    a = _composite_args(None, {k: v for k, v in coarse.items() if k != "vis"})
+    _check(load().nsff_coarse_fine(C.byref(a), _ptr(rays), _ptr(z_lin), int(n_importance), _ptr(u_static), _ptr(u_transient),
+                                   int(u_per_ray), _ptr(samples_static), _ptr(samples_transient), _ptr(zs_fine), _ptr(xyz_fine),
+                                   _stream()), "nsff_coarse_fine")
 
 
 def frame_rays(K4, c2w12, H, W, near, shift_near, first, count, rays):
diff --git a/nsff_pl_amd/csrc/rays.hip b/nsff_pl_amd/csrc/rays.hip
--- a/nsff_pl_amd/csrc/rays.hip
+++ b/nsff_pl_amd/csrc/rays.hip
@@ -11,6 +11,26 @@
 #pragma unroll
     for (int off = 32; off > 0; off >>= 1) v += __shfl_xor(v, off);
     return v;
+}
+
+template <int N>
+__device__ __forceinline__ void wave_sum_many(float* p) {
+#pragma unroll
+    for (int off = 32; off > 0; off >>= 1) {
+        float u[N];
+#pragma unroll
+        for (int k = 0; k < N; ++k) u[k] = __shfl_xor(p[k], off);
+#pragma unroll
+        for (int k = 0; k < N; ++k) p[k] += u[k];
+    }
+}
+
+__device__ __forceinline__ void wave_scan_mul4(float& a, float& b, float& c, float& d, int lane) {
+#pragma unroll
+    for (int off = 1; off < 64; off <<= 1) {
+        const float ua = __shfl_up(a, off), ub = __shfl_up(b, off), uc = __shfl_up(c, off), ud = __shfl_up(d, off);
+        if (lane >= off) { a *= ua; b *= ub; c *= uc; d *= ud; }
+    }
 }
 
 __device__ __forceinline__ float wave_scan_mul(float v, int lane) {
@@ -98,24 +118,30 @@
     float* zs_fine; float* xyz_fine;
 };
 
-__global__ __launch_bounds__(64 * WAVES_PER_BLOCK) void fine_samples_kernel(const FineArgs a) {
-    extern __shared__ __attribute__((aligned(16))) float smem[];
+__host__ __device__ __forceinline__ int fine_lds_floats(int S, int Sf) { return WAVES_PER_BLOCK * S + ((S + 3) & ~3) + ((Sf + 3) & ~3); }
+
+__device__ __forceinline__ void fine_stage_inputs(const FineArgs& a, const long long ray, float* smem, const int tid, const int n) {
+    const int S = a.S;
+    float* bins = smem + WAVES_PER_BLOCK * S;
+    float* merged = bins + ((S + 3) & ~3);
+    for (int j = tid; j < S - 1; j += n) bins[j] = 0.5f * (a.z_lin[j] + a.z_lin[j + 1]);
+    for (int j = tid; j < S; j += n) merged[j] = a.zs_coarse[ray * S + j];
+}
+
+__device__ __forceinline__ void fine_samples_ray(const FineArgs& a, const long long ray, float* smem, const float* w_static,
+                                                 const float* w_transient) {
     const int lane = threadIdx.x & 63, wave = threadIdx.x >> 6, tid = threadIdx.x;
     constexpr int T = 64 * WAVES_PER_BLOCK;
-    const long long ray = blockIdx.x;
     const int S = a.S, n_imp = a.n_imp;
     const int k_sets = a.w_transient ? 2 : 1;
     const int Sf = S + k_sets * n_imp;
     float* cdf = smem + wave * S;
     float* bins = smem + WAVES_PER_BLOCK * S;
     float* merged = bins + ((S + 3) & ~3);
-    for (int j = tid; j < S - 1; j += T) bins[j] = 0.5f * (a.z_lin[j] + a.z_lin[j + 1]);
-    for (int j = tid; j < S; j += T) merged[j] = a.zs_coarse[ray * S + j];
-    __syncthreads();
     {
         const bool mine = wave < k_sets;
         const int set = mine ? wave : 0;
-        const float* w = (set == 0 ? a.w_static : a.w_transient) + ray * S + 1;
+        const float* w = (set == 0 ? w_static : w_transient) + 1;
         const float* ub = set == 0 ? a.u_static : a.u_transient;
         const float* u = a.u_per_ray ? ub + ray * n_imp : ub;
         float* keep = set == 0 ? a.samples_static : a.samples_transient;
@@ -145,6 +171,14 @@
         a.xyz_fine[dst * 3 + 1] = o1 + d1 * v;
         a.xyz_fine[dst * 3 + 2] = o2 + d2 * v;
     }
+}
+
+__global__ __launch_bounds__(64 * WAVES_PER_BLOCK) void fine_samples_kernel(const FineArgs a) {
+    extern __shared__ __attribute__((aligned(16))) float smem[];
+    const long long ray = blockIdx.x;
+    fine_stage_inputs(a, ray, smem, threadIdx.x, 64 * WAVES_PER_BLOCK);
+    __syncthreads();
+    fine_samples_ray(a, ray, smem, a.w_static + ray * a.S, a.w_transient ? a.w_transient + ray * a.S : nullptr);
 }
 
 struct PdfArgs {
@@ -297,10 +331,8 @@
     if (p < n_points) out[p] = frustum_count(v, xyz[3 * p], xyz[3 * p + 1], xyz[3 * p + 2]);
 }
 
-__global__ __launch_bounds__(64 * WAVES_PER_BLOCK) void composite_kernel(const NsffCompositeArgs a) {
-    const int lane = threadIdx.x & 63;
-    const long long ray = (long long)blockIdx.x * WAVES_PER_BLOCK + (threadIdx.x >> 6);
-    if (ray >= a.n_rays) return;
+__device__ __forceinline__ void composite_ray(const NsffCompositeArgs& a, const long long ray, const int lane,
+                                              float* keep_ws, float* keep_wt) {
     const int S = a.n_samples;
     const bool tr = a.has_transient != 0;
     const bool flows = tr && a.flow_mode >= 1;
@@ -371,6 +403,8 @@
                 if (a.static_weights) a.static_weights[idx] = w;
                 if (a.weights) a.weights[idx] = w;
             }
+            if (keep_ws) keep_ws[i] = tr ? w_s : w;
+            if (keep_wt) keep_wt[i] = w_t;
         }
         if (!a.has_rgb) continue;
 
@@ -505,10 +539,44 @@
     }
 }
 
-template <int NCH>
+__global__ __launch_bounds__(64 * WAVES_PER_BLOCK) void composite_kernel(const NsffCompositeArgs a) {
+    const long long ray = (long long)blockIdx.x * WAVES_PER_BLOCK + (threadIdx.x >> 6);
+    if (ray >= a.n_rays) return;
+    composite_ray(a, ray, threadIdx.x & 63, nullptr, nullptr);
+}
+
+__global__ __launch_bounds__(64 * WAVES_PER_BLOCK) void coarse_fine_kernel(const NsffCompositeArgs ca, const FineArgs a) {
+    extern __shared__ __attribute__((aligned(16))) float smem[];
+    const int lane = threadIdx.x & 63, wave = threadIdx.x >> 6;
+    constexpr int T = 64 * WAVES_PER_BLOCK;
+    const long long ray = blockIdx.x;
+    const int S = a.S;
+    const int k_sets = a.w_transient ? 2 : 1;
+    float* w_s = smem + fine_lds_floats(S, S + k_sets * a.n_imp);
+    float* w_t = w_s + S;
+    if (wave == 0) composite_ray(ca, ray, lane, w_s, a.w_transient ? w_t : nullptr);
+    else fine_stage_inputs(a, ray, smem, (int)threadIdx.x - 64, T - 64);
+    __syncthreads();
+    fine_samples_ray(a, ray, smem, w_s, w_t);
+}
+
+constexpr int STAGE_IN = 3, STAGE_OUT = 6, STAGE_LEN = 192;
+enum { ST_XYZ, ST_XYZ_FW, ST_XYZ_BW, ST_SRGB, ST_TRGB, ST_FLOW_FW, ST_FLOW_BW, ST_CYC_FW, ST_CYC_BW };
+
+__device__ __forceinline__ void load_record(float* dst, const float* src, int first_quad, int n_quads) {
+#pragma unroll
+    for (int q = 0; q < 4; ++q) {
+        if (q < first_quad || q >= first_quad + n_quads) continue;
+        const float4 v = reinterpret_cast<const float4*>(src)[q];
+        dst[4 * q + 0] = v.x; dst[4 * q + 1] = v.y; dst[4 * q + 2] = v.z; dst[4 * q + 3] = v.w;
+    }
+}
+
+template <int NCH, bool VEC>
 __global__ __launch_bounds__(64 * NCH) void composite_kernel_chunks(const NsffCompositeArgs a) {
     __shared__ float tot[NCH][4];
     __shared__ float part[NCH][32];
+    __shared__ float stage[VEC ? NCH * (STAGE_IN + STAGE_OUT) * STAGE_LEN : 1];
     const int lane = threadIdx.x & 63, c = threadIdx.x >> 6;
     const long long ray = blockIdx.x;
     const int S = a.n_samples;
@@ -525,6 +593,31 @@
     const float d_s = last ? 100.f : dz;
     const float d_t = last ? 1e-3f : dz;
     const float* rec = a.raw + idx * RS;
+    float rec_v[16], recw_v[2][16];
+    float* st = stage + (VEC ? c * (STAGE_IN + STAGE_OUT) * STAGE_LEN : 0);
+    const long long idx0 = ray * S + 64 * c;
+    const int n3 = 3 * min(64, S - 64 * c);
+    if constexpr (VEC) {
+        load_record(rec_v, rec, 0, 4);
+        rec = rec_v;
+        if (a.has_rgb && warps) {
+            load_record(recw_v[0], a.raw_fw + idx * RS, 1, 3);
+            load_record(recw_v[1], a.raw_bw + idx * RS, 1, 2);
+        }
+        if (a.has_rgb && flows) {
+#pragma unroll
+            for (int j = 0; j < 3; ++j) {
+                const int e = 64 * j + lane;
+                if (e < n3) {
+                    st[ST_XYZ * STAGE_LEN + e] = a.xyz[idx0 * 3 + e];
+                    if (warps) {
+                        st[ST_XYZ_FW * STAGE_LEN + e] = a.xyz_fw[idx0 * 3 + e];
+                        st[ST_XYZ_BW * STAGE_LEN + e] = a.xyz_bw[idx0 * 3 + e];
+                    }
+                }
+            }
+        }
+    }
 
     float sig_s = rec[3];
     if (a.noise_static) sig_s += a.noise_static[idx] * a.noise_std;
@@ -545,21 +638,28 @@
         alpha = 1.f - (1.f - al_s) * (1.f - al_t);
         if (a.has_rgb) { rgb_t[0] = rec[4]; rgb_t[1] = rec[5]; rgb_t[2] = rec[6]; }
     }
-    const float inc = wave_scan_mul(on ? 1.f - alpha : 1.f, lane);
+    const bool scan4 = VEC && a.has_rgb && warps;
+    float inc = on ? 1.f - alpha : 1.f;
+    if (!scan4) inc = wave_scan_mul(inc, lane);
     float incs = 1.f, incw[2] = {1.f, 1.f}, al_tw[2] = {0.f, 0.f};
-    if (a.has_rgb && tr) incs = wave_scan_mul(on ? 1.f - al_s : 1.f, lane);
+    if (a.has_rgb && tr) {
+        incs = on ? 1.f - al_s : 1.f;
+        if (!scan4) incs = wave_scan_mul(incs, lane);
+    }
     if (a.has_rgb && warps) {
 #pragma unroll
         for (int dir = 0; dir < 2; ++dir) {
-            const float* recw = (dir == 0 ? a.raw_fw : a.raw_bw) + idx * RS;
+            const float* recw = VEC ? recw_v[dir] : (dir == 0 ? a.raw_fw : a.raw_bw) + idx * RS;
             const float* nz = dir == 0 ? a.noise_fw : a.noise_bw;
             float sg = recw[7];
             if (nz) sg += nz[idx] * a.noise_std;
             al_tw[dir] = 1.f - expf(-d_t * softplus(sg));
             const float al_w = 1.f - (1.f - al_s) * (1.f - al_tw[dir]);
-            incw[dir] = wave_scan_mul(on ? 1.f - al_w : 1.f, lane);
-        }
-    }
+            incw[dir] = on ? 1.f - al_w : 1.f;
+            if (!scan4) incw[dir] = wave_scan_mul(incw[dir], lane);
+        }
+    }
+    if (scan4) wave_scan_mul4(inc, incs, incw[0], incw[1], lane);
     if (lane == 63) { tot[c][0] = inc; tot[c][1] = incs; tot[c][2] = incw[0]; tot[c][3] = incw[1]; }
     __syncthreads();
     float cT = 1.f, cTs = 1.f, cTw[2] = {1.f, 1.f};
@@ -572,14 +672,14 @@
     if (on) {
         if (a.static_sigmas) a.static_sigmas[idx] = sig_s;
         if (a.has_rgb && a.static_rgbs) {
-            a.static_rgbs[idx * 3 + 0] = rgb_s[0]; a.static_rgbs[idx * 3 + 1] = rgb_s[1];
-            a.static_rgbs[idx * 3 + 2] = rgb_s[2];
+            float* o = VEC ? st + ST_SRGB * STAGE_LEN + lane * 3 : a.static_rgbs + idx * 3;
+            o[0] = rgb_s[0]; o[1] = rgb_s[1]; o[2] = rgb_s[2];
         }
         if (tr) {
             if (a.transient_sigmas) a.transient_sigmas[idx] = sig_t;
             if (a.has_rgb && a.transient_rgbs) {
-                a.transient_rgbs[idx * 3 + 0] = rgb_t[0]; a.transient_rgbs[idx * 3 + 1] = rgb_t[1];
-                a.transient_rgbs[idx * 3 + 2] = rgb_t[2];
+                float* o = VEC ? st + ST_TRGB * STAGE_LEN + lane * 3 : a.transient_rgbs + idx * 3;
+                o[0] = rgb_t[0]; o[1] = rgb_t[1]; o[2] = rgb_t[2];
             }
             if (a.static_alphas) a.static_alphas[idx] = al_s;
             if (a.transient_alphas) a.transient_alphas[idx] = al_t;
@@ -627,20 +727,20 @@
         for (int k = 0; k < 3; ++k) {
             ffw[k] = far ? 0.f : rec[8 + k];
             fbw[k] = far ? 0.f : rec[11 + k];
-            x[k] = a.xyz[idx * 3 + k];
+            x[k] = VEC ? st[ST_XYZ * STAGE_LEN + lane * 3 + k] : a.xyz[idx * 3 + k];
         }
         if (on) {
 #pragma unroll
             for (int k = 0; k < 3; ++k) {
-                if (a.flows_fw) a.flows_fw[idx * 3 + k] = ffw[k];
-                if (a.flows_bw) a.flows_bw[idx * 3 + k] = fbw[k];
+                if (a.flows_fw) (VEC ? st[ST_FLOW_FW * STAGE_LEN + lane * 3 + k] : a.flows_fw[idx * 3 + k]) = ffw[k];
+                if (a.flows_bw) (VEC ? st[ST_FLOW_BW * STAGE_LEN + lane * 3 + k] : a.flows_bw[idx * 3 + k]) = fbw[k];
                 p[P_XYZ + k] = w * x[k]; p[P_FFW + k] = w * ffw[k]; p[P_FBW + k] = w * fbw[k];
             }
         }
         if (warps) {
 #pragma unroll
             for (int dir = 0; dir < 2; ++dir) {
-                const float* recw = (dir == 0 ? a.raw_fw : a.raw_bw) + idx * RS;
+                const float* recw = VEC ? recw_v[dir] : (dir == 0 ? a.raw_fw : a.raw_bw) + idx * RS;
                 float excw = __shfl_up(incw[dir], 1);
                 if (lane == 0) excw = 1.f;
                 const float Tw = cTw[dir] * excw;
@@ -648,12 +748,14 @@
                 if (on) {
 #pragma unroll
                     for (int k = 0; k < 3; ++k) p[(dir == 0 ? P_RGBFW : P_RGBBW) + k] = ws_w * rgb_s[k] + wt_w * recw[4 + k];
-                    const float* xw = (dir == 0 ? a.xyz_fw : a.xyz_bw) + idx * 3;
+                    const float* xw = VEC ? st + (dir == 0 ? ST_XYZ_FW : ST_XYZ_BW) * STAGE_LEN + lane * 3
+                                          : (dir == 0 ? a.xyz_fw : a.xyz_bw) + idx * 3;
                     float* cyc = dir == 0 ? a.xyzs_fw_bw : a.xyzs_bw_fw;
                     const int head = dir == 0 ? 11 : 8;
                     if (cyc) {
-#pragma unroll
-                        for (int k = 0; k < 3; ++k) cyc[idx * 3 + k] = xw[k] + (far ? 0.f : recw[head + k]);
+                        float* o = VEC ? st + (dir == 0 ? ST_CYC_FW : ST_CYC_BW) * STAGE_LEN + lane * 3 : cyc + idx * 3;
+#pragma unroll
+                        for (int k = 0; k < 3; ++k) o[k] = xw[k] + (far ? 0.f : recw[head + k]);
                     }
                     const float occ = wt_w - w_t;
                     if (dir == 0) { p[P_OCCFW] = occ; if (a.disoccs_fw) a.disoccs_fw[idx] = 1.f - fabsf(occ); }
@@ -663,14 +765,38 @@
         }
     }
     const int n_used = warps ? (int)P_N : (flows ? (int)P_RGBFW : (tr ? (int)P_XYZ : (int)P_TRGB));
-#pragma unroll
-    for (int k = 0; k < P_N; ++k) {
-        if (k < n_used) {
-            const float v = wave_sum(p[k]);
-            if (lane == 0) part[c][k] = v;
+    if constexpr (VEC) {
+        if (warps) wave_sum_many<P_N>(p);
+        else if (flows) wave_sum_many<P_RGBFW>(p);
+        else if (tr) wave_sum_many<P_XYZ>(p);
+        else wave_sum_many<P_TRGB>(p);
+        if (lane == 0) {
+#pragma unroll
+            for (int k = 0; k < P_N; ++k) if (k < n_used) part[c][k] = p[k];
+        }
+    } else {
+#pragma unroll
+        for (int k = 0; k < P_N; ++k) {
+            if (k < n_used) {
+                const float v = wave_sum(p[k]);
+                if (lane == 0) part[c][k] = v;
+            }
         }
     }
     __syncthreads();
+    if constexpr (VEC) {
+        float* const outs[STAGE_OUT] = {a.static_rgbs, tr ? a.transient_rgbs : nullptr, flows ? a.flows_fw : nullptr,
+                                        flows ? a.flows_bw : nullptr, warps ? a.xyzs_fw_bw : nullptr, warps ? a.xyzs_bw_fw : nullptr};
+#pragma unroll
+        for (int o = 0; o < STAGE_OUT; ++o) {
+            if (!outs[o]) continue;
+#pragma unroll
+            for (int j = 0; j < 3; ++j) {
+                const int e = 64 * j + lane;
+                if (e < n3) outs[o][idx0 * 3 + e] = st[(STAGE_IN + o) * STAGE_LEN + e];
+            }
+        }
+    }
     if (threadIdx.x != 0) return;
     float s[P_N];
 #pragma unroll
@@ -810,6 +936,8 @@
     }
 }
 
+bool stage_step_off(const char* step) { return getenv("NSFF_NO_STAGE_FUSION") != nullptr || getenv(step) != nullptr; }
+
 }
 
 extern "C" {
@@ -865,7 +993,7 @@
                weights_static, weights_transient, u_static, u_transient, u_per_ray,
                samples_static, samples_transient, zs_fine, xyz_fine};
     const int Sf = n_samples + (weights_transient ? 2 : 1) * n_importance;
-    const size_t lds = (size_t)(WAVES_PER_BLOCK * n_samples + ((n_samples + 3) & ~3) + Sf) * sizeof(float);
+    const size_t lds = (size_t)fine_lds_floats(n_samples, Sf) * sizeof(float);
     if (lds > 64 * 1024 || n_rays > 0x7fffffffLL) return NSFF_ERR_INVALID;
     const unsigned blocks = (unsigned)n_rays;
     hipLaunchKernelGGL(fine_samples_kernel, dim3(blocks), dim3(64 * WAVES_PER_BLOCK), lds,
@@ -930,23 +1058,56 @@
     return nsff_launch_status();
 }
 
-int nsff_composite(const NsffCompositeArgs* args, void* stream) {
-    if (!args) return NSFF_ERR_NULL;
-    const NsffCompositeArgs& a = *args;
-    if (a.n_rays < 0 || a.n_samples < 1 || a.flow_mode < 0 || a.flow_mode > 2) return NSFF_ERR_INVALID;
-    if (a.n_rays == 0) return NSFF_OK;
+static int composite_args_status(const NsffCompositeArgs& a) {
     if (!a.raw || !a.zs) return NSFF_ERR_NULL;
     if (a.flow_mode && (!a.has_transient || !a.has_rgb)) return NSFF_ERR_INVALID;
     if (a.flow_mode >= 1 && !a.xyz) return NSFF_ERR_NULL;
     if (a.flow_mode == 2 && (!a.raw_fw || !a.raw_bw || !a.xyz_fw || !a.xyz_bw)) return NSFF_ERR_NULL;
     if (a.vis.w2c && (!a.vis.ts || !a.xyz)) return NSFF_ERR_NULL;
     if (a.vis.w2c && (a.vis.n_cams < 1 || a.vis.n_frames < 1)) return NSFF_ERR_INVALID;
+    return NSFF_OK;
+}
+
+int nsff_coarse_fine(const NsffCompositeArgs* coarse, const float* rays, const float* z_lin, int32_t n_importance,
+                     const float* u_static, const float* u_transient, int32_t u_per_ray,
+                     float* samples_static, float* samples_transient, float* zs_fine, float* xyz_fine, void* stream) {
+    if (!coarse) return NSFF_ERR_NULL;
+    const NsffCompositeArgs& c = *coarse;
+    if (c.n_rays < 0 || c.n_samples < 3 || c.flow_mode < 0 || c.flow_mode > 2 || n_importance < 1) return NSFF_ERR_INVALID;
+    if (c.n_samples > 64 || c.vis.w2c || c.visibility) return NSFF_ERR_UNSUPPORTED;
+    if (c.n_rays == 0) return NSFF_OK;
+    if (const int rc = composite_args_status(c)) return rc;
+    if (!rays || !z_lin || !u_static || !zs_fine || !xyz_fine || !c.static_weights) return NSFF_ERR_NULL;
+    if (c.has_transient && (!u_transient || !c.transient_weights)) return NSFF_ERR_NULL;
+    FineArgs f{rays, (long long)c.n_rays, z_lin, c.zs, c.n_samples, n_importance,
+               c.static_weights, c.has_transient ? c.transient_weights : nullptr, u_static, u_transient, u_per_ray,
+               samples_static, samples_transient, zs_fine, xyz_fine};
+    const int Sf = c.n_samples + (c.has_transient ? 2 : 1) * n_importance;
+    const size_t lds = (size_t)(fine_lds_floats(c.n_samples, Sf) + 2 * c.n_samples) * sizeof(float);
+    if (lds > 64 * 1024 || c.n_rays > 0x7fffffffLL) return NSFF_ERR_INVALID;
+    hipLaunchKernelGGL(coarse_fine_kernel, dim3((unsigned)c.n_rays), dim3(64 * WAVES_PER_BLOCK), lds, (hipStream_t)stream, c, f);
+    return nsff_launch_status();
+}
+
+int nsff_composite(const NsffCompositeArgs* args, void* stream) {
+    if (!args) return NSFF_ERR_NULL;
+    const NsffCompositeArgs& a = *args;
+    if (a.n_rays < 0 || a.n_samples < 1 || a.flow_mode < 0 || a.flow_mode > 2) return NSFF_ERR_INVALID;
+    if (a.n_rays == 0) return NSFF_OK;
+    if (const int rc = composite_args_status(a)) return rc;
     const int nch = (a.n_samples + 63) / 64;
     if (nch >= 2 && nch <= 4 && a.n_rays <= 0x7fffffffLL && getenv("NSFF_SERIAL_COMPOSITE") == nullptr) {
         const dim3 grid((unsigned)a.n_rays);
-        if (nch == 2) hipLaunchKernelGGL(composite_kernel_chunks<2>, grid, dim3(128), 0, (hipStream_t)stream, a);
-        else if (nch == 3) hipLaunchKernelGGL(composite_kernel_chunks<3>, grid, dim3(192), 0, (hipStream_t)stream, a);
-        else hipLaunchKernelGGL(composite_kernel_chunks<4>, grid, dim3(256), 0, (hipStream_t)stream, a);
+        const bool vec = !(((uintptr_t)a.raw | (uintptr_t)a.raw_fw | (uintptr_t)a.raw_bw) & 15) && !stage_step_off("NSFF_NO_VEC_COMPOSITE");
+        if (vec) {
+            if (nch == 2) hipLaunchKernelGGL((composite_kernel_chunks<2, true>), grid, dim3(128), 0, (hipStream_t)stream, a);
+            else if (nch == 3) hipLaunchKernelGGL((composite_kernel_chunks<3, true>), grid, dim3(192), 0, (hipStream_t)stream, a);
+            else hipLaunchKernelGGL((composite_kernel_chunks<4, true>), grid, dim3(256), 0, (hipStream_t)stream, a);
+        } else {
+            if (nch == 2) hipLaunchKernelGGL((composite_kernel_chunks<2, false>), grid, dim3(128), 0, (hipStream_t)stream, a);
+            else if (nch == 3) hipLaunchKernelGGL((composite_kernel_chunks<3, false>), grid, dim3(192), 0, (hipStream_t)stream, a);
+            else hipLaunchKernelGGL((composite_kernel_chunks<4, false>), grid, dim3(256), 0, (hipStream_t)stream, a);
+        }
         return nsff_launch_status();
     }
     const unsigned blocks = (unsigned)((a.n_rays + WAVES_PER_BLOCK - 1) / WAVES_PER_BLOCK);
diff --git a/nsff_pl_amd/graphs.py b/nsff_pl_amd/graphs.py
--- a/nsff_pl_amd/graphs.py
+++ b/nsff_pl_amd/graphs.py
@@ -52,7 +52,8 @@
         if not rays.is_cuda:
             raise RuntimeError("GraphedRender needs GPU tensors (there is no CPU path)")
         shape_key = (int(rays.shape[0]), ts is not None, config.get_precision(), config.get_tile_points(), config.get_persistent(),
-                     os.environ.get("NSFF_H3A_SHAPE", ""))
+                     os.environ.get("NSFF_H3A_SHAPE", ""),
+                     tuple(bool(os.environ.get(k)) for k in ("NSFF_NO_STAGE_FUSION", "NSFF_NO_COARSE_FINE", "NSFF_NO_VEC_COMPOSITE")))
         key = shape_key + (self._param_addresses(),)
         entry = self._graphs.get(key)
         if entry is None:
diff --git a/nsff_pl_amd/rendering.py b/nsff_pl_amd/rendering.py
--- a/nsff_pl_amd/rendering.py
+++ b/nsff_pl_amd/rendering.py
@@ -160,7 +160,7 @@
 
 
 def _inference(results, ctx, model, xyz, zs, output_transient, output_transient_flow,
-               t_embedded, a_embedded):
+               t_embedded, a_embedded, defer_composite=False):
     typ = model.typ
     n_rays, S = zs.shape
     test_time = ctx.test_time
@@ -299,7 +299,10 @@
                     args['disocc_bw'] = out('disocc_bw', n_rays, 1)
                     args['disoccs_bw'] = out('disoccs_bw', n_rays, S, 1)
     if n_rays:
+        if defer_composite and _lib.coarse_fine_can_fuse(args):
+            return args
         _lib.composite(**args)
+    return None
 
 
 def render_rays(models,
@@ -360,7 +363,8 @@
             output_transient = bool(kwargs.get('output_transient', True) and model.encode_transient)
             t_embedded = _time_codes(ctx, models, kwargs, N_samples, N_importance, output_transient,
                                      kwargs.get('output_transient_flow', []))
-            _inference(results, ctx, model, xyz_coarse, zs, output_transient, [], t_embedded, None)
+            coarse_args = _inference(results, ctx, model, xyz_coarse, zs, output_transient, [], t_embedded, None,
+                                     defer_composite=fine_points is None)
 
             det = perturb == 0
             if det:
@@ -374,7 +378,10 @@
             zs_transient = _new(rays, n_rays, N_importance) if (test_time and output_transient) else None
             zs_fine = _new(rays, n_rays, S_fine)
             xyz_fine = _new(rays, n_rays, S_fine, 3)
-            if n_rays:
+            if coarse_args is not None:
+                _lib.coarse_fine(coarse_args, rays, z_lin, N_importance, u_s, u_t if output_transient else None,
+                                 0 if det else 1, zs_static, zs_transient, zs_fine, xyz_fine)
+            elif n_rays:
                 _lib.fine_samples(rays, z_lin, zs, N_importance,
                                   results['static_weights_coarse'],
                                   results['transient_weights_coarse'] if output_transient else None,
```

After: 71.62 million ray-samples/s, median of 6. About the same (+0.3%).
